# vgl-hub/kreeq

Measured on AMD Instinct MI355X. Metric: distinct+total k-mers/sec at k=21 (count path), higher is better.
Workload: dtype u64

## Files before the change

### include/kreeq_amd.h

```cpp
#ifndef KREEQ_AMD_H
#define KREEQ_AMD_H

#include <stdint.h>

#ifdef __cplusplus
extern "C" {
#endif

#define KQ_ABI_VERSION 4

typedef enum {
    KQ_OK = 0,
    KQ_ERR_INVALID = -1,
    KQ_ERR_NO_DEVICE = -2,
    KQ_ERR_HIP = -3,
    KQ_ERR_NOMEM = -4,
    KQ_ERR_TABLE_FULL = -5,
    KQ_ERR_CAPACITY = -6,
    KQ_ERR_MISMATCH = -7
} kq_status;

typedef struct kq_handle kq_handle;

typedef struct {
    uint64_t key;
    uint32_t fw[4], bw[4], cov;
    uint32_t hc;
} kq_entry;

typedef struct {
    uint32_t fw, bw, cov;
    uint8_t  isFw;
    uint8_t  pad[3];
} kq_dbgbase;

typedef struct {
    uint64_t total;
    uint64_t unique;
    uint64_t distinct;
    uint64_t missing;
    uint64_t edges;
} kq_stats;

typedef struct {
    uint64_t kmers_counted;
    uint64_t slots_used;
    uint64_t slots_total;
    uint64_t hc_used;
    uint64_t hc_total;
    uint64_t table_bytes;
    uint64_t table_passes;
} kq_info;


int  kq_create(kq_handle** out, int device, int k, int map_count, uint64_t capacity_hint);
void kq_destroy(kq_handle* h);
int  kq_clear(kq_handle* h);
int  kq_set_stream(kq_handle* h, void* hip_stream);
void* kq_get_stream(kq_handle* h);
enum { KQ_OPT_TRUST_CAPACITY = 1, KQ_OPT_COUNT_PATH = 2, KQ_OPT_SLICE_KMERS = 3, KQ_OPT_COUNT_MAP_RANGE = 4, KQ_OPT_PROFILE = 5,
       KQ_OPT_LOOKUP_PATH = 6, KQ_OPT_MERGE_PATH = 7, KQ_OPT_NARROW_MID = 8, KQ_OPT_PENDING_BYTES = 9, KQ_OPT_BUCKET_WINDOW = 10, KQ_OPT_OVERLAP = 11, KQ_OPT_COUNT_MAP_PASSES = 12, KQ_OPT_KERNEL_SET = 13, KQ_OPT_SHARD_WINDOW = 14, KQ_OPT_SUBGRAPH_BATCH = 15, KQ_OPT_VARIANT_BATCH = 16,
       KQ_OPT_TEST_FAIL_PLAN = 100  };
int  kq_set_option(kq_handle* h, int option, int64_t value);
int  kq_get_profile(kq_handle* h, char* buf, uint64_t cap);
int  kq_sync(kq_handle* h);
int  kq_flush(kq_handle* h);
int  kq_get_info(kq_handle* h, kq_info* out);
const char* kq_last_error(void);
int  kq_abi_version(void);
int  kq_device_available(void);
int  kq_device_memory(int device, uint64_t* free_bytes, uint64_t* total_bytes);


int  kq_count_batch(kq_handle* h, const char* bases, uint64_t len);
int  kq_count_batch_dev(kq_handle* h, const char* d_bases, uint64_t len);

void* kq_host_alloc(uint64_t bytes);
void  kq_host_free(void* p);
int  kq_count_batch_async(kq_handle* h, const char* bases, uint64_t len, uint64_t* ticket);
int  kq_host_wait(kq_handle* h, uint64_t ticket);

void kq_pack_bases(const char* bases, uint64_t len, uint32_t* codes, uint16_t* inv);
int  kq_count_packed_dev(kq_handle* h, const uint32_t* d_codes, const uint16_t* d_inv, uint64_t n_bases);
int  kq_count_packed_async(kq_handle* h, const uint32_t* codes, const uint16_t* inv, uint64_t n_bases, uint64_t* ticket);

int  kq_pack_bases_dev(kq_handle* h, const char* d_bases, uint64_t len, uint32_t* d_codes, uint16_t* d_inv);

enum { KQ_FASTX_FASTQ = 1, KQ_FASTX_FASTA = 2 };
int  kq_parse_fastx_dev(kq_handle* h, const char* d_text, uint64_t len, int format, char* d_bases, uint64_t cap, uint64_t* n_bases);
int  kq_count_fastx_dev(kq_handle* h, const char* d_text, uint64_t len, int format);
int  kq_count_fastx_async(kq_handle* h, const char* text, uint64_t len, int format, uint64_t* ticket);

typedef struct { uint64_t off; uint32_t size; uint32_t data_off; uint32_t data_len; uint32_t crc32; uint32_t isize; } kq_bgzf_block;
enum { KQ_BGZF_END = 1 };
int  kq_bgzf_scan(const void* data, uint64_t len, kq_bgzf_block* blocks, uint64_t cap, uint64_t* n_blocks, uint64_t* consumed);
int  kq_inflate_bgzf_dev(kq_handle* h, const void* d_comp, uint64_t comp_len, const kq_bgzf_block* blocks, uint64_t n_blocks,
                         char* d_text, uint64_t cap, uint64_t* n_text);
int  kq_count_bgzf_dev(kq_handle* h, const void* d_comp, uint64_t comp_len, const kq_bgzf_block* blocks, uint64_t n_blocks, int format, uint32_t flags);

enum { KQ_BGZF_EOF = 2 };
uint64_t kq_bgzf_bound(uint64_t n_text, uint32_t flags);
int  kq_deflate_bgzf_dev(kq_handle* h, const char* d_text, uint64_t n_text, void* d_out, uint64_t cap, uint64_t* n_out, uint32_t flags);
int  kq_deflate_bgzf(kq_handle* h, const char* text, uint64_t n_text, void* out, uint64_t cap, uint64_t* n_out, uint32_t flags);

int  kq_emit_records(kq_handle* h, const char* bases, uint64_t len,
                     uint64_t* keys, uint8_t* edges, uint64_t cap, uint64_t* n_out);
int  kq_emit_partitioned_dev(kq_handle* h, const char* d_bases, uint64_t len, int n_parts,
                             uint64_t* d_keys, uint8_t* d_edges, uint64_t cap,
                             uint64_t* part_counts);

int  kq_emit_packed_dev(kq_handle* h, const char* d_bases, uint64_t len, int n_parts,
                        uint64_t* d_recs, uint64_t cap, uint64_t* part_counts);
int  kq_insert_packed_dev(kq_handle* h, const uint64_t* d_recs, uint64_t n);

int  kq_emit_sharded_dev(kq_handle* h, const char* d_bases, uint64_t len, int n_parts, uint32_t* d_recs, uint8_t* d_aux, uint64_t cap,
                         uint64_t* d_bucket_counts, uint64_t* part_counts);
int  kq_insert_sharded_dev(kq_handle* h, const uint32_t* d_recs, const uint8_t* d_aux, uint64_t n, int n_peers, const uint64_t* d_bucket_counts);

int  kq_emit_sharded8_dev(kq_handle* h, const char* d_bases, uint64_t len, int n_parts, uint64_t* d_recs, uint64_t cap,
                          uint64_t* d_bucket_counts, uint64_t* part_counts);
int  kq_insert_sharded8_dev(kq_handle* h, const uint64_t* d_recs, uint64_t n, int n_peers, const uint64_t* d_bucket_counts);

int  kq_insert_records(kq_handle* h, const uint64_t* keys, const uint8_t* edges, uint64_t n);
int  kq_insert_records_dev(kq_handle* h, const uint64_t* d_keys, const uint8_t* d_edges, uint64_t n);


int  kq_summary(kq_handle* h, kq_stats* out);
int  kq_histogram(kq_handle* h, uint64_t* cov, uint64_t* cnt, uint64_t cap, uint64_t* n_out);


int  kq_lookup_sequence(kq_handle* h, const char* bases, uint64_t len, uint32_t cov_cutoff,
                        uint16_t map_lo, uint16_t map_hi, kq_dbgbase* per_base,
                        uint64_t counters[3]);
int  kq_lookup_sequence_dev(kq_handle* h, const char* d_bases, uint64_t len, uint32_t cov_cutoff,
                            uint16_t map_lo, uint16_t map_hi, kq_dbgbase* d_per_base,
                            uint64_t* d_counters);


enum { KQ_COPY_TO_DEVICE = 1, KQ_COPY_TO_HOST = 2 };
void* kq_dev_alloc(kq_handle* h, uint64_t bytes);
void  kq_dev_free(kq_handle* h, void* p);
int   kq_copy_async(kq_handle* h, void* dst, const void* src, uint64_t bytes, int kind);

int  kq_per_base_triples_dev(kq_handle* h, const kq_dbgbase* d_per_base, const uint64_t* seg_start, const uint64_t* seg_len,
                             uint64_t n_segs, uint32_t* d_triples);

int  kq_per_base_merge_dev(kq_handle* h, kq_dbgbase* d_per_base, const uint64_t* seg_start, const uint64_t* seg_len,
                           uint64_t n_segs, uint32_t* d_triples);

typedef struct { uint64_t first, n, abs_pos; uint32_t name_off, name_len, n_ctx, flags; } kq_table_seg;
enum { KQ_TABLE_SEG_HEADER = 1 };
enum { KQ_TABLE_KWIG = 1, KQ_TABLE_BED = 2, KQ_TABLE_CSV = 3 };
int  kq_format_table_dev(kq_handle* h, int format, const uint32_t* d_triples, uint64_t n_triples, const kq_table_seg* segs, uint64_t n_segs,
                         const char* names, uint64_t names_len, char* d_out, uint64_t cap, uint64_t* n_out);
int  kq_format_table(kq_handle* h, int format, const uint32_t* triples, uint64_t n_triples, const kq_table_seg* segs, uint64_t n_segs,
                     const char* names, uint64_t names_len, char* out, uint64_t cap, uint64_t* n_out);


int  kq_lookup_keys(kq_handle* h, const uint64_t* keys, uint64_t n, kq_entry* out);

int  kq_branch_scan(kq_handle* h, const char* bases, uint64_t len, uint32_t cov_cutoff, uint8_t* flags);

typedef struct { uint64_t pos, seg_start, seq_off; uint16_t seq_len, ref_len; uint8_t type, pad[3]; } kq_variant_path;
enum { KQ_VAR_SNV = 0, KQ_VAR_INS = 1, KQ_VAR_DEL = 2, KQ_VAR_COM = 3 };
int  kq_search_variants(kq_handle* h, const char* bases, uint64_t len, int depth, int max_span, uint32_t cov_cutoff,
                        kq_variant_path* paths, uint64_t path_cap, uint64_t* n_paths,
                        char* seq, uint64_t seq_cap, uint64_t* n_seq);


int  kq_merge(kq_handle* dst, kq_handle* src);

int  kq_import(kq_handle* h, const kq_entry* entries, uint64_t n);
int  kq_export(kq_handle* h, uint16_t map_lo, uint16_t map_hi, kq_entry* out, uint64_t cap,
               uint64_t* n_out);


int  kq_export_map_images(kq_handle* h, uint16_t map_lo, uint16_t map_hi, void* out, uint64_t cap, uint64_t* offsets,
                          kq_entry* hc_out, uint64_t hc_cap, uint64_t* n_hc);
int  kq_import_map_image(kq_handle* h, uint16_t map, const void* image, uint64_t n_bytes, uint64_t* n_entries,
                         uint64_t* n_tombstones);


enum { KQ_SUBGRAPH_NO_REFERENCE = 1 };
int  kq_subgraph_seed(kq_handle* db, kq_handle* sub, const char* bases, uint64_t len, uint32_t flags);
int  kq_subgraph_seed_dev(kq_handle* db, kq_handle* sub, const char* d_bases, uint64_t len, uint32_t flags);
int  kq_subgraph_expand(kq_handle* db, kq_handle* sub, int depth, uint64_t* n_added);
int  kq_subgraph_best_first(kq_handle* db, kq_handle* sub, int depth, uint32_t cov_cutoff, uint64_t* n_added);
int  kq_subgraph_trim(kq_handle* sub, uint32_t cov_cutoff);

typedef struct { uint64_t seq_off, head_key; uint32_t n_kmers, cov; uint8_t head_rc, pad[7]; } kq_gfa_segment;
typedef struct { uint32_t from, to, count; uint8_t from_rc, to_rc, pad[2]; } kq_gfa_edge;
typedef struct { uint64_t n_segments, n_seq, n_edges, n_dropped_edges, n_cycles; } kq_gfa_counts;
enum { KQ_GFA_NO_COLLAPSE = 1 };
int  kq_subgraph_gfa(kq_handle* sub, uint32_t flags, kq_gfa_segment* segs, uint64_t seg_cap, char* seq, uint64_t seq_cap,
                     kq_gfa_edge* edges, uint64_t edge_cap, kq_gfa_counts* counts);

#ifdef __cplusplus
}
#endif
#endif
```

### kreeq_amd/build.py

```python
import os
import shutil
import subprocess

PKG = os.path.dirname(os.path.abspath(__file__))
ROOT = os.path.dirname(PKG)
LIB = os.path.join(PKG, "lib", "libkreeq_amd.so")
CLI = os.path.join(PKG, "bin", "kreeq")
HOSTLIB = os.path.join(PKG, "lib", "libkreeq_host.so")

HIP_SOURCES = [os.path.join(PKG, "csrc", "kreeq_amd.hip")]
HIP_DEPS = HIP_SOURCES + [os.path.join(PKG, "csrc", f) for f in ("kq_device.h", "kq_partition.h", "kq_kernels.h", "kq_fastx.h", "kq_bgzf.h", "kq_bgzf_host.h", "kq_inflate_core.h", "kq_deflate.h", "kq_deflate_core.h", "kq_dbimage.h", "kq_dbimage_host.h", "kq_mem_host.h", "kq_plan_host.h", "kq_roff_host.h", "kq_seg_gate_host.h", "kq_select_host.h", "kq_formats.h", "kq_subgraph.h", "kq_gfa.h", "kq_bestfirst_core.h", "kq_nodequeue_core.h", "kq_variant_core.h", "kq_variants.h", "kq_table_core.h", "kq_table.h")] + [os.path.join(ROOT, "include", "kreeq_amd.h")]
HOST_DIR = os.path.join(PKG, "host")
DECOMPRESSOR_DIR = os.path.join(HOST_DIR, "decompressor")
DECOMPRESSOR = os.path.join(PKG, "bin", "kreeq-decompressor")


def _stale(target, deps):
    if not os.path.exists(target):
        return True
    t = os.path.getmtime(target)
    return any(os.path.getmtime(d) > t for d in deps if os.path.exists(d))


def hipcc():
    for c in (shutil.which("hipcc"), "/opt/rocm/bin/hipcc"):
        if c and os.path.exists(c):
            return c
    raise RuntimeError("hipcc not found: the HIP library cannot be built (there is no CPU fallback)")


def build_lib(force=False, verbose=False, out=None, defines=()):
    target = out or LIB
    if force or _stale(target, HIP_DEPS):
        os.makedirs(os.path.dirname(target), exist_ok=True)
        cmd = [hipcc(), "-O3", "-std=c++17", "--offload-arch=gfx950", "-fPIC", "-shared", "-Wall", "-Wextra",
               "-o", target] + ["-D" + d for d in defines] + HIP_SOURCES
        if verbose:
            print(" ".join(cmd))
        subprocess.check_call(cmd)
    return target


def host_sources():
    if not os.path.isdir(HOST_DIR):
        return []
    return sorted(os.path.join(HOST_DIR, f) for f in os.listdir(HOST_DIR) if f.endswith(".cpp") and f != "hostlib.cpp")


def build_hostlib(force=False, verbose=False):
    srcs = [os.path.join(HOST_DIR, f) for f in ("hostlib.cpp", "kreeq_db.cpp")]
    deps = srcs + [os.path.join(HOST_DIR, "kreeq_db.h"), os.path.join(ROOT, "include", "kreeq_amd.h")]
    if force or _stale(HOSTLIB, deps):
        os.makedirs(os.path.dirname(HOSTLIB), exist_ok=True)
        cmd = ["g++", "-O2", "-std=c++17", "-Wall", "-Wextra", "-fPIC", "-shared", "-pthread", "-I", os.path.join(ROOT, "include"), "-o", HOSTLIB] + srcs
        if verbose:
            print(" ".join(cmd))
        subprocess.check_call(cmd)
    return HOSTLIB


def build_cli(force=False, verbose=False):
    srcs = host_sources()
    if not srcs:
        return None
    deps = srcs + [os.path.join(HOST_DIR, f) for f in os.listdir(HOST_DIR) if f.endswith(".h")] + [LIB]
    if force or _stale(CLI, deps):
        os.makedirs(os.path.dirname(CLI), exist_ok=True)
        cmd = ["g++", "-O2", "-std=c++17", "-Wall", "-Wextra", "-pthread", "-I", os.path.join(ROOT, "include"), "-o", CLI] + srcs + \
              ["-L", os.path.dirname(LIB), "-lkreeq_amd", "-lz", "-Wl,-rpath,$ORIGIN/../lib"]
        if verbose:
            print(" ".join(cmd))
        subprocess.check_call(cmd)
    return CLI


def build_decompressor(force=False, verbose=False):
    srcs = [os.path.join(DECOMPRESSOR_DIR, "main.cpp")]
    deps = srcs + [os.path.join(HOST_DIR, "bkwig_index.h"), os.path.join(PKG, "csrc", "kq_table_core.h"), os.path.join(ROOT, "include", "kreeq_amd.h"), LIB]
    if force or _stale(DECOMPRESSOR, deps):
        os.makedirs(os.path.dirname(DECOMPRESSOR), exist_ok=True)
        cmd = ["g++", "-O2", "-std=c++17", "-Wall", "-Wextra", "-o", DECOMPRESSOR] + srcs + \
              ["-L", os.path.dirname(LIB), "-lkreeq_amd", "-Wl,-rpath,$ORIGIN/../lib"]
        if verbose:
            print(" ".join(cmd))
        subprocess.check_call(cmd)
    return DECOMPRESSOR


def build_all(force=False, verbose=False):
    build_lib(force, verbose)
    build_cli(force, verbose)
    build_decompressor(force, verbose)
    build_hostlib(force, verbose)
```

### kreeq_amd/capi.py

```python
import ctypes as C
import os

import numpy as np

from . import build as _build

ENTRY_DTYPE = np.dtype([("key", "<u8"), ("fw", "<u4", 4), ("bw", "<u4", 4), ("cov", "<u4"), ("hc", "<u4")])
DBGBASE_DTYPE = np.dtype([("fw", "<u4"), ("bw", "<u4"), ("cov", "<u4"), ("isFw", "u1"), ("pad", "u1", 3)])
VARIANT_PATH_DTYPE = np.dtype([("pos", "<u8"), ("seg_start", "<u8"), ("seq_off", "<u8"), ("seq_len", "<u2"), ("ref_len", "<u2"), ("type", "u1"), ("pad", "u1", 3)])
VAR_SNV, VAR_INS, VAR_DEL, VAR_COM = 0, 1, 2, 3
ERR_CAPACITY = -6

SYMBOLS = ["kq_create", "kq_destroy", "kq_clear", "kq_set_option", "kq_get_profile", "kq_set_stream", "kq_get_stream", "kq_sync", "kq_flush", "kq_get_info", "kq_last_error",
           "kq_abi_version", "kq_device_available", "kq_device_memory", "kq_count_batch", "kq_count_batch_dev", "kq_host_alloc", "kq_host_free", "kq_count_batch_async", "kq_host_wait", "kq_pack_bases", "kq_count_packed_dev", "kq_count_packed_async",
           "kq_pack_bases_dev", "kq_parse_fastx_dev", "kq_count_fastx_dev", "kq_count_fastx_async", "kq_bgzf_scan", "kq_inflate_bgzf_dev", "kq_count_bgzf_dev", "kq_bgzf_bound", "kq_deflate_bgzf_dev", "kq_deflate_bgzf", "kq_emit_records",
           "kq_emit_partitioned_dev", "kq_emit_packed_dev", "kq_insert_packed_dev", "kq_emit_sharded_dev", "kq_insert_sharded_dev", "kq_emit_sharded8_dev", "kq_insert_sharded8_dev", "kq_insert_records", "kq_insert_records_dev", "kq_summary", "kq_histogram",
           "kq_lookup_sequence", "kq_lookup_sequence_dev", "kq_dev_alloc", "kq_dev_free", "kq_copy_async", "kq_per_base_triples_dev", "kq_per_base_merge_dev", "kq_format_table_dev", "kq_format_table", "kq_lookup_keys", "kq_branch_scan", "kq_search_variants", "kq_merge", "kq_import", "kq_export",
           "kq_export_map_images", "kq_import_map_image", "kq_subgraph_seed", "kq_subgraph_seed_dev", "kq_subgraph_expand", "kq_subgraph_best_first", "kq_subgraph_trim", "kq_subgraph_gfa"]

FASTX_FASTQ, FASTX_FASTA = 1, 2
BGZF_END = 1
BGZF_EOF = 2
BGZF_MEMBER_TEXT = 0xff00
BGZF_BLOCK_DTYPE = np.dtype([("off", "<u8"), ("size", "<u4"), ("data_off", "<u4"), ("data_len", "<u4"), ("crc32", "<u4"), ("isize", "<u4"), ("pad", "<u4")])
TABLE_KWIG, TABLE_BED, TABLE_CSV = 1, 2, 3
TABLE_SEG_HEADER = 1
TABLE_SEG_DTYPE = np.dtype([("first", "<u8"), ("n", "<u8"), ("abs_pos", "<u8"), ("name_off", "<u4"), ("name_len", "<u4"), ("n_ctx", "<u4"), ("flags", "<u4")])
SUBGRAPH_NO_REFERENCE = 1
GFA_NO_COLLAPSE = 1
GFA_SEGMENT_DTYPE = np.dtype([("seq_off", "<u8"), ("head_key", "<u8"), ("n_kmers", "<u4"), ("cov", "<u4"), ("head_rc", "u1"), ("pad", "u1", 7)])
GFA_EDGE_DTYPE = np.dtype([("from", "<u4"), ("to", "<u4"), ("count", "<u4"), ("from_rc", "u1"), ("to_rc", "u1"), ("pad", "u1", 2)])


class KqError(RuntimeError):
    def __init__(self, code, msg):
        super().__init__(f"kreeq_amd error {code}: {msg}")
        self.code = code


class Stats(C.Structure):
    _fields_ = [("total", C.c_uint64), ("unique", C.c_uint64), ("distinct", C.c_uint64), ("missing", C.c_uint64),
                ("edges", C.c_uint64)]


class GfaCounts(C.Structure):
    _fields_ = [("n_segments", C.c_uint64), ("n_seq", C.c_uint64), ("n_edges", C.c_uint64), ("n_dropped_edges", C.c_uint64), ("n_cycles", C.c_uint64)]


class Info(C.Structure):
    _fields_ = [("kmers_counted", C.c_uint64), ("slots_used", C.c_uint64), ("slots_total", C.c_uint64), ("hc_used", C.c_uint64),
                ("hc_total", C.c_uint64), ("table_bytes", C.c_uint64), ("table_passes", C.c_uint64)]


_lib = None


def lib_path():
    return _build.LIB


def _preload_process_hip_runtime():
    import importlib.util

    try:
        spec = importlib.util.find_spec("torch")
    except (ImportError, ValueError):
        spec = None
    if not spec or not spec.origin:
        return
    d = os.path.join(os.path.dirname(spec.origin), "lib")
    for name in ("libhsa-runtime64.so", "libamdhip64.so"):
        p = os.path.join(d, name)
        if os.path.exists(p):
            try:
                C.CDLL(p, mode=C.RTLD_GLOBAL)
            except OSError:
                return


def load():
    global _lib
    if _lib is not None:
        return _lib
    path = os.environ.get("KQ_LIB") or _build.LIB
    if not os.path.exists(path):
        raise KqError(-2, f"{path} is missing: build it with `python -c 'import __graft_entry__ as g; g.build()'` "
                          "(the product has no CPU fallback)")
    _preload_process_hip_runtime()
    L = C.CDLL(path)
    vp, u64, u32, u16, ci = C.c_void_p, C.c_uint64, C.c_uint32, C.c_uint16, C.c_int
    L.kq_create.argtypes = [C.POINTER(vp), ci, ci, ci, u64]
    L.kq_destroy.argtypes = [vp]
    L.kq_destroy.restype = None
    L.kq_clear.argtypes = [vp]
    L.kq_set_stream.argtypes = [vp, vp]
    L.kq_set_option.argtypes = [vp, ci, C.c_int64]
    L.kq_get_profile.argtypes = [vp, C.c_char_p, u64]
    L.kq_get_stream.argtypes = [vp]
    L.kq_get_stream.restype = vp
    L.kq_sync.argtypes = [vp]
    L.kq_flush.argtypes = [vp]
    L.kq_get_info.argtypes = [vp, C.POINTER(Info)]
    L.kq_last_error.restype = C.c_char_p
    L.kq_device_memory.argtypes = [ci, C.POINTER(u64), C.POINTER(u64)]
    L.kq_count_batch.argtypes = [vp, vp, u64]
    L.kq_count_batch_dev.argtypes = [vp, vp, u64]
    L.kq_host_alloc.argtypes = [u64]
    L.kq_host_alloc.restype = vp
    L.kq_host_free.argtypes = [vp]
    L.kq_host_free.restype = None
    L.kq_count_batch_async.argtypes = [vp, vp, u64, C.POINTER(u64)]
    L.kq_host_wait.argtypes = [vp, u64]
    L.kq_pack_bases.argtypes = [vp, u64, vp, vp]
    L.kq_pack_bases.restype = None
    L.kq_count_packed_dev.argtypes = [vp, vp, vp, u64]
    L.kq_count_packed_async.argtypes = [vp, vp, vp, u64, C.POINTER(u64)]
    L.kq_pack_bases_dev.argtypes = [vp, vp, u64, vp, vp]
    L.kq_parse_fastx_dev.argtypes = [vp, vp, u64, ci, vp, u64, C.POINTER(u64)]
    L.kq_count_fastx_dev.argtypes = [vp, vp, u64, ci]
    L.kq_count_fastx_async.argtypes = [vp, vp, u64, ci, C.POINTER(u64)]
    L.kq_bgzf_scan.argtypes = [vp, u64, vp, u64, C.POINTER(u64), C.POINTER(u64)]
    L.kq_inflate_bgzf_dev.argtypes = [vp, vp, u64, vp, u64, vp, u64, C.POINTER(u64)]
    L.kq_count_bgzf_dev.argtypes = [vp, vp, u64, vp, u64, ci, u32]
    L.kq_bgzf_bound.argtypes = [u64, u32]
    L.kq_bgzf_bound.restype = u64
    L.kq_deflate_bgzf_dev.argtypes = [vp, vp, u64, vp, u64, C.POINTER(u64), u32]
    L.kq_deflate_bgzf.argtypes = [vp, vp, u64, vp, u64, C.POINTER(u64), u32]
    L.kq_emit_records.argtypes = [vp, vp, u64, vp, vp, u64, C.POINTER(u64)]
    L.kq_emit_partitioned_dev.argtypes = [vp, vp, u64, ci, vp, vp, u64, vp]
    L.kq_emit_packed_dev.argtypes = [vp, vp, u64, ci, vp, u64, vp]
    L.kq_insert_packed_dev.argtypes = [vp, vp, u64]
    L.kq_emit_sharded_dev.argtypes = [vp, vp, u64, ci, vp, vp, u64, vp, vp]
    L.kq_insert_sharded_dev.argtypes = [vp, vp, vp, u64, ci, vp]
    L.kq_emit_sharded8_dev.argtypes = [vp, vp, u64, ci, vp, u64, vp, vp]
    L.kq_insert_sharded8_dev.argtypes = [vp, vp, u64, ci, vp]
    L.kq_insert_records.argtypes = [vp, vp, vp, u64]
    L.kq_insert_records_dev.argtypes = [vp, vp, vp, u64]
    L.kq_summary.argtypes = [vp, C.POINTER(Stats)]
    L.kq_histogram.argtypes = [vp, vp, vp, u64, C.POINTER(u64)]
    L.kq_lookup_sequence.argtypes = [vp, vp, u64, u32, u16, u16, vp, vp]
    L.kq_lookup_sequence_dev.argtypes = [vp, vp, u64, u32, u16, u16, vp, vp]
    L.kq_dev_alloc.argtypes = [vp, u64]
    L.kq_dev_alloc.restype = vp
    L.kq_dev_free.argtypes = [vp, vp]
    L.kq_dev_free.restype = None
    L.kq_copy_async.argtypes = [vp, vp, vp, u64, ci]
    L.kq_per_base_triples_dev.argtypes = [vp, vp, vp, vp, u64, vp]
    L.kq_per_base_merge_dev.argtypes = [vp, vp, vp, vp, u64, vp]
    L.kq_format_table_dev.argtypes = [vp, ci, vp, u64, vp, u64, vp, u64, vp, u64, C.POINTER(u64)]
    L.kq_format_table.argtypes = [vp, ci, vp, u64, vp, u64, vp, u64, vp, u64, C.POINTER(u64)]
    L.kq_lookup_keys.argtypes = [vp, vp, u64, vp]
    L.kq_branch_scan.argtypes = [vp, vp, u64, u32, vp]
    L.kq_search_variants.argtypes = [vp, vp, u64, ci, ci, u32, vp, u64, C.POINTER(u64), vp, u64, C.POINTER(u64)]
    L.kq_merge.argtypes = [vp, vp]
    L.kq_import.argtypes = [vp, vp, u64]
    L.kq_export.argtypes = [vp, u16, u16, vp, u64, C.POINTER(u64)]
    L.kq_export_map_images.argtypes = [vp, u16, u16, vp, u64, vp, vp, u64, C.POINTER(u64)]
    L.kq_import_map_image.argtypes = [vp, u16, vp, u64, C.POINTER(u64), C.POINTER(u64)]
    L.kq_subgraph_seed.argtypes = [vp, vp, vp, u64, u32]
    L.kq_subgraph_seed_dev.argtypes = [vp, vp, vp, u64, u32]
    L.kq_subgraph_expand.argtypes = [vp, vp, ci, C.POINTER(u64)]
    L.kq_subgraph_best_first.argtypes = [vp, vp, ci, u32, C.POINTER(u64)]
    L.kq_subgraph_trim.argtypes = [vp, u32]
    L.kq_subgraph_gfa.argtypes = [vp, u32, vp, u64, vp, u64, vp, u64, C.POINTER(GfaCounts)]
    _lib = L
    return L


def _check(rc):
    if rc != 0:
        raise KqError(rc, load().kq_last_error().decode(errors="replace"))


def _p(a):
    return a.ctypes.data_as(C.c_void_p) if a is not None else None


def pack_bases(bases: bytes):
    buf = np.frombuffer(bases, dtype=np.uint8)
    units = (len(buf) + 15) // 16
    codes, inv = np.zeros(max(units, 1), dtype=np.uint32), np.zeros(max(units, 1), dtype=np.uint16)
    load().kq_pack_bases(_p(buf) if len(buf) else None, len(buf), _p(codes), _p(inv))
    return codes[:units], inv[:units]


def bgzf_bound(n_text, flags=0):
    return int(load().kq_bgzf_bound(n_text, flags))


def bgzf_scan(data: bytes, cap=None):
    buf = np.frombuffer(data, dtype=np.uint8)
    n, used = C.c_uint64(0), C.c_uint64(0)
    L = load()
    room = len(buf) // 26 + 1 if cap is None else cap
    blocks = np.zeros(max(room, 1), dtype=BGZF_BLOCK_DTYPE)
    rc = L.kq_bgzf_scan(_p(buf) if len(buf) else None, len(buf), _p(blocks) if room else None, room, C.byref(n), C.byref(used))
    if rc != 0:
        e = KqError(rc, L.kq_last_error().decode(errors="replace"))
        e.n_blocks, e.consumed = n.value, used.value
        raise e
    return blocks[:n.value], used.value


def device_available():
# ... 356 lines not shown
```

### kreeq_amd/csrc/kq_formats.h

```cpp
#pragma once
#include <cstdint>
namespace kq {
#ifndef KQ_REGION_SHIFT
#define KQ_REGION_SHIFT 11
#endif
constexpr int REGION_SHIFT = KQ_REGION_SHIFT;
constexpr uint32_t REGION_SLOTS = 1u << REGION_SHIFT;
constexpr int HI_K = 29;
constexpr int TILE_STARTS = 4032;
constexpr uint64_t n_tiles_of(uint64_t lead, uint64_t len) { return (lead + len + TILE_STARTS - 1) / TILE_STARTS; }
struct EmitRange { uint64_t lo, hi; };

constexpr int NB_MAX = 2048;
constexpr int PART_MAX_K = 28;
constexpr int FMT_PACK8 = 0, FMT_WIDE = 1, FMT_NARROW = 2;
constexpr int FMT_PACK8_TO_NARROW = 3;
constexpr uint32_t NARROW_CBITS = 8, NARROW_MAX_K = 21;
constexpr int FMT_TOP8 = 4;
constexpr int FMT_TIGHT = 5;
constexpr int FMT_NARROW_TO_TIGHT = 6;

constexpr int MS_THREADS = 256;
constexpr int MS_ITEMS = 16;
constexpr int MS_TILE = MS_THREADS * MS_ITEMS;
constexpr int SEG_MAX = 65536;
constexpr uint32_t SUB_BITS_MAX = 8;
constexpr int AUX_IDX6 = 0, AUX_EDGE_BYTE = 1, AUX_TIGHT = 2;
constexpr uint64_t TIGHT_MIN_REGIONS = 1ull << 16;
constexpr int P1_F = 1;
constexpr uint32_t P2_UNIT = 4 * MS_TILE;
constexpr uint32_t SCAN_CHUNK = 16384;

struct PartCfg {
    uint64_t n_regions;
    uint32_t g_shift;
    uint32_t n_coarse;
    uint32_t mode;
    uint32_t map_count;
    uint32_t map_mask;
    uint32_t filt_lo, filt_hi;
    uint32_t raw_out;
    uint32_t narrow;
    uint32_t owner_sub;
    uint32_t sub_bits;
    uint32_t win_lo, win_hi;
    uint32_t n_rng;
};

constexpr int P3_MAX_SETS = 64;
struct P3Set { const uint64_t* recs; const uint8_t* aux; const unsigned long long* base; uint64_t n_max; };

struct LevelCfg {
    uint64_t n_regions;
    uint32_t n_seg, nb, seg_shift, out_shift;
    uint32_t in_raw;
    uint32_t k;
    uint32_t narrow;
    uint32_t top8;
    uint32_t nr_shift, nr_rps, nr_sub, nr_div, nr_inv;
    uint32_t nr_mid, nr_fshift, nr_fmask, nr_f24;
    uint32_t spb;
    uint32_t rep_shift;
    const uint32_t* rstart = nullptr;
};
}
```

### kreeq_amd/csrc/kq_kernels.h

```cpp
#pragma once

#include <hip/hip_runtime.h>

#include <type_traits>

#include "../../include/kreeq_amd.h"
#include "kq_device.h"
#include "kq_partition.h"

using namespace kq;


__global__ __launch_bounds__(TILE_THREADS) void k_count_direct(TableView t, const uint8_t* __restrict__ ab,
                                                                uint64_t lead, uint64_t len, int k, EmitRange er, PartCfg filt,
                                                                const uint16_t* __restrict__ pinv ) {
    uint32_t n_new = 0;
    uint64_t n_kmers = 0;
    scan_tiles(ab, lead, len, k, [&](uint64_t pos, uint64_t fw, uint64_t rv, uint32_t prev, uint32_t next) {
        if (pos < er.lo || pos >= er.hi) return;
        const bool is_fw = fw < rv;
        const uint64_t key = is_fw ? fw : rv;
        if (filt.filt_lo != 0 || filt.filt_hi != filt.map_count) {
            const uint32_t m = map_index(key, filt.map_count, filt.map_mask);
            if (m < filt.filt_lo || m >= filt.filt_hi) return;
// ... 376 lines not shown
        });
        landed(nxt.x); landed(nxt.y); landed(nxt.z); landed(nxt.w);
    }
}

__global__ __launch_bounds__(1024) void k_lv_units(const unsigned long long* __restrict__ seg_off, const unsigned long long* __restrict__ seg_hi, LevelCfg lv,
                                                   unsigned long long* __restrict__ unit_base) {
    __shared__ unsigned long long s_part[1024];
    const uint32_t tid = threadIdx.x, per = (lv.n_seg + 1023) / 1024;
    const uint32_t lo = min(tid * per, lv.n_seg), hi = min(lo + per, lv.n_seg);
    unsigned long long sum = 0;
    for (uint32_t b = lo; b < hi; ++b) sum += (seg_hi[b] - seg_off[b] + P2_UNIT - 1) / P2_UNIT;
    s_part[tid] = sum;
    __syncthreads();
    if (tid < 64) {
        unsigned long long loc[16], tot = 0;
#pragma unroll
        for (int j = 0; j < 16; ++j) { loc[j] = s_part[tid * 16 + j]; tot += loc[j]; }
        unsigned long long incl = tot;
#pragma unroll
        for (int o = 1; o < 64; o <<= 1) { unsigned long long nn = __shfl_up(incl, o, 64); if ((int)tid >= o) incl += nn; }
        unsigned long long run = incl - tot;
#pragma unroll
        for (int j = 0; j < 16; ++j) { s_part[tid * 16 + j] = run; run += loc[j]; }
        if (tid == 63) unit_base[lv.n_seg] = incl;
    }
    __syncthreads();
    unsigned long long run = s_part[tid];
    for (uint32_t b = lo; b < hi; ++b) { unit_base[b] = run; run += (seg_hi[b] - seg_off[b] + P2_UNIT - 1) / P2_UNIT; }
}
__device__ __forceinline__ uint32_t seg_of_unit(const unsigned long long* unit_base, uint32_t n_seg, uint64_t u) {
    uint32_t lo = 0, hi = n_seg;
    while (hi - lo > 1) { uint32_t mid = (lo + hi) >> 1; if (unit_base[mid] <= u) lo = mid; else hi = mid; }
    return lo;
}
template <int FMT>
__global__ __launch_bounds__(MS_THREADS) void k_lv_hist(const uint64_t* __restrict__ recs, const uint8_t* __restrict__ , LevelCfg lv,
                                                        const unsigned long long* __restrict__ seg_off, const unsigned long long* __restrict__ seg_hi,
                                                        const unsigned long long* __restrict__ unit_base, uint32_t* __restrict__ m2) {
    __shared__ uint32_t s_hist[NB_MAX];
    const uint64_t n_units = unit_base[lv.n_seg];
    for (uint64_t u = blockIdx.x; u < n_units; u += gridDim.x) {
        const uint32_t b_in = seg_of_unit(unit_base, lv.n_seg, u);
        const uint32_t b = lv.spb > 1 ? b_in / lv.spb : b_in;
        const uint64_t lo = seg_off[b_in] + (u - unit_base[b_in]) * P2_UNIT;
        const uint64_t hi = lo + P2_UNIT < seg_hi[b_in] ? lo + P2_UNIT : seg_hi[b_in];
        for (uint32_t i = threadIdx.x; i < lv.nb; i += MS_THREADS) s_hist[i] = 0;
        __syncthreads();
        const uint64_t last = hi - 1;
        if (FMT == FMT_NARROW) {
            const uint4* v4 = reinterpret_cast<const uint4*>(recs);
            const uint64_t q0 = lo >> 2, q1 = (hi + 3) >> 2;
            for (uint64_t qb = q0; qb < q1; qb += 4ull * MS_THREADS) {
                uint4 q[4];
#pragma unroll
                for (int j = 0; j < 4; ++j) q[j] = v4[min(qb + (uint64_t)j * MS_THREADS + threadIdx.x, q1 - 1)];
#pragma unroll
                for (int j = 0; j < 4; ++j) {
                    const uint64_t qi = qb + (uint64_t)j * MS_THREADS + threadIdx.x;
                    const uint32_t e[4] = {q[j].x, q[j].y, q[j].z, q[j].w};
#pragma unroll
                    for (int c = 0; c < 4; ++c) {
                        const uint64_t ri = 4 * qi + c;
                        if (qi < q1 && ri >= lo && ri < hi) atomicAdd(&s_hist[narrow_bin(lv, b, e[c])], 1u);
                    }
                }
            }
        } else
        for (uint64_t base = lo; base < hi; base += 8ull * MS_THREADS) {
            uint64_t r[8];
#pragma unroll
            for (int j = 0; j < 8; ++j) {
                const uint64_t i = min(base + (uint64_t)j * MS_THREADS + threadIdx.x, last);
                r[j] = FMT == FMT_NARROW ? (uint64_t)reinterpret_cast<const uint32_t*>(recs)[i] : recs[i];
            }
#pragma unroll
            for (int j = 0; j < 8; ++j)
                if (base + (uint64_t)j * MS_THREADS + threadIdx.x < hi) {
                    const uint32_t bin = FMT == FMT_NARROW ? narrow_bin(lv, b, (uint32_t)r[j])
                        : FMT == FMT_TOP8 ? narrow_bin(lv, b, (uint32_t)(r[j] >> 32))
                        : (FMT == FMT_PACK8 && lv.top8) ? (uint32_t)(rec_hash<false>(r[j]) >> (64 - NARROW_CBITS))
                        : level_bin(lv, b, hash_region(lv.in_raw ? table_hash(r[j], lv.k) : rec_hash<FMT == FMT_WIDE>(r[j]), lv.n_regions));
                    atomicAdd(&s_hist[bin], 1u);
                }
        }
        __syncthreads();
        for (uint32_t i = threadIdx.x; i < lv.nb; i += MS_THREADS) m2[u * lv.nb + i] = s_hist[i];
        __syncthreads();
    }
}
__global__ __launch_bounds__(256) void k_lv_offsets(uint32_t* __restrict__ m2, LevelCfg lv, const unsigned long long* __restrict__ unit_base,
                                                    unsigned long long* __restrict__ group_count) {
    const uint64_t r = ((uint64_t)blockIdx.x * blockDim.x + threadIdx.x) >> 6;
    const uint32_t lane = threadIdx.x & 63;
    const uint32_t n_lseg = lv.n_seg / lv.spb;
    if (r >= (uint64_t)n_lseg * lv.nb) return;
    const uint32_t b = (uint32_t)(r / lv.nb), bin = (uint32_t)(r % lv.nb);
    const uint64_t u0 = unit_base[b * lv.spb], u1 = unit_base[(b + 1) * lv.spb];
    unsigned long long run = 0;
    for (uint64_t base = u0; base < u1; base += 64) {
        const uint64_t u = base + lane;
        const uint32_t c = u < u1 ? m2[u * lv.nb + bin] : 0u;
        unsigned long long incl = c;
#pragma unroll
        for (int o = 1; o < 64; o <<= 1) { const unsigned long long n = __shfl_up(incl, o, 64); if ((int)lane >= o) incl += n; }
        if (u < u1) m2[u * lv.nb + bin] = (uint32_t)(run + incl - c);
        run += __shfl(incl, 63, 64);
    }
    if (lane == 0) group_count[r] = run;
}
__global__ __launch_bounds__(256) void k_lv_offsets_thread(uint32_t* __restrict__ m2, LevelCfg lv, const unsigned long long* __restrict__ unit_base,
                                                           unsigned long long* __restrict__ group_count) {
    const uint64_t r = (uint64_t)blockIdx.x * blockDim.x + threadIdx.x;
    const uint32_t n_lseg = lv.n_seg / lv.spb;
    if (r >= (uint64_t)n_lseg * lv.nb) return;
    const uint32_t b = (uint32_t)(r / lv.nb), bin = (uint32_t)(r % lv.nb);
    const uint64_t u0 = unit_base[b * lv.spb], u1 = unit_base[(b + 1) * lv.spb];
    unsigned long long run = 0;
    for (uint64_t u = u0; u < u1; ++u) {
        const uint32_t c = m2[u * lv.nb + bin];
        m2[u * lv.nb + bin] = (uint32_t)run;
        run += c;
    }
    group_count[r] = run;
}
#ifndef KQ_LV_THREADS
#define KQ_LV_THREADS 512
#define KQ_LV_ITEMS 8
#define KQ_LV_OCC 4
#endif
constexpr int LV_THREADS = KQ_LV_THREADS, LV_ITEMS = KQ_LV_ITEMS, LV_TILE = LV_THREADS * LV_ITEMS;
template <int FMT, int NBC>
__global__ __launch_bounds__(LV_THREADS, KQ_LV_OCC) void k_lv_scatter(const uint64_t* __restrict__ recs, const uint8_t* __restrict__ recs_aux, LevelCfg lv,
                                                           const unsigned long long* __restrict__ seg_off, const unsigned long long* __restrict__ seg_hi,
                                                           const unsigned long long* __restrict__ unit_base, const uint32_t* __restrict__ m2,
                                                           const unsigned long long* __restrict__ group_base, uint64_t* __restrict__ out,
                                                           uint8_t* __restrict__ out_aux) {
    constexpr bool WIDE = FMT == FMT_WIDE, TIGHT = FMT == FMT_NARROW_TO_TIGHT, NARROW = FMT == FMT_NARROW || TIGHT, CONVERT = FMT == FMT_PACK8_TO_NARROW,
                   TOP8 = FMT == FMT_TOP8, HAS_AUX = WIDE || NARROW;
    constexpr int MS_FMT = (CONVERT || TIGHT) ? FMT_NARROW : TOP8 ? FMT_PACK8 : FMT;
    const uint32_t* recs32 = reinterpret_cast<const uint32_t*>(recs);
    __shared__ MsShared<NBC, MS_FMT, LV_TILE> s;
    __shared__ uint32_t s_rst[TIGHT ? NBC : 1];
    const uint32_t nb = lv.nb;
    const uint64_t n_units = unit_base[lv.n_seg];
    for (uint64_t u = blockIdx.x; u < n_units; u += gridDim.x) {
        const uint32_t b_in = seg_of_unit(unit_base, lv.n_seg, u);
        const uint32_t b = lv.spb > 1 ? b_in / lv.spb : b_in;
        const uint64_t lo = seg_off[b_in] + (u - unit_base[b_in]) * P2_UNIT;
        const uint64_t hi = lo + P2_UNIT < seg_hi[b_in] ? lo + P2_UNIT : seg_hi[b_in];
        for (uint32_t i = threadIdx.x; i < nb; i += LV_THREADS)
            s.gbase[i] = (uint32_t)(group_base[(uint64_t)b * nb + i] + m2[u * nb + i]);
        if (TIGHT) {
            const uint32_t first = (b >> lv.nr_shift) * lv.nr_rps + (b & ((1u << lv.nr_shift) - 1u)) * lv.nr_sub;
            for (uint32_t i = threadIdx.x; i < nb; i += LV_THREADS) s_rst[i] = lv.rstart[first + i];
        }
        __syncthreads();
        uint64_t nxt[LV_ITEMS];
        uint32_t nxt_aux[LV_ITEMS];
        const uint64_t last = hi - 1;
#pragma unroll
        for (int j = 0; j < LV_ITEMS; ++j) {
            const uint64_t i = min(lo + (uint64_t)j * LV_THREADS + threadIdx.x, last);
            nxt[j] = NARROW ? (uint64_t)recs32[i] : recs[i];
            nxt_aux[j] = HAS_AUX ? recs_aux[i] : 0;
        }
#pragma unroll
        for (int j = 0; j < LV_ITEMS; ++j) { landed(nxt[j]); if (HAS_AUX) landed(nxt_aux[j]); }
        for (uint64_t pos = lo; pos < hi; pos += LV_TILE) {
            uint64_t rec[LV_ITEMS];
            uint32_t aux[LV_ITEMS], bin[LV_ITEMS];
#pragma unroll
            for (int j = 0; j < LV_ITEMS; ++j) {
                const uint64_t i = pos + (uint64_t)j * LV_THREADS + threadIdx.x;
                rec[j] = (WIDE && lv.in_raw) ? table_hash(nxt[j], lv.k) : nxt[j];
                aux[j] = nxt_aux[j];
                if (TIGHT) {
                    const uint32_t bn = i >= hi ? nb : narrow_bin(lv, b, (uint32_t)rec[j]);
                    rec[j] = narrow_word(tight_rec(b >> lv.nr_shift, (uint32_t)rec[j], aux[j], s_rst[bn < nb ? bn : 0u]), 0u, bn);
                }
                else if (NARROW) rec[j] = narrow_word((uint32_t)rec[j], aux[j], i >= hi ? nb : narrow_bin(lv, b, (uint32_t)rec[j]));
                else if (CONVERT) {
                    const uint64_t hh = rec_hash<false>(rec[j]);
                    rec[j] = narrow_word(narrow_main(hh), narrow_aux(hh, (uint32_t)(rec[j] >> REC_EDGE_SHIFT) & 63u), i >= hi ? nb : (uint32_t)(hh >> (64 - NARROW_CBITS)));
                }
                else if (TOP8) bin[j] = i >= hi ? nb : narrow_bin(lv, b, (uint32_t)(rec[j] >> 32));
                else bin[j] = i >= hi ? nb : level_bin(lv, b, hash_region(rec_hash<WIDE>(rec[j]), lv.n_regions));
            }
#pragma unroll
            for (int j = 0; j < LV_ITEMS; ++j) {
                const uint64_t i = min(pos + LV_TILE + (uint64_t)j * LV_THREADS + threadIdx.x, last);
                nxt[j] = NARROW ? (uint64_t)recs32[i] : recs[i];
                nxt_aux[j] = HAS_AUX ? recs_aux[i] : 0;
            }
            block_multisplit<MS_FMT, LV_THREADS, LV_ITEMS>(s, rec, aux, bin, nb, out, out_aux, [&] {
#pragma unroll
                for (int j = 0; j < LV_ITEMS; ++j) { landed(nxt[j]); if (HAS_AUX) landed(nxt_aux[j]); }
            }, NBC <= 512 ? lv.rep_shift : 0u);
        }
    }
}
#ifndef KQ_LVS_OCC
#define KQ_LVS_OCC 4
#define KQ_LVS_OCC_TIGHT 4
#endif
template <bool TIGHT>
__global__ __launch_bounds__(LV_THREADS, TIGHT ? KQ_LVS_OCC_TIGHT : KQ_LVS_OCC) void k_lv_scatter_s(const uint32_t* __restrict__ recs32, const uint8_t* __restrict__ recs_aux, LevelCfg lv,
                                                           const unsigned long long* __restrict__ seg_off, const unsigned long long* __restrict__ seg_hi,
                                                           const unsigned long long* __restrict__ unit_base, const uint32_t* __restrict__ m2,
                                                           const unsigned long long* __restrict__ group_base, uint32_t* __restrict__ out,
                                                           uint8_t* __restrict__ out_aux) {
    constexpr int NC = 512;
    static_assert(LV_THREADS == NC && LV_ITEMS == 8, "one counter per thread");
    __shared__ uint64_t s_buf[LV_TILE];
    __shared__ uint32_t s_hist[2][NC], s_loff[NC + 1], s_grel[NC], s_wave[LV_THREADS / 64];
    __shared__ uint32_t s_rst[TIGHT ? NC : 1];
    const int tid = threadIdx.x;
    const uint32_t nb = lv.nb, rs = lv.rep_shift, n_ctr = (nb + 1) << rs;
    const uint32_t sub = (uint32_t)tid & ((1u << rs) - 1u), my_bin = (uint32_t)tid >> rs;
    const bool own_bin = sub == 0 && my_bin < nb;
    const uint64_t n_units = unit_base[lv.n_seg];
    for (uint64_t u = blockIdx.x; u < n_units; u += gridDim.x) {
        const uint32_t b_in = seg_of_unit(unit_base, lv.n_seg, u);
        const uint32_t b = lv.spb > 1 ? b_in / lv.spb : b_in;
        const uint64_t lo = seg_off[b_in] + (u - unit_base[b_in]) * P2_UNIT;
        const uint64_t hi = lo + P2_UNIT < seg_hi[b_in] ? lo + P2_UNIT : seg_hi[b_in];
        uint32_t gabs = own_bin ? (uint32_t)(group_base[(uint64_t)b * nb + my_bin] + m2[u * nb + my_bin]) : 0u;
        if (TIGHT) {
            const uint32_t first = (b >> lv.nr_shift) * lv.nr_rps + (b & ((1u << lv.nr_shift) - 1u)) * lv.nr_sub;
            if ((uint32_t)tid < nb) s_rst[tid] = lv.rstart[first + tid];
        }
        s_hist[0][tid] = 0;
        __syncthreads();
        uint32_t nxt[LV_ITEMS], nxt_aux[LV_ITEMS];
        const uint64_t last = hi - 1;
#pragma unroll
        for (int j = 0; j < LV_ITEMS; ++j) {
            const uint64_t i = min(lo + (uint64_t)j * LV_THREADS + tid, last);
            nxt[j] = recs32[i];
            nxt_aux[j] = recs_aux[i];
        }
#pragma unroll
        for (int j = 0; j < LV_ITEMS; ++j) { landed(nxt[j]); landed(nxt_aux[j]); }
        uint32_t par = 0;
        for (uint64_t pos = lo; pos < hi; pos += LV_TILE, par ^= 1u) {
            uint32_t* hist = s_hist[par];
            uint64_t w[LV_ITEMS];
#pragma unroll
            for (int j = 0; j < LV_ITEMS; ++j) {
                const uint64_t i = pos + (uint64_t)j * LV_THREADS + tid;
                const uint32_t bn = i >= hi ? nb : narrow_bin(lv, b, nxt[j]);
                w[j] = TIGHT ? narrow_word(tight_rec(b >> lv.nr_shift, nxt[j], nxt_aux[j], s_rst[bn < nb ? bn : 0u]), 0u, bn) : narrow_word(nxt[j], nxt_aux[j], bn);
                if (bn != nb) atomicAdd(&hist[(bn << rs) | sub], 1u);
            }
#pragma unroll
            for (int j = 0; j < LV_ITEMS; ++j) {
                const uint64_t i = min(pos + LV_TILE + (uint64_t)j * LV_THREADS + tid, last);
                nxt[j] = recs32[i];
                nxt_aux[j] = recs_aux[i];
            }
            __syncthreads();
            const uint32_t cnt = (uint32_t)tid < n_ctr ? hist[tid] : 0u;
            uint32_t incl = cnt;
#pragma unroll
            for (int o = 1; o < 64; o <<= 1) { const uint32_t n = __shfl_up(incl, o, 64); if ((tid & 63) >= o) incl += n; }
            if ((tid & 63) == 63) s_wave[tid >> 6] = incl;
            s_hist[par ^ 1u][tid] = 0;
            __syncthreads();
            uint32_t excl = incl - cnt;
            for (int v = 0; v < (tid >> 6); ++v) excl += s_wave[v];
            s_loff[tid] = excl;
            hist[tid] = excl;
            if (own_bin) s_grel[my_bin] = gabs - excl;
            __syncthreads();
            if (own_bin) gabs += s_loff[(my_bin + 1) << rs] - excl;
#pragma unroll
            for (int j = 0; j < LV_ITEMS; ++j) {
                const uint32_t bn = narrow_word_bin(w[j]);
                if (bn != nb) s_buf[atomicAdd(&hist[(bn << rs) | sub], 1u)] = w[j];
            }
            __syncthreads();
            const uint32_t total = s_loff[nb << rs];
            uint64_t cv[LV_ITEMS];
            uint32_t cg[LV_ITEMS];
#pragma unroll
            for (int it = 0; it < LV_ITEMS; ++it) cv[it] = s_buf[tid + it * LV_THREADS];
#pragma unroll
            for (int it = 0; it < LV_ITEMS; ++it) cg[it] = s_grel[(uint32_t)(tid + it * LV_THREADS) < total ? narrow_word_bin(cv[it]) : 0u] + (tid + it * LV_THREADS);
#pragma unroll
            for (int j = 0; j < LV_ITEMS; ++j) { landed(nxt[j]); landed(nxt_aux[j]); }
#pragma unroll
            for (int it = 0; it < LV_ITEMS; ++it) {
                if ((uint32_t)(tid + it * LV_THREADS) < total) {
                    out[cg[it]] = (uint32_t)cv[it];
                    if (!TIGHT) out_aux[cg[it]] = (uint8_t)(cv[it] >> 48);
                }
            }
        }
    }
}
#ifndef KQ_LVG_BACK
#define KQ_LVG_BACK 0
#endif
__global__ __launch_bounds__(LV_THREADS, KQ_LVS_OCC_TIGHT) void k_lv_segment_s(const uint32_t* __restrict__ recs32, const uint8_t* __restrict__ recs_aux, LevelCfg lv,
                                                           const unsigned long long* __restrict__ seg_off, unsigned long long* __restrict__ gb,
                                                           uint32_t* __restrict__ out) {
    constexpr int NC = 512;
    constexpr bool BACK = KQ_LVG_BACK != 0;
    static_assert(LV_THREADS == NC && LV_ITEMS == 8, "one counter per thread");
    __shared__ uint64_t s_buf[LV_TILE];
    __shared__ uint32_t s_hist[2][NC], s_loff[NC + 1], s_grel[NC], s_wave[LV_THREADS / 64], s_rst[NC];
    const int tid = threadIdx.x;
    const uint32_t nb = lv.nb, rs = lv.rep_shift, n_ctr = (nb + 1) << rs;
    const uint32_t sub = (uint32_t)tid & ((1u << rs) - 1u), my_bin = (uint32_t)tid >> rs;
    const bool own_bin = sub == 0 && my_bin < nb;
    const uint32_t b = blockIdx.x;
    const uint64_t lo = seg_off[b], hi = seg_off[b + 1];
    {
        const uint32_t first = (b >> lv.nr_shift) * lv.nr_rps + (b & ((1u << lv.nr_shift) - 1u)) * lv.nr_sub;
        if ((uint32_t)tid < nb) s_rst[tid] = lv.rstart[first + tid];
    }
    s_hist[0][tid] = 0;
    s_hist[1][tid] = 0;
    __syncthreads();
    {
        const uint4* v4 = reinterpret_cast<const uint4*>(recs32);
        const uint64_t q0 = lo >> 2, q1 = hi > lo ? (hi + 3) >> 2 : q0;
        for (uint64_t qb = q0; qb < q1; qb += 4ull * LV_THREADS) {
            uint4 q[4];
#pragma unroll
            for (int j = 0; j < 4; ++j) q[j] = v4[min(qb + (uint64_t)j * LV_THREADS + tid, q1 - 1)];
#pragma unroll
            for (int j = 0; j < 4; ++j) {
                const uint64_t qi = qb + (uint64_t)j * LV_THREADS + tid;
                const uint32_t e[4] = {q[j].x, q[j].y, q[j].z, q[j].w};
#pragma unroll
                for (int c = 0; c < 4; ++c) {
                    const uint64_t ri = 4 * qi + c;
                    if (qi < q1 && ri >= lo && ri < hi) atomicAdd(&s_hist[1][(narrow_bin(lv, b, e[c]) << rs) | sub], 1u);
                }
            }
        }
    }
    __syncthreads();
    uint32_t gabs = 0;
    {
        uint32_t cnt = 0;
        if (own_bin) for (uint32_t r = 0; r < (1u << rs); ++r) cnt += s_hist[1][(uint32_t)tid + r];
        uint32_t incl = cnt;
#pragma unroll
        for (int o = 1; o < 64; o <<= 1) { const uint32_t n = __shfl_up(incl, o, 64); if ((tid & 63) >= o) incl += n; }
        if ((tid & 63) == 63) s_wave[tid >> 6] = incl;
        __syncthreads();
        uint32_t excl = incl - cnt;
        for (int v = 0; v < (tid >> 6); ++v) excl += s_wave[v];
        if (own_bin) {
            gabs = (uint32_t)lo + excl;
            gb[(uint64_t)b * nb + my_bin] = lo + excl;
        }
        if (b + 1 == lv.n_seg && tid == 0) gb[(uint64_t)lv.n_seg * nb] = hi;
    }
    if (hi == lo) return;
    uint32_t nxt[LV_ITEMS], nxt_aux[LV_ITEMS];
    const uint64_t last = hi - 1, n_rounds = (hi - lo + LV_TILE - 1) / LV_TILE;
    uint64_t pos = BACK ? lo + (n_rounds - 1) * LV_TILE : lo;
#pragma unroll
    for (int j = 0; j < LV_ITEMS; ++j) {
        const uint64_t i = min(pos + (uint64_t)j * LV_THREADS + tid, last);
        nxt[j] = recs32[i];
        nxt_aux[j] = recs_aux[i];
    }
#pragma unroll
    for (int j = 0; j < LV_ITEMS; ++j) { landed(nxt[j]); landed(nxt_aux[j]); }
    uint32_t par = 0;
    for (uint64_t r = 0; r < n_rounds; ++r, par ^= 1u) {
        uint32_t* hist = s_hist[par];
        uint64_t w[LV_ITEMS];
#pragma unroll
        for (int j = 0; j < LV_ITEMS; ++j) {
            const uint64_t i = pos + (uint64_t)j * LV_THREADS + tid;
            const uint32_t bn = i >= hi ? nb : narrow_bin(lv, b, nxt[j]);
            w[j] = narrow_word(tight_rec(b >> lv.nr_shift, nxt[j], nxt_aux[j], s_rst[bn < nb ? bn : 0u]), 0u, bn);
            if (bn != nb) atomicAdd(&hist[(bn << rs) | sub], 1u);
        }
        pos = BACK ? (r + 1 < n_rounds ? pos - LV_TILE : pos) : pos + LV_TILE;
#pragma unroll
        for (int j = 0; j < LV_ITEMS; ++j) {
            const uint64_t i = min(pos + (uint64_t)j * LV_THREADS + tid, last);
            nxt[j] = recs32[i];
            nxt_aux[j] = recs_aux[i];
        }
        __syncthreads();
        const uint32_t cnt = (uint32_t)tid < n_ctr ? hist[tid] : 0u;
        uint32_t incl = cnt;
#pragma unroll
        for (int o = 1; o < 64; o <<= 1) { const uint32_t n = __shfl_up(incl, o, 64); if ((tid & 63) >= o) incl += n; }
        if ((tid & 63) == 63) s_wave[tid >> 6] = incl;
        s_hist[par ^ 1u][tid] = 0;
        __syncthreads();
        uint32_t excl = incl - cnt;
        for (int v = 0; v < (tid >> 6); ++v) excl += s_wave[v];
        s_loff[tid] = excl;
        hist[tid] = excl;
        if (own_bin) s_grel[my_bin] = gabs - excl;
        __syncthreads();
        if (own_bin) gabs += s_loff[(my_bin + 1) << rs] - excl;
#pragma unroll
        for (int j = 0; j < LV_ITEMS; ++j) {
            const uint32_t bn = narrow_word_bin(w[j]);
            if (bn != nb) s_buf[atomicAdd(&hist[(bn << rs) | sub], 1u)] = w[j];
        }
        __syncthreads();
        const uint32_t total = s_loff[nb << rs];
        uint64_t cv[LV_ITEMS];
        uint32_t cg[LV_ITEMS];
#pragma unroll
        for (int it = 0; it < LV_ITEMS; ++it) cv[it] = s_buf[tid + it * LV_THREADS];
#pragma unroll
        for (int it = 0; it < LV_ITEMS; ++it) cg[it] = s_grel[(uint32_t)(tid + it * LV_THREADS) < total ? narrow_word_bin(cv[it]) : 0u] + (tid + it * LV_THREADS);
#pragma unroll
        for (int j = 0; j < LV_ITEMS; ++j) { landed(nxt[j]); landed(nxt_aux[j]); }
#pragma unroll
        for (int it = 0; it < LV_ITEMS; ++it)
            if ((uint32_t)(tid + it * LV_THREADS) < total) out[cg[it]] = (uint32_t)cv[it];
    }
}
__global__ void k_set2(unsigned long long* p, unsigned long long a, unsigned long long b) { p[0] = a; p[1] = b; }

__global__ __launch_bounds__(1024) void k_scan_sums(const unsigned long long* __restrict__ a, uint64_t n, unsigned long long* __restrict__ sums) {
    const uint64_t lo = (uint64_t)blockIdx.x * SCAN_CHUNK, hi = lo + SCAN_CHUNK < n ? lo + SCAN_CHUNK : n;
    unsigned long long v = 0;
    for (uint64_t i = lo + threadIdx.x; i < hi; i += 1024) v += a[i];
    uint64_t t = block_sum(v);
    if (threadIdx.x == 0) sums[blockIdx.x] = t;
}
__global__ __launch_bounds__(1024) void k_scan_apply(unsigned long long* __restrict__ a, uint64_t n, const unsigned long long* __restrict__ sums) {
    __shared__ unsigned long long s_part[1024];
    const uint64_t lo = (uint64_t)blockIdx.x * SCAN_CHUNK + (uint64_t)threadIdx.x * (SCAN_CHUNK / 1024);
    unsigned long long v[SCAN_CHUNK / 1024], sum = 0;
#pragma unroll
    for (uint32_t j = 0; j < SCAN_CHUNK / 1024; ++j) { v[j] = lo + j < n ? a[lo + j] : 0; sum += v[j]; }
    s_part[threadIdx.x] = sum;
    __syncthreads();
    if (threadIdx.x < 64) {
        unsigned long long loc[16], tot = 0;
#pragma unroll
        for (int j = 0; j < 16; ++j) { loc[j] = s_part[threadIdx.x * 16 + j]; tot += loc[j]; }
        unsigned long long incl = tot;
#pragma unroll
        for (int o = 1; o < 64; o <<= 1) { unsigned long long nn = __shfl_up(incl, o, 64); if ((int)threadIdx.x >= o) incl += nn; }
        unsigned long long run = incl - tot;
#pragma unroll
        for (int j = 0; j < 16; ++j) { s_part[threadIdx.x * 16 + j] = run; run += loc[j]; }
    }
    __syncthreads();
    unsigned long long run = sums[blockIdx.x] + s_part[threadIdx.x];
#pragma unroll
    for (uint32_t j = 0; j < SCAN_CHUNK / 1024; ++j) { if (lo + j < n) a[lo + j] = run; run += v[j]; }
}


template <class T> __device__ __forceinline__ T ld_global(const T* p) { return *(const __attribute__((address_space(1))) T*)p; }

template <uint32_t GRP, class LO = uint64_t>
struct SetTickets {
    LO lo; uint32_t cnt, first, n_grp;
    __device__ __forceinline__ void build(const P3Set* __restrict__ sets, uint32_t n_sets, uint64_t r, uint32_t lane) {
        lo = 0; cnt = 0;
        if (lane < n_sets) { const unsigned long long* b = ld_global(&sets[lane].base); lo = (LO)ld_global(b + r); cnt = (uint32_t)(ld_global(b + r + 1) - lo); }
// ... 1025 lines not shown
```

### kreeq_amd/csrc/kq_select_host.h

```cpp
#pragma once
#include "kq_formats.h"

namespace kq {

constexpr int KS_P1_ROUND2 = 1,
              KS_LV_NARROW_S = 2,
              KS_LV_TIGHT_UNITS = 4,
              KS_P3_SET_OFFSETS = 16,
              KS_SEG_NEVER = 32,
              KS_SEG_ALWAYS = 64,
              KS_P1_NO_COMPACT = 128,
              KS_ALL = KS_P1_ROUND2 | KS_LV_NARROW_S | KS_LV_TIGHT_UNITS | KS_P3_SET_OFFSETS | KS_SEG_NEVER | KS_SEG_ALWAYS | KS_P1_NO_COMPACT;

enum Kernel { K_P1_HIST, K_P1_SCATTER, K_P1_SCATTER_S, K_P1_SCATTER_C, K_LV_HIST, K_LV_SCATTER, K_LV_SCATTER_S, K_LV_SEGMENT_S, K_LV_UNITS ,
              K_COUNT_REGIONS, K_COUNT_REGIONS_Q4, K_COUNT_REGIONS_Q4R, K_LOOKUP_REGIONS };
struct KernelSel {
    Kernel fam; int fmt = 0, nbc = 0, bin = 0, kc = 0, tpr = 0; bool flag = false;
    bool operator==(const KernelSel& o) const { return fam == o.fam && fmt == o.fmt && nbc == o.nbc && bin == o.bin && kc == o.kc && tpr == o.tpr && flag == o.flag; }
};
inline KernelSel sel_of(Kernel fam, int fmt, int nbc, int bin, int kc, int tpr = 0, bool flag = false) { KernelSel s{fam}; s.fmt = fmt; s.nbc = nbc; s.bin = bin; s.kc = kc; s.tpr = tpr; s.flag = flag; return s; }

struct P1Case { bool plain, owner_plain, narrow_filt, narrow_win; };
inline P1Case p1_case(int k, uint32_t mode, uint32_t narrow, uint32_t map_mask, bool full_range, bool windowed) {
    const bool plain = mode == 0 && full_range;
    return P1Case{plain, mode == 1 && map_mask != 0 && full_range, mode == 0 && narrow && !plain && map_mask != 0 && k <= (int)NARROW_MAX_K,
                  plain && narrow && (k <= (int)NARROW_MAX_K || k > PART_MAX_K) && windowed};
}
inline KernelSel select_p1_hist(int k, uint32_t mode, uint32_t narrow, uint32_t map_mask, bool full_range, bool windowed) {
    const P1Case c = p1_case(k, mode, narrow, map_mask, full_range, windowed);
    const int bin = c.owner_plain ? 3 : c.narrow_filt ? 4 : c.narrow_win ? 6 : !c.plain ? 0 : narrow ? 2 : 1;
    return sel_of(K_P1_HIST, 0, 0, bin, bin == 0 ? 0 : bin == 1 ? (k == 31 ? 31 : 0) : bin == 6 && k == 31 ? 31 : k == 21 ? 21 : 0);
}
inline KernelSel select_p1_hist_cached(int k, int pass_bin) { return sel_of(K_P1_HIST, 0, 0, pass_bin == 4 ? 5 : 2, k == 21 ? 21 : 0); }
inline KernelSel select_p1_scatter(int k, uint32_t mode, uint32_t narrow, uint32_t map_mask, bool full_range, bool windowed, bool lockstep,
                                   uint32_t n_coarse, int tpr, int kernel_set) {
    const P1Case c = p1_case(k, mode, narrow, map_mask, full_range, windowed);
    const bool small = n_coarse < 512;
    const int nbc = small ? 512 : NB_MAX, kc21 = k == 21 ? 21 : 0, kc31 = k == 31 ? 31 : 0;
    if (narrow) {
        const bool top8 = k > PART_MAX_K;
        int bin, kc, t = 1;
        if (top8) { bin = c.narrow_win ? 6 : c.plain ? 2 : 0; kc = bin ? kc31 : 0; }
        else if (c.narrow_filt) { bin = 4; kc = kc21; }
        else if (c.narrow_win) { bin = 6; kc = kc21; }
        else if (c.plain) { bin = 2; kc = kc21; t = tpr; }
        else { bin = 0; kc = 0; }
        if (kernel_set & KS_P1_ROUND2) return sel_of(K_P1_SCATTER, top8 ? FMT_TOP8 : FMT_NARROW, 512, bin, kc);
        if (bin == 4 && !(kernel_set & KS_P1_NO_COMPACT)) return sel_of(K_P1_SCATTER_C, 0, 0, 0, kc);
        return sel_of(K_P1_SCATTER_S, 0, 0, bin, kc, t, top8);
    }
    if (lockstep) return c.plain && k == 31 ? sel_of(K_P1_SCATTER, FMT_WIDE, nbc, 1, 31)  : sel_of(K_P1_SCATTER, FMT_WIDE, nbc, 0, 0);
    if (c.owner_plain && small) return sel_of(K_P1_SCATTER, FMT_PACK8, 512, 3, kc21);
    return sel_of(K_P1_SCATTER, FMT_PACK8, nbc, c.plain ? 1 : 0, 0);
}

inline int level_format(uint32_t lv_narrow, bool lockstep) { return lv_narrow == 2 ? FMT_TOP8 : lv_narrow ? FMT_NARROW : lockstep ? FMT_WIDE : FMT_PACK8; }
inline KernelSel select_level_hist(uint32_t lv_narrow, bool lockstep) { return sel_of(K_LV_HIST, level_format(lv_narrow, lockstep), 0, 0, 0); }
inline KernelSel select_level_scatter(uint32_t lv_narrow, bool lockstep, bool lv_top8, uint32_t nb, bool rstart, int kernel_set) {
    const int fmt = level_format(lv_narrow, lockstep), nbc = nb < 512 ? 512 : NB_MAX;
    if (lv_top8) return sel_of(K_LV_SCATTER, FMT_PACK8_TO_NARROW, 512, 0, 0);
    if (fmt == FMT_NARROW && nb < 512 && (rstart ? !(kernel_set & KS_LV_TIGHT_UNITS) : (kernel_set & KS_LV_NARROW_S) != 0)) return sel_of(K_LV_SCATTER_S, 0, 0, 0, 0, 0, rstart);
    return sel_of(K_LV_SCATTER, fmt == FMT_NARROW && rstart ? FMT_NARROW_TO_TIGHT : fmt, nbc, 0, 0);
}
inline KernelSel select_last_level(int plan_fmt, uint32_t lv_narrow, bool rstart, uint32_t nr_shift, uint32_t nb, uint32_t spb, bool even_buckets, int kernel_set) {
    const bool ok = plan_fmt == FMT_NARROW && lv_narrow == 1 && rstart && nr_shift != 0 && nb < 512 && spb == 1;
    return sel_of(ok && ((kernel_set & KS_SEG_ALWAYS) || (even_buckets && !(kernel_set & KS_SEG_NEVER))) ? K_LV_SEGMENT_S : K_LV_UNITS, 0, 0, 0, 0);
}

inline bool table_pass_wants_matrix(int fmt, int kernel_set) { return (fmt == FMT_TIGHT || fmt == FMT_NARROW) && !(kernel_set & KS_P3_SET_OFFSETS); }
inline KernelSel select_table_pass(int fmt, int k, bool matrix) {
    if (fmt == FMT_TIGHT || fmt == FMT_NARROW) return sel_of(matrix ? K_COUNT_REGIONS_Q4R : K_COUNT_REGIONS_Q4, 0, 0, 0, k == 21 ? 21 : 0, 0, fmt == FMT_TIGHT);
    return sel_of(K_COUNT_REGIONS, fmt, 0, 0, 0);
}
inline KernelSel select_hot_pass(int fmt) { return sel_of(K_COUNT_REGIONS, fmt == FMT_TIGHT ? FMT_NARROW : fmt, 0, 0, 0, 0, true); }
inline KernelSel select_lookup(int fmt) { return sel_of(K_LOOKUP_REGIONS, fmt, 0, 0, 0); }

}
```

### kreeq_amd/csrc/kreeq_amd.hip

```cpp
#include <hip/hip_runtime.h>
#include <hipcub/hipcub.hpp>

#include <algorithm>
#include <cstdarg>
#include <cstdio>
#include <cstdlib>
#include <cstring>
#include <mutex>
#include <new>
#include <numeric>
#include <string>
#include <thread>
#include <type_traits>
#include <vector>

#include "../../include/kreeq_amd.h"
#include "kq_device.h"
#include "kq_partition.h"
#include "kq_mem_host.h"
#include "kq_plan_host.h"
#include "kq_roff_host.h"
#include "kq_seg_gate_host.h"
#include "kq_select_host.h"
#include "kq_bgzf_host.h"

using namespace kq;

#include "kq_kernels.h"
#include "kq_fastx.h"
#include "kq_bgzf.h"
#include "kq_deflate.h"
#include "kq_dbimage.h"
#include "kq_subgraph.h"
#include "kq_gfa.h"
#include "kq_variants.h"
#include "kq_table.h"


static thread_local std::string g_err;
static int fail(int code, const char* fmt, ...) {
    char buf[512];
    va_list ap; va_start(ap, fmt); vsnprintf(buf, sizeof buf, fmt, ap); va_end(ap);
    g_err = buf;
    return code;
}
#define HIPC(expr)                                                                                   \
    do {                                                                                             \
        hipError_t e_ = (expr);                                                                      \
        if (e_ != hipSuccess)                                                                        \
            return fail(e_ == hipErrorOutOfMemory ? KQ_ERR_NOMEM : KQ_ERR_HIP, "%s: %s (%s:%d)", #expr, \
                        hipGetErrorString(e_), __FILE__, __LINE__);                                  \
    } while (0)

struct Scrambled {
    void* p = nullptr; size_t bytes = 0, chunk = 0;
    std::vector<hipMemGenericAllocationHandle_t> hs;
    bool vmm = false;

    Scrambled() = default;
    Scrambled(const Scrambled&) = delete;
    Scrambled& operator=(const Scrambled&) = delete;
    Scrambled(Scrambled&& o) noexcept { swap(o); }
    Scrambled& operator=(Scrambled&& o) noexcept { if (this != &o) { reset(); swap(o); } return *this; }
    ~Scrambled() { reset(); }
    void swap(Scrambled& o) noexcept { std::swap(p, o.p); std::swap(bytes, o.bytes); std::swap(chunk, o.chunk); hs.swap(o.hs); std::swap(vmm, o.vmm); }
    friend void swap(Scrambled& a, Scrambled& b) noexcept { a.swap(b); }

    void reset() {
        if (!p) return;
        (void)hipDeviceSynchronize();
        if (vmm) {
            (void)hipMemUnmap(p, hs.size() * chunk);
            for (auto& hnd : hs) (void)hipMemRelease(hnd);
            (void)hipMemAddressFree(p, hs.size() * chunk);
        } else (void)hipFree(p);
        p = nullptr; bytes = chunk = 0; hs.clear(); vmm = false;
    }
    bool alloc(size_t n, int device, bool try_vmm) {
        reset();
        if (try_vmm && map_chunks(n, device)) return true;
        if (hipMalloc(&p, n) != hipSuccess) { (void)hipGetLastError(); p = nullptr; return false; }
        bytes = n; vmm = false;
        return true;
    }
private:
    bool map_chunks(size_t n_bytes, int device) {
        static const size_t chunk_mb = getenv("KQ_SCRAMBLE_MB") ? (size_t)atoi(getenv("KQ_SCRAMBLE_MB")) : 2;
        if (!chunk_mb) return false;
        hipMemAllocationProp prop = {};
        prop.type = hipMemAllocationTypePinned; prop.location.type = hipMemLocationTypeDevice; prop.location.id = device;
        size_t gran = 0;
        if (hipMemGetAllocationGranularity(&gran, &prop, hipMemAllocationGranularityMinimum) != hipSuccess || !gran) { (void)hipGetLastError(); return false; }
        const size_t ck = ((chunk_mb << 20) + gran - 1) / gran * gran, n = (n_bytes + ck - 1) / ck;
        void* base = nullptr;
        if (hipMemAddressReserve(&base, n * ck, 0, nullptr, 0) != hipSuccess) { (void)hipGetLastError(); return false; }
        std::vector<hipMemGenericAllocationHandle_t> fresh;
        fresh.reserve(n);
        bool ok = true;
        for (size_t i = 0; i < n && ok; ++i) { hipMemGenericAllocationHandle_t hnd; ok = hipMemCreate(&hnd, ck, &prop, 0) == hipSuccess; if (ok) fresh.push_back(hnd); }
        size_t mapped = 0;
        if (ok) {
            size_t mul = 7919;
            while (std::gcd(mul, n) != 1) ++mul;
            for (; mapped < n && ok; ++mapped) ok = hipMemMap((char*)base + mapped * ck, ck, 0, fresh[(mapped * mul + 13) % n], 0) == hipSuccess;
            if (!ok) --mapped;
        }
        if (ok) {
            hipMemAccessDesc acc = {};
            acc.location = prop.location; acc.flags = hipMemAccessFlagsProtReadWrite;
            ok = hipMemSetAccess(base, n * ck, &acc, 1) == hipSuccess;
        }
        if (!ok) {
            (void)hipGetLastError();
            if (mapped) (void)hipMemUnmap(base, mapped * ck);
            for (auto& hnd : fresh) (void)hipMemRelease(hnd);
            (void)hipMemAddressFree(base, n * ck);
            return false;
        }
        p = base; bytes = n * ck; chunk = ck; hs.swap(fresh); vmm = true;
        return true;
    }
};
static int scr_ensure(Scrambled& b, size_t need, int device) {
    if (b.bytes >= need) return KQ_OK;
    b.reset();
    const size_t sz = need + std::min<size_t>(need / 4, (size_t)256 << 20) + 4096;
    if (!b.alloc(sz, device, true)) return fail(KQ_ERR_NOMEM, "partition scratch allocation failed");
    return KQ_OK;
}

struct ScratchSet { DevMem part; Scrambled part2; };

struct kq_handle {
    int device = 0, k = 0, map_count = 0;
    Stream own_stream;
    hipStream_t stream = nullptr;
    int n_cu = 256;
    DevMem slots;
    uint64_t n_regions = 0;
    uint32_t win_lo = 0, win_hi = 256;
    bool windowed = false;
    DevMem hc;
    uint64_t hc_cap = 0;
    DevMem rstart;
    DevMem st;
    PinnedMem st_host;
    DevMem scratch;
    DevMem stage;
    uint64_t kmers_bound = 0;
    uint64_t used_bound = 0;
    uint64_t hc_check_at = 0;
    bool table_empty = true;
    uint32_t mid_rps = 2048;
    int merge_path = 0;
    int lookup_path = 0;
    bool slots_dirty = false;
    bool trust_capacity = false;
    int count_path = 0;
    uint64_t slice_kmers = 1ull << 28;
    bool slice_user = false;
    uint32_t filt_lo = 0, filt_hi = 0;
    bool profile = false;
    std::vector<std::pair<const char*, Event>> marks;
    ScratchSet work, fork_work;
    hipStream_t base = nullptr;
    Stream fork_stream[2];
    bool fork_busy[2] = {false, false};
    static constexpr int EV_RING = 64;
    Event ev_ring[EV_RING];
    uint64_t ev_next = 0;
    int overlap = 1;
    int kernel_set = 0;
    struct HistKey { const void* ab; const void* pinv; uint64_t lead, len, er_lo, er_hi; uint32_t g1, n_rng; int k;
                     bool operator==(const HistKey& o) const { return ab == o.ab && pinv == o.pinv && lead == o.lead && len == o.len && er_lo == o.er_lo && er_hi == o.er_hi && g1 == o.g1 && n_rng == o.n_rng && k == o.k; } };
    struct HistEntry { HistKey key; DevMem m1_all; };
    std::vector<HistEntry> hist_cache;
    size_t hist_cache_bytes = 0;
    int map_passes = 1;
    Scrambled arena;
    size_t arena_bytes = 0, arena_used = 0;
    DevMem d_sets;
    P3Set pend_sets[P3_MAX_SETS] = {};
    DevMem tot;
    DevMem roff;
    int n_pend = 0, pend_fmt = -1, pend_aux_fmt = 0;
    uint64_t pend_records = 0;
    int64_t pend_budget = -1;
    uint64_t table_passes = 0;
    static constexpr int IN_SLOTS = 3, IN_TICKETS = 512;
    Stream copy_stream;
    DevMem in_buf[IN_SLOTS];
    Event in_consumed[IN_SLOTS];
    std::vector<Event> in_copied;
    uint64_t in_next = 0;
    std::mutex in_m;
    uint8_t in_bad[IN_TICKETS] = {};
    DevMem fx_units, fx_out, in_cmp[IN_SLOTS];
    DevMem fx_res;
    PinnedMem fx_res_host;
    int fx_bad = 0;
    DevMem bz_desc, bz_stat, bz_text, bz_carry;
    PinnedMem bz_desc_host, bz_stat_host;
    DevMem df_slots, df_sizes, df_offs, df_stat, df_in, df_out;
    PinnedMem df_stat_host;
    uint64_t bz_carry_len = 0;
    bool bz_bad = false;
    std::string bz_err;
    bool hist_cache_off = false;
    bool test_fail_plan = false;
    DevMem hot;
    uint64_t var_batch = 0;
    uint64_t sg_batch = 0;
    std::vector<DevMem> user_mem;
    DevMem tab_segs;

    TableView view() const {
        TableView v; v.slots = slots.as<Slot>() - (reg_lo() << REGION_SHIFT); v.n_regions = n_regions; v.hc = hc.as<HcSlot>(); v.hc_mask = hc_cap - 1; v.st = d_state(); v.k = (uint32_t)k;
        v.reg_lo = reg_lo(); v.reg_hi = reg_hi();
        v.rps = k >= HI_K ? (uint32_t)(n_regions >> 8) : 0u;
        v.rstart = rstart.as<uint32_t>();
        return v;
    }
    DevState* d_state() const { return st.as<DevState>(); }
    DevState* host_state() const { return st_host.as<DevState>(); }
    FxResult* fx_host() const { return fx_res_host.as<FxResult>(); }
    uint64_t reg_lo() const { return windowed ? (uint64_t)win_lo * (n_regions >> 8) : 0; }
    uint64_t reg_hi() const { return windowed ? (uint64_t)win_hi * (n_regions >> 8) : n_regions; }
    uint64_t n_alloc_regions() const { return reg_hi() - reg_lo(); }
    uint64_t n_slots() const { return n_alloc_regions() << REGION_SHIFT; }
    uint64_t table_bytes() const { return n_slots() * sizeof(Slot); }
    TableShape shape() const { return TableShape{k, n_regions, map_count, mid_rps}; }
};

static void marks_reset(kq_handle* h);
static int flush_pending(kq_handle* h);

static int ev_get(kq_handle* h, hipEvent_t* out) {
    Event& e = h->ev_ring[h->ev_next++ % kq_handle::EV_RING];
    if (!e) HIPC(e.create(hipEventDisableTiming));
    else HIPC(hipEventSynchronize(e.get()));
    *out = e.get();
    return KQ_OK;
}
static int join_forks(kq_handle* h) {
    for (int w = 0; w < 2; ++w) {
        if (!h->fork_busy[w]) continue;
        hipEvent_t e; int rc = ev_get(h, &e); if (rc) return rc;
        HIPC(hipEventRecord(e, h->fork_stream[w].get()));
        HIPC(hipStreamWaitEvent(h->base, e, 0));
        h->fork_busy[w] = false;
    }
    return KQ_OK;
}

static int grid_for(const kq_handle* h, uint64_t work_items, int per_block, int per_cu = 8) {
    uint64_t blocks = (work_items + per_block - 1) / per_block;
    uint64_t cap = (uint64_t)h->n_cu * per_cu;
    if (blocks > cap) blocks = cap;
    if (blocks < 1) blocks = 1;
    return (int)blocks;
}

static void clear_words(kq_handle* h, void* p, uint32_t words_per_slot, uint64_t n_slots) {
    const uint64_t n_pairs = n_slots * words_per_slot / 2;
    hipLaunchKernelGGL(k_clear_slots, dim3(grid_for(h, n_pairs, 256)), dim3(256), 0, h->stream, (ulonglong2*)p, words_per_slot, n_pairs);
}
static void clear_main(kq_handle* h, Slot* p, uint64_t n_slots) { (void)hipMemsetAsync(p, 0, (size_t)n_slots * sizeof(Slot), h->stream); }
static void materialize(kq_handle* h) {
    if (!h->slots_dirty) return;
    clear_main(h, h->slots.as<Slot>(), h->n_slots());
    h->slots_dirty = false;
}
static int alloc_main(kq_handle* h, uint64_t n_regions, uint64_t alloc_regions, DevMem& slots, DevMem& rstart) {
    HIPC(slots.alloc((size_t)(alloc_regions << REGION_SHIFT) * sizeof(Slot)));
    if (rstart.alloc((size_t)(n_regions + 1) * sizeof(uint32_t)) != hipSuccess) { slots.reset(); return fail(KQ_ERR_NOMEM, "region index allocation failed"); }
    clear_main(h, slots.as<Slot>(), alloc_regions << REGION_SHIFT);
    hipLaunchKernelGGL(k_region_starts, dim3(grid_for(h, n_regions + 1, 256)), dim3(256), 0, h->stream, rstart.as<uint32_t>(), n_regions);
    return KQ_OK;
}
static int alloc_hc(kq_handle* h, uint64_t cap, DevMem& hc) {
    HIPC(hc.alloc((size_t)cap * sizeof(HcSlot)));
    clear_words(h, hc.get(), sizeof(HcSlot) / 8, cap);
    return KQ_OK;
}

static int read_state_raw(kq_handle* h) {
    HIPC(hipMemcpyAsync(h->host_state(), h->d_state(), sizeof(DevState), hipMemcpyDeviceToHost, h->stream));
    HIPC(hipStreamSynchronize(h->stream));
    return KQ_OK;
}
static int read_state(kq_handle* h) {
    int frc = flush_pending(h);
    if (frc) return frc;
    return read_state_raw(h);
}
static int check_errors(kq_handle* h) {
    int rc = read_state(h);
    if (rc) return rc;
    if (h->host_state()->err_table_full) return fail(KQ_ERR_TABLE_FULL, "k-mer table region overflow (slots %llu / %llu)",
                                                 (unsigned long long)h->host_state()->slots_used, (unsigned long long)h->n_slots());
    if (h->host_state()->err_hc_full) return fail(KQ_ERR_TABLE_FULL, "high-copy side table overflow (%llu / %llu)",
                                              (unsigned long long)h->host_state()->hc_used, (unsigned long long)h->hc_cap);
    return KQ_OK;
}

static int grow_main(kq_handle* h, uint64_t need_slots) {
    int frc = flush_pending(h);
    if (frc) return frc;
    const GrowTarget grown = grow_target(h->n_slots(), h->n_regions, need_slots);
    const uint64_t want = grown.slots, new_regions = grown.regions;
    if (!grown.ok) return fail(KQ_ERR_TABLE_FULL, "cannot grow k-mer table to %llu slots: region index overflow", (unsigned long long)want);
    DevMem slots, rstart;
    int rc = alloc_main(h, new_regions, want >> REGION_SHIFT, slots, rstart);
    if (rc) return rc == KQ_ERR_NOMEM ? fail(KQ_ERR_TABLE_FULL, "cannot grow k-mer table to %llu slots: out of device memory",
                                             (unsigned long long)want) : rc;
    const uint64_t n_old = h->n_slots();
    const TableView old_view = h->view();
    slots.swap(h->slots); rstart.swap(h->rstart);
    h->n_regions = new_regions;
    if (h->slots_dirty) h->slots_dirty = false;
    else hipLaunchKernelGGL(k_rehash, dim3(grid_for(h, n_old, 256)), dim3(256), 0, h->stream, h->view(), old_view);
    HIPC(hipStreamSynchronize(h->stream));
    return KQ_OK;
}
static int grow_hc(kq_handle* h, uint64_t need) {
    uint64_t want = h->hc_cap;
    while (want < need) want *= 2;
    DevMem hc;
    int rc = alloc_hc(h, want, hc);
    if (rc) return rc;
    const uint64_t n_old = h->hc_cap;
    hc.swap(h->hc); h->hc_cap = want;
    HIPC(hipMemsetAsync(&h->d_state()->hc_used, 0, sizeof(unsigned long long), h->stream));
    hipLaunchKernelGGL(k_rehash_hc, dim3(grid_for(h, n_old, 256)), dim3(256), 0, h->stream, h->view(), hc.as<HcSlot>(), n_old);
    HIPC(hipStreamSynchronize(h->stream));
    return KQ_OK;
}

static int reserve(kq_handle* h, uint64_t extra, uint64_t extra_instances) {
    int rc;
    bool state_read = false;
    if (!h->trust_capacity) {
        uint64_t need = main_need(h->used_bound, extra);
        if (need > h->n_slots()) {
            rc = read_state(h); if (rc) return rc;
            state_read = true;
            h->used_bound = h->host_state()->slots_used;
            need = main_need(h->used_bound, extra);
            if (need > h->n_slots()) { rc = grow_main(h, need); if (rc) return rc; }
        }
    }
    h->used_bound += extra;
    h->kmers_bound += extra_instances;
    uint64_t need_hc = hc_need(h->kmers_bound);
    if (hc_follows_fill(h->kmers_bound) && h->kmers_bound >= h->hc_check_at && h->n_pend == 0) {
        if (!state_read) { rc = read_state_raw(h); if (rc) return rc; }
        need_hc = hc_need(h->kmers_bound, h->host_state()->hc_used);
        h->hc_check_at = 2 * h->kmers_bound;
    }
    if (need_hc > h->hc_cap) { rc = grow_hc(h, need_hc); if (rc) return rc; }
    return KQ_OK;
}

static int stage_in(kq_handle* h, const void* host, size_t bytes, void** dev) {
    HIPC(h->stage.ensure(bytes + 64));
    if (bytes) HIPC(hipMemcpyAsync(h->stage.get(), host, bytes, hipMemcpyHostToDevice, h->stream));
    *dev = h->stage.get();
    return KQ_OK;
}

static void parallel_sort_entries(kq_entry* a, uint64_t n) {
    auto less = [](const kq_entry& x, const kq_entry& y) { return x.key < y.key; };
    unsigned hw = std::thread::hardware_concurrency();
    unsigned t = std::max(1u, std::min(16u, hw ? hw : 1u));
    while (t > 1 && n / t < (1u << 16)) t /= 2;
    if (t <= 1) { std::sort(a, a + n, less); return; }
    std::vector<uint64_t> cut(t + 1);
    for (unsigned i = 0; i <= t; ++i) cut[i] = n * i / t;
    {
        std::vector<std::thread> th;
        for (unsigned i = 0; i < t; ++i) th.emplace_back([&, i] { std::sort(a + cut[i], a + cut[i + 1], less); });
        for (auto& x : th) x.join();
    }
    for (unsigned width = 1; width < t; width *= 2) {
        std::vector<std::thread> th;
        for (unsigned i = 0; i + width < t; i += 2 * width) {
            const uint64_t lo = cut[i], mid = cut[i + width], hi = cut[std::min(i + 2 * width, t)];
            th.emplace_back([=] { std::inplace_merge(a + lo, a + mid, a + hi, less); });
        }
        for (auto& x : th) x.join();
    }
}

template <class Fn> struct KernelRow { KernelSel sel; Fn fn; };
template <class Fn, size_t N, class... A>
static int launch_row(const KernelRow<Fn> (&rows)[N], const char* family, const KernelSel& s, kq_handle* h, dim3 grid, dim3 block, A... args) {
    for (const KernelRow<Fn>& r : rows) if (r.sel == s) { hipLaunchKernelGGL(r.fn, grid, block, 0, h->stream, args...); return KQ_OK; }
    return fail(KQ_ERR_INVALID, "%s has no instantiation <fmt %d, nbc %d, bin %d, kc %d, tpr %d, flag %d> (selector family %d)", family, s.fmt, s.nbc, s.bin, s.kc, s.tpr, (int)s.flag, (int)s.fam);
}
template <int B, int K> static KernelRow<decltype(&k_p1_hist<0, 0>)> p1h() { return {sel_of(K_P1_HIST, 0, 0, B, K), k_p1_hist<B, K>}; }
template <int W, int N, int B, int K> static KernelRow<decltype(&k_p1_scatter<0, 512, 0, 0>)> p1w() { return {sel_of(K_P1_SCATTER, W, N, B, K), k_p1_scatter<W, N, B, K>}; }
template <int B, int K, int T, bool TOP8 = false> static KernelRow<decltype(&k_p1_scatter_s<0, 0, 1>)> p1s() { return {sel_of(K_P1_SCATTER_S, 0, 0, B, K, T, TOP8), k_p1_scatter_s<B, K, T, TOP8>}; }
template <int K> static KernelRow<decltype(&k_p1_scatter_c<0>)> p1c() { return {sel_of(K_P1_SCATTER_C, 0, 0, 0, K), k_p1_scatter_c<K>}; }
template <int W> static KernelRow<decltype(&k_lv_hist<0>)> lvh() { return {sel_of(K_LV_HIST, W, 0, 0, 0), k_lv_hist<W>}; }
template <int W, int N> static KernelRow<decltype(&k_lv_scatter<0, 512>)> lvw() { return {sel_of(K_LV_SCATTER, W, N, 0, 0), k_lv_scatter<W, N>}; }
template <bool T> static KernelRow<decltype(&k_lv_scatter_s<false>)> lvs() { return {sel_of(K_LV_SCATTER_S, 0, 0, 0, 0, 0, T), k_lv_scatter_s<T>}; }
template <int W, bool HOT> static KernelRow<decltype(&k_count_regions<0, false>)> p3g() { return {sel_of(K_COUNT_REGIONS, W, 0, 0, 0, 0, HOT), k_count_regions<W, HOT>}; }
template <int K, bool T> static KernelRow<decltype(&k_count_regions_q4<0, false>)> p3q() { return {sel_of(K_COUNT_REGIONS_Q4, 0, 0, 0, K, 0, T), k_count_regions_q4<K, T>}; }
template <int K, bool T> static KernelRow<decltype(&k_count_regions_q4r<0, false>)> p3r() { return {sel_of(K_COUNT_REGIONS_Q4R, 0, 0, 0, K, 0, T), k_count_regions_q4r<K, T>}; }
template <int W> static KernelRow<decltype(&k_lookup_regions<0>)> lkr() { return {sel_of(K_LOOKUP_REGIONS, W, 0, 0, 0), k_lookup_regions<W>}; }

extern "C" {

const char* kq_last_error(void) { return g_err.c_str(); }
int kq_abi_version(void) { return KQ_ABI_VERSION; }

int kq_device_available(void) {
    int n = 0;
    if (hipGetDeviceCount(&n) != hipSuccess || n <= 0) return 0;
    hipDeviceProp_t p;
    if (hipGetDeviceProperties(&p, 0) != hipSuccess) return 0;
    return strncmp(p.gcnArchName, "gfx950", 6) == 0 ? 1 : 0;
}

int kq_device_memory(int device, uint64_t* free_bytes, uint64_t* total_bytes) {
    if (!free_bytes || !total_bytes) return fail(KQ_ERR_INVALID, "null argument");
    int n = 0;
    if (hipGetDeviceCount(&n) != hipSuccess || n <= 0) return fail(KQ_ERR_NO_DEVICE, "no HIP device visible (this library has no CPU path)");
    if (device < 0 || device >= n) return fail(KQ_ERR_NO_DEVICE, "device %d out of range (%d visible)", device, n);
    HIPC(hipSetDevice(device));
    size_t f = 0, t = 0;
    HIPC(hipMemGetInfo(&f, &t));
    *free_bytes = f; *total_bytes = t;
    return KQ_OK;
}

static int set_window(kq_handle* h, uint32_t lo, uint32_t hi, bool shard = false) {
    if (lo >= hi || hi > 256) return fail(KQ_ERR_INVALID, "bucket window [%u, %u) is not a range of the 256 hash-prefix buckets", lo, hi);
    if (shard && h->k > (int)NARROW_MAX_K && h->k < HI_K)
        return fail(KQ_ERR_INVALID, "shard windows need k <= %u (5-byte records) or k >= %d (8-byte hash-remainder records); k = %u..%d shards own map ranges", NARROW_MAX_K, HI_K, NARROW_MAX_K + 1, HI_K - 1);
    if (!shard && h->k > (int)NARROW_MAX_K) return fail(KQ_ERR_INVALID, "bucket windows need k <= %u (5-byte records)", NARROW_MAX_K);
    if (!h->table_empty || h->n_pend || h->kmers_bound) return fail(KQ_ERR_INVALID, "the bucket window is chosen before anything is counted");
    if (h->windowed && hi - lo == h->win_hi - h->win_lo && !(lo == 0 && hi == 256)) {
        HIPC(hipStreamSynchronize(h->stream));
        h->win_lo = lo; h->win_hi = hi;
        return KQ_OK;
    }
    const WindowGeom g = window_geometry(h->n_alloc_regions(), lo, hi, h->k);
    if (!g.ok) return fail(KQ_ERR_INVALID, "bucket window too narrow for a table of %llu regions", (unsigned long long)h->n_alloc_regions());
    HIPC(hipStreamSynchronize(h->stream));
    DevMem slots, rstart;
    int rc = alloc_main(h, g.virt, g.alloc_new, slots, rstart);
    if (rc) return rc;
    HIPC(hipStreamSynchronize(h->stream));
    slots.swap(h->slots); rstart.swap(h->rstart);
    h->n_regions = g.virt; h->win_lo = lo; h->win_hi = hi; h->windowed = !(lo == 0 && hi == 256);
    h->slots_dirty = false;
    return KQ_OK;
}

int kq_create(kq_handle** out, int device, int k, int map_count, uint64_t capacity_hint) {
    if (!out) return fail(KQ_ERR_INVALID, "out is null");
    *out = nullptr;
    if (k < 2 || k > 32) return fail(KQ_ERR_INVALID, "k must be in 2..32 (got %d)", k);
    if (map_count < 1 || map_count > 65535) return fail(KQ_ERR_INVALID, "map_count must be in 1..65535 (got %d)", map_count);
    int n = 0;
    if (hipGetDeviceCount(&n) != hipSuccess || n <= 0) return fail(KQ_ERR_NO_DEVICE, "no HIP device visible (this library has no CPU path)");
    if (device < 0 || device >= n) return fail(KQ_ERR_NO_DEVICE, "device %d out of range (%d visible)", device, n);
    HIPC(hipSetDevice(device));
    hipDeviceProp_t prop;
    HIPC(hipGetDeviceProperties(&prop, device));
    if (strncmp(prop.gcnArchName, "gfx950", 6) != 0)
        return fail(KQ_ERR_NO_DEVICE, "device %d is %s; this library carries gfx950 code only", device, prop.gcnArchName);
    kq_handle* h = new (std::nothrow) kq_handle();
    if (!h) return fail(KQ_ERR_NOMEM, "host allocation failed");
    h->device = device; h->k = k; h->map_count = map_count; h->n_cu = prop.multiProcessorCount;
    h->filt_hi = (uint32_t)map_count;
    hipError_t e = h->own_stream.create(hipStreamNonBlocking);
    if (e != hipSuccess) { delete h; return fail(KQ_ERR_HIP, "hipStreamCreate: %s", hipGetErrorString(e)); }
    h->stream = h->base = h->own_stream.get();
    int rc = KQ_OK;
    do {
        if (h->st.alloc(sizeof(DevState)) != hipSuccess || h->st_host.alloc(sizeof(DevState)) != hipSuccess) {
            rc = fail(KQ_ERR_NOMEM, "state allocation failed"); break;
        }
        (void)hipMemsetAsync(h->d_state(), 0, sizeof(DevState), h->stream);
        const uint64_t regions = initial_regions(capacity_hint, k);
        rc = alloc_main(h, regions, regions, h->slots, h->rstart); if (rc) break;
        h->n_regions = regions;
        uint64_t hc = 1u << 16;
        rc = alloc_hc(h, hc, h->hc); if (rc) break;
        h->hc_cap = hc;
        if (hipStreamSynchronize(h->stream) != hipSuccess) { rc = fail(KQ_ERR_HIP, "table initialisation failed"); break; }
    } while (0);
    if (rc) { kq_destroy(h); return rc; }
    *out = h;
    return KQ_OK;
}

void kq_destroy(kq_handle* h) {
    if (!h) return;
    (void)hipSetDevice(h->device);
    if (h->stream) (void)hipStreamSynchronize(h->stream);
    for (auto& s : h->fork_stream) if (s) (void)hipStreamSynchronize(s.get());
    if (h->copy_stream) (void)hipStreamSynchronize(h->copy_stream.get());
    delete h;
}

int kq_clear(kq_handle* h) {
    if (!h) return fail(KQ_ERR_INVALID, "null handle");
    HIPC(hipSetDevice(h->device));
    h->slots_dirty = true;
    clear_words(h, h->hc.get(), sizeof(HcSlot) / 8, h->hc_cap);
    HIPC(hipMemsetAsync(h->d_state(), 0, sizeof(DevState), h->stream));
    h->kmers_bound = 0;
    h->used_bound = 0;
    h->hc_check_at = 0;
    h->table_empty = true;
    h->n_pend = 0; h->arena_used = 0; h->pend_records = 0;
    h->fx_bad = 0;
    h->bz_bad = false; h->bz_carry_len = 0;
    return KQ_OK;
}

int kq_set_stream(kq_handle* h, void* s) {
    if (!h) return fail(KQ_ERR_INVALID, "null handle");
    HIPC(hipStreamSynchronize(h->stream));
    h->stream = h->base = s ? (hipStream_t)s : h->own_stream.get();
    return KQ_OK;
}
int kq_set_option(kq_handle* h, int option, int64_t value) {
    if (!h) return fail(KQ_ERR_INVALID, "null handle");
    switch (option) {
        case KQ_OPT_TRUST_CAPACITY: h->trust_capacity = value != 0; return KQ_OK;
        case KQ_OPT_COUNT_PATH:
            if (value < 0 || value > 2) return fail(KQ_ERR_INVALID, "KQ_OPT_COUNT_PATH must be 0, 1 or 2");
            h->count_path = (int)value; return KQ_OK;
        case KQ_OPT_COUNT_MAP_RANGE: {
            const int64_t lo = value & 0xFFFF, hi = (value >> 16) & 0xFFFF;
            if (lo >= hi || hi > h->map_count) return fail(KQ_ERR_INVALID, "map range [%lld,%lld) outside [0,%d]", (long long)lo, (long long)hi, h->map_count);
            h->filt_lo = (uint32_t)lo; h->filt_hi = (uint32_t)hi; return KQ_OK;
        }
        case KQ_OPT_NARROW_MID:
            if (value < 2 || value > (1 << 14)) return fail(KQ_ERR_INVALID, "KQ_OPT_NARROW_MID must be in [2, 16384]");
            h->mid_rps = (uint32_t)value; return KQ_OK;
        case KQ_OPT_MERGE_PATH:
            if (value < 0 || value > 2) return fail(KQ_ERR_INVALID, "KQ_OPT_MERGE_PATH must be 0, 1 or 2");
            h->merge_path = (int)value; return KQ_OK;
        case KQ_OPT_LOOKUP_PATH:
            if (value < 0 || value > 2) return fail(KQ_ERR_INVALID, "KQ_OPT_LOOKUP_PATH must be 0, 1 or 2");
            h->lookup_path = (int)value; return KQ_OK;
        case KQ_OPT_PROFILE: h->profile = value != 0; if (!h->profile) marks_reset(h); return KQ_OK;
        case KQ_OPT_TEST_FAIL_PLAN: h->test_fail_plan = value != 0; return KQ_OK;
        case KQ_OPT_COUNT_MAP_PASSES: {
            if (value != 1 && value != 2 && value != 4 && value != 8) return fail(KQ_ERR_INVALID, "KQ_OPT_COUNT_MAP_PASSES must be 1, 2, 4 or 8");
            if ((h->map_count & (h->map_count - 1)) != 0 || value > h->map_count) return fail(KQ_ERR_INVALID, "KQ_OPT_COUNT_MAP_PASSES needs a power-of-two map count");
            HIPC(hipStreamSynchronize(h->stream));
            h->hist_cache.clear(); h->hist_cache_bytes = 0;
            h->map_passes = (int)value; return KQ_OK;
        }
        case KQ_OPT_KERNEL_SET:
            if (value < 0 || (value & ~(int64_t)KS_ALL)) return fail(KQ_ERR_INVALID, "KQ_OPT_KERNEL_SET is a mask of bits 1, 2, 4, 16, 32, 64, 128");
            h->kernel_set = (int)value; return KQ_OK;
        case KQ_OPT_OVERLAP:
            if (value < 0 || value > 2) return fail(KQ_ERR_INVALID, "KQ_OPT_OVERLAP must be 0, 1 or 2");
            h->overlap = (int)value; return KQ_OK;
        case KQ_OPT_PENDING_BYTES: {
            if (value < -1) return fail(KQ_ERR_INVALID, "KQ_OPT_PENDING_BYTES must be -1 (auto), 0 (off) or a byte count");
            int rc = flush_pending(h);
            if (rc) return rc;
            if (h->arena.p && value != h->pend_budget) { HIPC(hipStreamSynchronize(h->stream)); h->arena.reset(); h->arena_bytes = 0; }
            h->pend_budget = value; return KQ_OK;
        }
        case KQ_OPT_BUCKET_WINDOW:
            HIPC(hipSetDevice(h->device));
            return set_window(h, (uint32_t)(value & 0xFFFF), (uint32_t)((value >> 16) & 0xFFFF));
        case KQ_OPT_SHARD_WINDOW:
            HIPC(hipSetDevice(h->device));
            return set_window(h, (uint32_t)(value & 0xFFFF), (uint32_t)((value >> 16) & 0xFFFF), true);
        case KQ_OPT_SLICE_KMERS:
            if (value < 1) return fail(KQ_ERR_INVALID, "KQ_OPT_SLICE_KMERS must be positive");
            h->slice_kmers = (uint64_t)value; h->slice_user = true; return KQ_OK;
        case KQ_OPT_SUBGRAPH_BATCH:
            if (value < 0) return fail(KQ_ERR_INVALID, "KQ_OPT_SUBGRAPH_BATCH must be 0 (automatic) or a number of searches");
            h->sg_batch = (uint64_t)value; return KQ_OK;
        case KQ_OPT_VARIANT_BATCH:
            if (value < 0) return fail(KQ_ERR_INVALID, "KQ_OPT_VARIANT_BATCH must be 0 (automatic) or a number of searches");
            h->var_batch = (uint64_t)value; return KQ_OK;
        default: return fail(KQ_ERR_INVALID, "unknown option %d", option);
    }
}
int kq_get_profile(kq_handle* h, char* buf, uint64_t cap) {
    if (!h || !buf || !cap) return fail(KQ_ERR_INVALID, "null argument");
    HIPC(hipSetDevice(h->device));
    HIPC(hipStreamSynchronize(h->stream));
    std::string out;
    for (size_t i = 1; i < h->marks.size(); ++i) {
        float ms = 0;
        HIPC(hipEventElapsedTime(&ms, h->marks[i - 1].second.get(), h->marks[i].second.get()));
        char tmp[96];
        snprintf(tmp, sizeof tmp, "%s%s=%.4f", out.empty() ? "" : ";", h->marks[i].first, ms);
        out += tmp;
    }
    if (out.size() + 1 > cap) return fail(KQ_ERR_CAPACITY, "profile buffer too small: need %zu", out.size() + 1);
    memcpy(buf, out.c_str(), out.size() + 1);
    return KQ_OK;
}
void* kq_get_stream(kq_handle* h) { return h ? (void*)h->stream : nullptr; }
int kq_sync(kq_handle* h) {
    if (!h) return fail(KQ_ERR_INVALID, "null handle");
    HIPC(hipSetDevice(h->device));
    HIPC(hipStreamSynchronize(h->stream));
    const int rc = check_errors(h);
    if (h->bz_bad) return fail(KQ_ERR_INVALID, "%s: submitted for counting and skipped (kq_clear resets this)", h->bz_err.c_str());
    if (h->fx_bad) return fail(KQ_ERR_INVALID, "malformed %s text was submitted for counting and skipped (kq_clear resets this)", h->fx_bad == KQ_FASTX_FASTQ ? "FASTQ" : "FASTA");
    return rc;
}
int kq_flush(kq_handle* h) {
    if (!h) return fail(KQ_ERR_INVALID, "null handle");
    HIPC(hipSetDevice(h->device));
    return flush_pending(h);
}
int kq_get_info(kq_handle* h, kq_info* out) {
    if (!h || !out) return fail(KQ_ERR_INVALID, "null argument");
    HIPC(hipSetDevice(h->device));
    int rc = read_state(h);
    if (rc) return rc;
    out->kmers_counted = h->host_state()->kmers_added;
    out->slots_used = h->host_state()->slots_used;
    out->slots_total = h->n_slots();
    out->hc_used = h->host_state()->hc_used;
    out->hc_total = h->hc_cap;
    out->table_bytes = h->n_slots() * sizeof(Slot) + h->hc_cap * sizeof(HcSlot);
    out->table_passes = h->table_passes;
    return KQ_OK;
}

struct PartPlan : PlanSizes {
    bool even_buckets = false;
    uint64_t *recs1, *recs2;
    uint8_t *aux1, *aux2;
    unsigned long long *m1, *seg_off, *unit_base, *group_base, *sums, *total, *hot;
    uint32_t* m2;
    uint8_t* a1() const { return fmt == FMT_WIDE || fmt == FMT_NARROW ? aux1 : nullptr; }
    uint8_t* a2() const { return fmt == FMT_WIDE || fmt == FMT_NARROW ? aux2 : nullptr; }
};
static int plan_alloc(kq_handle* h, PartPlan* p, uint64_t n_max, uint64_t n_tiles, uint32_t p1_bins, bool allow_narrow = false,
                      uint64_t min_segs = 0 ) {
    if (h->test_fail_plan) { h->test_fail_plan = false; return fail(KQ_ERR_NOMEM, "partition scratch allocation failed (injected by KQ_OPT_TEST_FAIL_PLAN)"); }
    if (n_max >= (1ull << 32) - 16) return fail(KQ_ERR_INVALID, "a partition pass handles fewer than 2^32 records (got %llu): slice the input", (unsigned long long)n_max);
    static_cast<PlanSizes&>(*p) = plan_sizes(h->shape(), h->n_cu, n_max, n_tiles, p1_bins, allow_narrow, min_segs);
    const PlanLayout at = plan_layout(*p);
    if (p->split2) { int rc2 = scr_ensure(h->work.part2, at.part2_bytes, h->device); if (rc2) return rc2; }
    HIPC(h->work.part.ensure((size_t)at.words * 8));
    uint64_t* const base = h->work.part.as<uint64_t>();
    uint64_t* const base2 = p->split2 ? (uint64_t*)h->work.part2.p : base;
    p->recs1 = base + at.recs1; p->aux1 = (uint8_t*)(base + at.aux1);
    p->recs2 = base2 + at.recs2; p->aux2 = (uint8_t*)(base2 + at.aux2);
    p->m1 = (unsigned long long*)(base + at.m1);
    p->seg_off = (unsigned long long*)(base + at.seg_off);
    p->unit_base = (unsigned long long*)(base + at.unit_base);
    p->group_base = (unsigned long long*)(base + at.group_base);
    p->sums = (unsigned long long*)(base + at.sums);
    p->total = (unsigned long long*)(base + at.total);
    p->hot = (unsigned long long*)(base + at.hot);
    p->m2 = (uint32_t*)(base + at.m2);
    return KQ_OK;
}
static void scan_u64(kq_handle* h, unsigned long long* a, uint64_t n, unsigned long long* sums_scratch, unsigned long long* total) {
    if (n <= 2 * SCAN_CHUNK) {
        hipLaunchKernelGGL(k_exclusive_scan, dim3(1), dim3(1024), 0, h->stream, a, n, total);
        return;
    }
    const uint64_t chunks = (n + SCAN_CHUNK - 1) / SCAN_CHUNK;
    hipLaunchKernelGGL(k_scan_sums, dim3((unsigned)chunks), dim3(1024), 0, h->stream, a, n, sums_scratch);
    hipLaunchKernelGGL(k_exclusive_scan, dim3(1), dim3(1024), 0, h->stream, sums_scratch, chunks, total);
    hipLaunchKernelGGL(k_scan_apply, dim3((unsigned)chunks), dim3(1024), 0, h->stream, a, n, sums_scratch);
}
static void mark(kq_handle* h, const char* name) {
    if (!h->profile) return;
    Event e;
    if (e.create(hipEventDefault) != hipSuccess) return;
    (void)hipEventRecord(e.get(), h->stream);
    h->marks.emplace_back(name, std::move(e));
}
static void marks_reset(kq_handle* h) { h->marks.clear(); }

struct P1Scan { const uint8_t* ab; uint64_t lead, len; EmitRange er; const uint16_t* pinv; };
static int launch_p1_hist(kq_handle* h, const KernelSel& s, uint32_t grid, const P1Scan& in, const PartCfg& cfg, uint32_t g1, unsigned long long* m1) {
    static const KernelRow<decltype(&k_p1_hist<0, 0>)> rows[] = {p1h<6, 21>(), p1h<6, 31>(), p1h<6, 0>(), p1h<2, 21>(), p1h<2, 0>(), p1h<1, 31>(), p1h<1, 0>(),
                                                                  p1h<3, 21>(), p1h<3, 0>(), p1h<4, 21>(), p1h<4, 0>(), p1h<0, 0>(), p1h<5, 21>(), p1h<5, 0>()};
    return launch_row(rows, "k_p1_hist", s, h, dim3(grid), dim3(TILE_THREADS), in.ab, in.lead, in.len, h->k, cfg, in.er, g1, m1, in.pinv);
}
static int launch_p1_scatter(kq_handle* h, const KernelSel& s, uint32_t grid, const P1Scan& in, const PartCfg& cfg, const unsigned long long* m1, uint64_t* out, uint8_t* out_aux, int aux_fmt) {
    static const KernelRow<decltype(&k_p1_scatter<0, 512, 0, 0>)> wide[] = {
        p1w<FMT_TOP8, 512, 6, 31>(), p1w<FMT_TOP8, 512, 6, 0>(), p1w<FMT_TOP8, 512, 2, 31>(), p1w<FMT_TOP8, 512, 2, 0>(), p1w<FMT_TOP8, 512, 0, 0>(),
        p1w<FMT_NARROW, 512, 4, 21>(), p1w<FMT_NARROW, 512, 4, 0>(), p1w<FMT_NARROW, 512, 6, 21>(), p1w<FMT_NARROW, 512, 6, 0>(), p1w<FMT_NARROW, 512, 2, 21>(), p1w<FMT_NARROW, 512, 2, 0>(), p1w<FMT_NARROW, 512, 0, 0>(),
        p1w<FMT_WIDE, 512, 1, 31>(), p1w<FMT_WIDE, NB_MAX, 1, 31>(), p1w<FMT_WIDE, 512, 0, 0>(), p1w<FMT_WIDE, NB_MAX, 0, 0>(),
        p1w<FMT_PACK8, 512, 3, 21>(), p1w<FMT_PACK8, 512, 3, 0>(), p1w<FMT_PACK8, 512, 1, 0>(), p1w<FMT_PACK8, NB_MAX, 1, 0>(), p1w<FMT_PACK8, 512, 0, 0>(), p1w<FMT_PACK8, NB_MAX, 0, 0>()};
    static const KernelRow<decltype(&k_p1_scatter_s<0, 0, 1>)> streamed[] = {
        p1s<4, 21, 1>(), p1s<4, 0, 1>(), p1s<6, 21, 1>(), p1s<6, 0, 1>(), p1s<2, 21, KQ_P1S_TPR>(), p1s<2, 0, KQ_P1S_TPR>(), p1s<0, 0, 1>(),
        p1s<6, 31, 1, true>(), p1s<6, 0, 1, true>(), p1s<2, 31, 1, true>(), p1s<2, 0, 1, true>(), p1s<0, 0, 1, true>()};
    static const KernelRow<decltype(&k_p1_scatter_c<0>)> compact[] = {p1c<21>(), p1c<0>()};
    if (s.fam == K_P1_SCATTER_S) return launch_row(streamed, "k_p1_scatter_s", s, h, dim3(grid), dim3(TILE_THREADS * s.tpr), in.ab, in.lead, in.len, h->k, cfg, in.er, m1, (uint32_t*)out, out_aux, in.pinv);
    if (s.fam == K_P1_SCATTER_C) return launch_row(compact, "k_p1_scatter_c", s, h, dim3(grid), dim3(TILE_THREADS), in.ab, in.lead, in.len, h->k, cfg, in.er, m1, (uint32_t*)out, out_aux, in.pinv);
    return launch_row(wide, "k_p1_scatter", s, h, dim3(grid), dim3(TILE_THREADS), in.ab, in.lead, in.len, h->k, cfg, in.er, m1, out, out_aux, aux_fmt, in.pinv);
}

static int run_p1(kq_handle* h, PartPlan* p, const PartCfg& cfg, const uint8_t* ab, uint64_t lead, uint64_t len, EmitRange er, uint64_t* out,
                  uint8_t* out_aux, int aux_fmt, const uint16_t* pinv = nullptr ) {
    const P1Scan in{ab, lead, len, er, pinv};
    const bool full_range = cfg.filt_lo == 0 && cfg.filt_hi == cfg.map_count, windowed = cfg.win_lo != 0 || cfg.win_hi != (1u << NARROW_CBITS);
    const KernelSel hist = select_p1_hist(h->k, cfg.mode, cfg.narrow, cfg.map_mask, full_range, windowed);
    const bool narrow_filt = hist.bin == 4, narrow_win = hist.bin == 6;
    int rc = KQ_OK;
    auto cached_hist = [&](const kq_handle::HistKey& key, size_t bytes, const PartCfg& all) -> kq_handle::HistEntry* {
        for (auto& e : h->hist_cache) if (e.key == key) return &e;
        if (h->hist_cache_bytes + bytes > ((size_t)4 << 30)) return nullptr;
        DevMem buf;
        if (buf.alloc(bytes) != hipSuccess) { (void)hipGetLastError(); return nullptr; }
        rc = launch_p1_hist(h, select_p1_hist_cached(h->k, hist.bin), p->g1, in, all, p->g1, buf.as<unsigned long long>());
        if (rc) return nullptr;
        h->hist_cache.push_back(kq_handle::HistEntry{key, std::move(buf)});
        h->hist_cache_bytes += bytes;
        return &h->hist_cache.back();
    };
    bool have_hist = false;
    const size_t row = (size_t)p->g1 * sizeof(unsigned long long), block = row << NARROW_CBITS;
    if (narrow_filt && h->map_passes > 1 && P1_F == 1 && !h->hist_cache_off) {
        const uint32_t n = (uint32_t)h->map_passes, per = cfg.map_count / n, rr = cfg.filt_lo / per;
        if (cfg.filt_lo == rr * per && cfg.filt_hi == (rr + 1) * per) {
            PartCfg all = cfg;
            all.n_rng = n; all.n_coarse = n << NARROW_CBITS;
            if (const auto* ent = cached_hist({ab, pinv, lead, len, er.lo, er.hi, p->g1, n, h->k}, n * block, all)) {
                (void)hipMemcpyAsync(p->m1, ent->m1_all.as<char>() + rr * block, block, hipMemcpyDeviceToDevice, h->stream);
                have_hist = true;
            }
        }
    }
    if (narrow_win && h->map_passes > 1 && P1_F == 1 && !h->hist_cache_off) {
        PartCfg all = cfg;
        all.win_lo = 0; all.win_hi = 1u << NARROW_CBITS;
        if (const auto* ent = cached_hist({ab, pinv, lead, len, er.lo, er.hi, p->g1, 0xB0C4E7u, h->k}, block, all)) {
            (void)hipMemcpyAsync(p->m1, ent->m1_all.get(), block, hipMemcpyDeviceToDevice, h->stream);
            if (cfg.win_lo) (void)hipMemsetAsync(p->m1, 0, (size_t)cfg.win_lo * row, h->stream);
            if (cfg.win_hi < (1u << NARROW_CBITS)) (void)hipMemsetAsync((char*)p->m1 + (size_t)cfg.win_hi * row, 0, (size_t)((1u << NARROW_CBITS) - cfg.win_hi) * row, h->stream);
            have_hist = true;
        }
    }
    if (!rc && !have_hist) rc = launch_p1_hist(h, hist, p->g1 * P1_F, in, cfg, p->g1, p->m1);
    if (rc) return rc;
    scan_u64(h, p->m1, (uint64_t)cfg.n_coarse * p->g1 * P1_F, p->sums, p->total);
    hipLaunchKernelGGL(k_p1_offsets, dim3((cfg.n_coarse + 256) / 256), dim3(256), 0, h->stream, p->m1, p->total, cfg, p->g1, p->seg_off);
    mark(h, "k_p1_hist+scan");
    rc = launch_p1_scatter(h, select_p1_scatter(h->k, cfg.mode, cfg.narrow, cfg.map_mask, full_range, windowed, out_aux != nullptr, cfg.n_coarse, KQ_P1S_TPR, h->kernel_set), p->g1, in, cfg, p->m1, out, out_aux, aux_fmt);
    mark(h, "k_p1_scatter");
    return rc;
}
struct LevelIn { const uint64_t* recs; const uint8_t* aux; const unsigned long long *seg_lo, *seg_hi; uint32_t n_seg, spb; };
static LevelIn own_segments(const PartPlan& p, const uint64_t* recs, const uint8_t* aux, uint32_t n_seg) { return LevelIn{recs, aux, p.seg_off, p.seg_off + 1, n_seg, 1}; }
struct LevelUnits { const uint64_t* in; const uint8_t* in_aux; LevelCfg lv; const unsigned long long *seg_lo, *seg_hi, *unit_base; uint32_t* m2; unsigned grid; };
static int launch_level_hist(kq_handle* h, const KernelSel& s, const LevelUnits& u) {
    static const KernelRow<decltype(&k_lv_hist<0>)> rows[] = {lvh<FMT_TOP8>(), lvh<FMT_NARROW>(), lvh<FMT_WIDE>(), lvh<FMT_PACK8>()};
    return launch_row(rows, "k_lv_hist", s, h, dim3(u.grid), dim3(MS_THREADS), u.in, u.in_aux, u.lv, u.seg_lo, u.seg_hi, u.unit_base, u.m2);
}
static int launch_level_scatter(kq_handle* h, const KernelSel& s, const LevelUnits& u, const unsigned long long* gb, uint64_t* out, uint8_t* out_aux) {
    static const KernelRow<decltype(&k_lv_scatter<0, 512>)> rows[] = {
        lvw<FMT_PACK8_TO_NARROW, 512>(), lvw<FMT_TOP8, 512>(), lvw<FMT_TOP8, NB_MAX>(), lvw<FMT_NARROW_TO_TIGHT, 512>(), lvw<FMT_NARROW_TO_TIGHT, NB_MAX>(),
        lvw<FMT_NARROW, 512>(), lvw<FMT_NARROW, NB_MAX>(), lvw<FMT_WIDE, 512>(), lvw<FMT_WIDE, NB_MAX>(), lvw<FMT_PACK8, 512>(), lvw<FMT_PACK8, NB_MAX>()};
    static const KernelRow<decltype(&k_lv_scatter_s<false>)> streamed[] = {lvs<true>(), lvs<false>()};
    if (s.fam == K_LV_SCATTER_S) return launch_row(streamed, "k_lv_scatter_s", s, h, dim3(u.grid), dim3(LV_THREADS), (const uint32_t*)u.in, u.in_aux, u.lv, u.seg_lo, u.seg_hi, u.unit_base, u.m2, gb, (uint32_t*)out, out_aux);
    return launch_row(rows, "k_lv_scatter", s, h, dim3(u.grid), dim3(LV_THREADS), u.in, u.in_aux, u.lv, u.seg_lo, u.seg_hi, u.unit_base, u.m2, gb, out, out_aux);
}
static int run_level(kq_handle* h, PartPlan* p, const LevelCfg& lv, const LevelIn& src, uint64_t* out, uint8_t* out_aux,
                     unsigned long long* gb = nullptr ) {
    if (!gb) gb = p->group_base;
    const LevelCfg lv_ = with_rep_shift(lv);
    const uint64_t groups = (uint64_t)(lv.n_seg / lv.spb) * lv.nb;
    hipLaunchKernelGGL(k_lv_units, dim3(1), dim3(1024), 0, h->stream, src.seg_lo, src.seg_hi, lv_, p->unit_base);
    const LevelUnits u{src.recs, src.aux, lv_, src.seg_lo, src.seg_hi, p->unit_base, p->m2, (unsigned)std::min<uint64_t>(p->n_max / P2_UNIT + lv.n_seg + 1, 1u << 30)};
    int rc = launch_level_hist(h, select_level_hist(lv.narrow, src.aux != nullptr), u);
    if (rc) return rc;
    if (p->n_max / P2_UNIT + 1 <= 8 * (uint64_t)(lv.n_seg / lv.spb))
        hipLaunchKernelGGL(k_lv_offsets_thread, dim3((unsigned)((groups + 255) / 256)), dim3(256), 0, h->stream, p->m2, lv_, p->unit_base, gb);
    else
        hipLaunchKernelGGL(k_lv_offsets, dim3((unsigned)((groups * 64 + 255) / 256)), dim3(256), 0, h->stream, p->m2, lv_, p->unit_base, gb);
    (void)hipMemsetAsync(gb + groups, 0, 8, h->stream);
    scan_u64(h, gb, groups + 1, p->sums, p->total + 1);
    mark(h, "k_lv_hist+offsets+scan");
    rc = launch_level_scatter(h, select_level_scatter(lv.narrow, src.aux != nullptr, lv.top8 != 0, lv.nb, lv.rstart != nullptr, h->kernel_set), u, gb, out, out_aux);
    mark(h, "k_lv_scatter");
    return rc;
}
static void run_segment_level(kq_handle* h, PartPlan* p, const LevelCfg& lv, const uint64_t* in, const uint8_t* in_aux, uint64_t* out, unsigned long long* gb) {
    mark(h, "segment_level");
    mark(h, "k_lv_hist+offsets+scan");
    hipLaunchKernelGGL(k_lv_segment_s, dim3(lv.n_seg), dim3(LV_THREADS), 0, h->stream, (const uint32_t*)in, in_aux, with_rep_shift(lv), p->seg_off, gb, (uint32_t*)out);
    mark(h, "k_lv_scatter");
}
__global__ void k_p3set(P3Set* sets, int i, P3Set v) { sets[i] = v; }

struct Dest {
    int fmt, aux_fmt;
    bool tight = false;
    uint64_t* recs = nullptr; uint8_t* aux = nullptr; unsigned long long* base = nullptr; uint64_t n_max = 0;
    bool in_arena() const { return recs != nullptr; }
};
static int arena_take(kq_handle* h, uint64_t n_max, uint64_t R, Dest* d) {
    if (h->pend_budget == 0) return KQ_OK;
    const int fmt = d->fmt;
    const SetLayout lay = set_bytes(n_max, fmt, R);
    const size_t need = lay.total;
    bool was_full = false;
    if (h->n_pend && (h->n_pend >= P3_MAX_SETS || h->pend_fmt != fmt || h->arena_used + need > h->arena_bytes)) {
        was_full = h->pend_fmt == fmt && h->n_pend < P3_MAX_SETS;
        int rc = flush_pending(h);
        if (rc) return rc;
    }
    const size_t want = arena_want(need, h->arena_bytes, was_full, h->pend_budget);
    if (want > h->arena_bytes) {
        size_t free_b = 0, total_b = 0;
        if (hipMemGetInfo(&free_b, &total_b) != hipSuccess) return KQ_OK;
        const size_t budget = arena_budget(want, need, h->arena_bytes, h->pend_budget, free_b, total_b, (size_t)h->table_bytes());
        if (budget == ARENA_STAY) return KQ_OK;
        if (budget) {
            if (h->arena.p) { HIPC(hipStreamSynchronize(h->stream)); HIPC(hipStreamSynchronize(h->base)); h->arena.reset(); h->arena_bytes = 0; }
            static const bool scramble_arena = !getenv("KQ_SCRAMBLE_ARENA") || atoi(getenv("KQ_SCRAMBLE_ARENA")) != 0;
            if (!h->arena.alloc(budget, h->device, scramble_arena && budget >= ((size_t)1 << 30))) return KQ_OK;
            h->arena_bytes = budget; h->arena_used = 0;
        }
    }
    uint8_t* set = (uint8_t*)h->arena.p + h->arena_used;
    d->recs = (uint64_t*)set;
    d->aux = lay.has_aux ? set + lay.aux_off : nullptr;
    d->base = (unsigned long long*)(set + lay.base_off);
    d->n_max = n_max;
    h->arena_used += need;
    return KQ_OK;
}
static int pend_add(kq_handle* h, const P3Set& set, int fmt, int aux_fmt) {
    if (h->n_pend && (h->n_pend >= P3_MAX_SETS || h->pend_fmt != fmt || h->pend_aux_fmt != aux_fmt)) {
        int rc = flush_pending(h);
        if (rc) return rc;
    }
    if (!h->d_sets) HIPC(h->d_sets.alloc(sizeof(P3Set) * P3_MAX_SETS));
    hipLaunchKernelGGL(k_p3set, dim3(1), dim3(1), 0, h->stream, h->d_sets.as<P3Set>(), h->n_pend, set);
    h->pend_sets[h->n_pend] = set;
    h->pend_fmt = fmt; h->pend_aux_fmt = aux_fmt;
    ++h->n_pend;
    h->pend_records += set.n_max;
    return KQ_OK;
}
static int flush_pending_base(kq_handle* h);
static int flush_pending(kq_handle* h) {
    if (!h->n_pend) return KQ_OK;
    hipStream_t work = h->stream;
    h->stream = h->base;
    int rc = join_forks(h);
    if (!rc) rc = flush_pending_base(h);
    if (!rc && h->fork_stream[0]) {
        hipEvent_t e; rc = ev_get(h, &e);
        if (!rc && hipEventRecord(e, h->base) != hipSuccess) rc = fail(KQ_ERR_HIP, "hipEventRecord failed");
        for (int w = 0; w < 2 && !rc; ++w) if (hipStreamWaitEvent(h->fork_stream[w].get(), e, 0) != hipSuccess) rc = fail(KQ_ERR_HIP, "hipStreamWaitEvent failed");
    }
    h->stream = work;
    return rc;
}
static_assert(ROFF_MAX_SETS == (uint32_t)P3_MAX_SETS, "the offset matrix has a column for every set of a pass");
static uint32_t* roff_take(kq_handle* h) {
    for (int i = 0; i < h->n_pend; ++i) if (h->pend_sets[i].n_max >> 32) return nullptr;
    const size_t need = roff_bytes(h->n_alloc_regions());
    if (!need || !roff_pitch((uint32_t)h->n_pend)) return nullptr;
    if (h->roff.bytes() < need && h->roff.alloc(need) != hipSuccess) { (void)hipGetLastError(); return nullptr; }
    return h->roff.as<uint32_t>();
}
static int launch_table_pass(kq_handle* h, const KernelSel& s, dim3 grid, const Q4SetsRow& rows, int empty, unsigned long long* hot, uint32_t rps) {
    static const KernelRow<decltype(&k_count_regions<0, false>)> generic[] = {p3g<FMT_TOP8, false>(), p3g<FMT_WIDE, false>(), p3g<FMT_PACK8, false>(), p3g<FMT_NARROW, true>(), p3g<FMT_TOP8, true>(), p3g<FMT_WIDE, true>(), p3g<FMT_PACK8, true>()};
    static const KernelRow<decltype(&k_count_regions_q4<0, false>)> compact[] = {p3q<21, true>(), p3q<0, true>(), p3q<21, false>(), p3q<0, false>()};
    static const KernelRow<decltype(&k_count_regions_q4r<0, false>)> matrix[] = {p3r<21, true>(), p3r<0, true>(), p3r<21, false>(), p3r<0, false>()};
    const P3Set* sets = h->d_sets.as<P3Set>();
    if (s.fam == K_COUNT_REGIONS_Q4R) return launch_row(matrix, "k_count_regions_q4r", s, h, grid, dim3(Q4_THREADS), h->view(), rows, empty, hot, rps);
    if (s.fam == K_COUNT_REGIONS_Q4) return launch_row(compact, "k_count_regions_q4", s, h, grid, dim3(Q4_THREADS), h->view(), sets, (uint32_t)h->n_pend, empty, hot, rps);
    return launch_row(generic, "k_count_regions", s, h, grid, dim3(P3_THREADS), h->view(), sets, (uint32_t)h->n_pend, h->pend_aux_fmt, empty, hot, rps);
}
static int flush_pending_base(kq_handle* h) {
    const uint64_t R = h->n_regions;
    HIPC(h->hot.ensure((size_t)(R + 2) * 8));
    int rc;
    if (hc_follows_fill(h->kmers_bound)) {
        rc = read_state_raw(h); if (rc) return rc;
        const uint64_t need_hc = hc_need(h->kmers_bound, h->host_state()->hc_used);
        if (need_hc > h->hc_cap) { rc = grow_hc(h, need_hc); if (rc) return rc; }
    }
    unsigned long long* hot = h->hot.as<unsigned long long>();
    HIPC(hipMemsetAsync(hot, 0, 8, h->stream));
    const dim3 grid((unsigned)std::min<uint64_t>(h->n_alloc_regions(), 1u << 30)), grid_hot(h->n_cu);
    const int empty = h->slots_dirty ? 2 : h->table_empty ? 1 : 0;
    const int fmt = h->pend_fmt;
    const uint32_t rps = (fmt == FMT_NARROW || fmt == FMT_TIGHT || fmt == FMT_TOP8) ? (uint32_t)(R >> NARROW_CBITS) : 1u;
    Q4SetsRow rows = {};
    if (table_pass_wants_matrix(fmt, h->kernel_set)) {
        if (uint32_t* roff = roff_take(h)) {
            rows.pitch = roff_pitch((uint32_t)h->n_pend);
            if (!h->tot) {
                const size_t tb = (size_t)TOT_LINES * 64;
                if (h->tot.alloc(tb) != hipSuccess) (void)hipGetLastError();
                else HIPC(hipMemsetAsync(h->tot.get(), 0, tb, h->stream));
            }
            rows.tot = h->tot.as<unsigned long long>();
            rows.roff = roff - h->reg_lo() * rows.pitch;
            for (int i = 0; i < h->n_pend; ++i) { rows.d[i].recs = (const uint32_t*)h->pend_sets[i].recs; rows.d[i].aux = h->pend_sets[i].aux; }
            const uint64_t n_rows = roff_rows(h->n_alloc_regions());
            hipLaunchKernelGGL(k_p3_region_offsets, dim3(grid_for(h, n_rows, ROFF_ROWS, 32)), dim3(ROFF_THREADS), 0, h->stream,
                               roff, h->d_sets.as<P3Set>(), (uint32_t)h->n_pend, rows.pitch, h->reg_lo(), n_rows);
        }
    }
    rc = launch_table_pass(h, select_table_pass(fmt, h->k, rows.roff != nullptr), grid, rows, empty, hot, rps);
    if (!rc) rc = launch_table_pass(h, select_hot_pass(fmt), grid_hot, rows, empty, hot, rps);
    if (rc) return rc;
    if (rows.roff && rows.tot) hipLaunchKernelGGL(k_fold_totals, dim3(1), dim3(256), 0, h->stream, rows.tot, h->d_state());
    h->n_pend = 0; h->arena_used = 0; h->pend_records = 0;
    ++h->table_passes;
    h->slots_dirty = false;
    h->table_empty = false;
    mark(h, "k_count_regions");
    HIPC(hipGetLastError());
    return KQ_OK;
}

static int dest_take(kq_handle* h, const PartPlan& p, uint64_t n_max, Dest* d) {
    d->tight = tight_ok(p.fmt, p.R, (bool)h->rstart);
    if (d->tight) { d->fmt = FMT_TIGHT; d->aux_fmt = AUX_TIGHT; }
    return arena_take(h, n_max, p.R, d);
}
static int sort_to_regions(kq_handle* h, PartPlan* p, const LevelIn& in, const Dest& d, P3Set* set) {
    const bool arena = d.in_arena();
    int rc = KQ_OK;
    uint64_t* fin = arena ? d.recs : p->recs2;
    uint8_t* fin_aux = arena ? d.aux : p->a2();
    unsigned long long* fin_base = arena ? d.base : p->group_base;
    if (p->fmt == FMT_NARROW || p->fmt == FMT_TOP8) {
        const uint32_t sb = p->cfg.sub_bits;
        const bool t8 = p->fmt == FMT_TOP8;
        const bool mid_to_2 = sb != 0 && in.recs == p->recs1;
        if (!arena && mid_to_2) { fin = p->recs1; fin_aux = p->a1(); }
        if (d.tight) fin_aux = nullptr;
        LevelCfg last = level_narrow(p->cfg, sb, false, t8);
        if (d.tight) last.rstart = h->rstart.as<uint32_t>();
        if (sb == 0) {
            last.n_seg = in.n_seg; last.spb = in.spb;
            rc = run_level(h, p, last, in, fin, fin_aux, fin_base);
        } else {
            LevelCfg mid = level_narrow(p->cfg, sb, true, t8);
            mid.n_seg = in.n_seg; mid.spb = in.spb;
            uint64_t* m = mid_to_2 ? p->recs2 : p->recs1;
            uint8_t* m_aux = mid_to_2 ? p->a2() : p->a1();
            rc = run_level(h, p, mid, in, m, m_aux);
            if (rc) return rc;
            (void)hipMemcpyAsync(p->seg_off, p->group_base, (size_t)(((1u << NARROW_CBITS) << sb) + 1) * 8, hipMemcpyDeviceToDevice, h->stream);
            if (select_last_level(p->fmt, last.narrow, last.rstart != nullptr, last.nr_shift, last.nb, last.spb, p->even_buckets, h->kernel_set).fam == K_LV_SEGMENT_S)
                run_segment_level(h, p, last, m, m_aux, fin, fin_base);
            else
                rc = run_level(h, p, last, own_segments(*p, m, m_aux, last.n_seg), fin, fin_aux, fin_base);
        }
    } else if (p->two_level) {
        rc = run_level(h, p, level_coarse_to_regions(p->cfg), in, fin, fin_aux, fin_base);
    } else {
        *set = P3Set{in.recs, in.aux, in.seg_lo, p->n_max};
        return KQ_OK;
    }
    *set = P3Set{fin, fin_aux, fin_base, arena ? d.n_max : p->n_max};
    return rc;
}

static int submit(kq_handle* h, const P3Set& set, const Dest& d) {
    HIPC(hipGetLastError());
    int rc = pend_add(h, set, d.fmt, d.aux_fmt);
    if (rc) return rc;
    return d.in_arena() ? KQ_OK : flush_pending(h);
}
static int sort_and_submit(kq_handle* h, PartPlan* p, const LevelIn& in, const Dest& d) {
    P3Set set; int rc = sort_to_regions(h, p, in, d, &set);
    return rc ? rc : submit(h, set, d);
}

static int plan_sequence(kq_handle* h, PartPlan* p, uint64_t lead, uint64_t len) {
    int rc = plan_alloc(h, p, len, n_tiles_of(lead, len), plan_cfg(h->shape(), true).n_coarse, true);
    if (rc) return rc;
    p->fmt = sequence_fmt(p->fmt, h->k);
    return KQ_OK;
}

static int count_partitioned(kq_handle* h, const uint8_t* ab, uint64_t lead, uint64_t len, EmitRange er, const uint16_t* pinv = nullptr) {
    PartPlan p;
    int rc = plan_sequence(h, &p, lead, len);
    if (rc) return rc;
    p.cfg.filt_lo = h->filt_lo; p.cfg.filt_hi = h->filt_hi;
    if (h->windowed) { p.cfg.win_lo = h->win_lo; p.cfg.win_hi = h->win_hi; }
    const bool leveled = p.fmt == FMT_NARROW || p.fmt == FMT_TOP8 || p.two_level;
    Dest dst{p.fmt, AUX_IDX6};
    const bool filtered = p.cfg.filt_lo != 0 || p.cfg.filt_hi != p.cfg.map_count || h->windowed;
    if (leveled && !filtered) { rc = dest_take(h, p, p.n_max, &dst); if (rc) return rc; }
    marks_reset(h);
    mark(h, "start");
    rc = run_p1(h, &p, p.cfg, ab, lead, len, er, p.recs1, p.a1(), AUX_IDX6, pinv);
    if (rc) return rc;
    if (leveled && filtered) {
        constexpr uint32_t NBK = 1u << NARROW_CBITS;
        const bool with_offsets = p.fmt == FMT_NARROW && p.cfg.sub_bits != 0 && p.cfg.n_coarse == NBK;
        unsigned long long offs[NBK + 1];
        unsigned long long n_recs = 0;
        if (with_offsets) HIPC(hipMemcpyAsync(offs, p.seg_off, sizeof offs, hipMemcpyDeviceToHost, h->stream));
        else HIPC(hipMemcpyAsync(&n_recs, p.total, sizeof n_recs, hipMemcpyDeviceToHost, h->stream));
        HIPC(hipStreamSynchronize(h->stream));
        if (with_offsets) { n_recs = offs[NBK]; p.even_buckets = kq::seg_gate_even(offs, NBK); }
        rc = dest_take(h, p, std::min<uint64_t>(p.n_max, ((uint64_t)n_recs + 15) & ~7ull), &dst); if (rc) return rc;
    }
    return sort_and_submit(h, &p, own_segments(p, p.recs1, p.a1(), p.cfg.n_coarse), dst);
}
static int count_partitioned_records(kq_handle* h, const uint64_t* d_recs, const uint8_t* d_aux, int aux_fmt, uint64_t n, bool raw) {
    PartPlan p;
    int rc = plan_alloc(h, &p, n, 0, 1, !d_aux && !raw);
    if (rc) return rc;
    if (d_aux) p.fmt = FMT_WIDE;
    Dest dst{p.fmt, aux_fmt};
    LevelCfg first = level_flat_to_coarse(p.cfg);
    if (p.fmt == FMT_NARROW) {
        rc = dest_take(h, p, p.n_max, &dst); if (rc) return rc;
        first.top8 = 1;
    } else {
        first.in_raw = raw ? 1 : 0; first.k = (uint32_t)h->k;
    }
    hipLaunchKernelGGL(k_set2, dim3(1), dim3(1), 0, h->stream, p.seg_off, 0ull, (unsigned long long)n);
    rc = run_level(h, &p, first, own_segments(p, d_recs, d_aux, 1), p.recs1, p.a1());
    if (rc) return rc;
    LevelIn coarse{p.recs1, p.a1(), p.group_base, p.group_base + 1, p.cfg.n_coarse, 1};
    if (p.two_level) {
        HIPC(hipMemcpyAsync(p.seg_off, p.group_base, (size_t)(p.cfg.n_coarse + 1) * 8, hipMemcpyDeviceToDevice, h->stream));
        coarse = own_segments(p, p.recs1, p.a1(), p.cfg.n_coarse);
    }
    return sort_and_submit(h, &p, coarse, dst);
}

static int count_seq_dev(kq_handle* h, const char* d_bases, const uint16_t* d_inv, uint64_t len) {
    if (!h || (!d_bases && len)) return fail(KQ_ERR_INVALID, "null argument");
    HIPC(hipSetDevice(h->device));
    if (len < (uint64_t)h->k) return KQ_OK;
    const uint64_t kmers = len - h->k + 1;
    size_t free_b = 0, total_b = 0;
    const bool have_mem_info = slice_reads_free(kmers, h->slice_kmers, h->slice_user, h->pend_budget, h->n_slots()) && hipMemGetInfo(&free_b, &total_b) == hipSuccess;
    const uint64_t slice = choose_slice(kmers, h->slice_kmers, h->slice_user, h->pend_budget, h->n_slots(), free_b, h->work.part.bytes(), have_mem_info);
    struct ForkGuard {
        kq_handle* h; bool swapped = false;
        void leave() { if (swapped) { std::swap(h->work, h->fork_work); swapped = false; } h->stream = h->base; }
        ~ForkGuard() { leave(); (void)join_forks(h); }
    } guard{h};
    const bool forked = slices_fork(h->overlap, h->profile, h->count_path, kmers, slice, h->filt_lo == 0 && h->filt_hi == (uint32_t)h->map_count && !h->windowed);
    if (forked) {
        for (int w = 0; w < 2; ++w) if (!h->fork_stream[w]) HIPC(h->fork_stream[w].create(hipStreamNonBlocking));
        hipEvent_t e_in; int erc = ev_get(h, &e_in); if (erc) return erc;
        HIPC(hipEventRecord(e_in, h->base));
        for (int w = 0; w < 2; ++w) HIPC(hipStreamWaitEvent(h->fork_stream[w].get(), e_in, 0));
    }
    uint64_t slice_no = 0;
    for (uint64_t a = 0; a < kmers; a += slice, ++slice_no) {
        const uint64_t b = std::min(kmers, a + slice);
        int rc = reserve(h, b - a, b - a);
        if (rc) return rc;
        const SliceView v = slice_view(d_bases, d_inv, len, h->k, a, b);
        const bool table_ok = part_table_ok(h->shape(), true);
        bool part = slice_partitions(b - a, table_ok, h->table_bytes(), h->n_regions, h->pend_budget, h->pend_records, h->arena.p != nullptr, h->arena_bytes);
        if (h->count_path == 1) part = false;
        if (h->count_path == 2) {
            if (!table_ok) return fail(KQ_ERR_INVALID, "table too large for the partitioned path");
            part = true;
        }
        if (part) {
            if (forked) {
                const int w = (int)(slice_no & 1);
                if (w == 1) { std::swap(h->work, h->fork_work); guard.swapped = true; }
                h->stream = h->fork_stream[w].get();
                h->fork_busy[w] = true;
            }
            rc = count_partitioned(h, v.ab, v.lead, v.len, v.er, v.pinv);
            if (forked) h->fork_busy[slice_no & 1] = true;
            guard.leave();
            if (rc) return rc;
            continue;
        }
        if (forked) { rc = join_forks(h); if (rc) return rc; }
        PartCfg filt = plan_cfg(h->shape());
        filt.filt_lo = h->filt_lo; filt.filt_hi = h->filt_hi;
        materialize(h);
        h->table_empty = false;
        hipLaunchKernelGGL(k_count_direct, dim3(grid_for(h, n_tiles_of(v.lead, v.len), 1, 32)), dim3(TILE_THREADS), 0, h->stream,
                           h->view(), v.ab, v.lead, v.len, h->k, v.er, filt, v.pinv);
        HIPC(hipGetLastError());
    }
    return KQ_OK;
}
int kq_count_batch_dev(kq_handle* h, const char* d_bases, uint64_t len) { return count_seq_dev(h, d_bases, nullptr, len); }
int kq_count_packed_dev(kq_handle* h, const uint32_t* d_codes, const uint16_t* d_inv, uint64_t n_bases) {
    if (!d_inv && n_bases) return fail(KQ_ERR_INVALID, "null argument");
    return count_seq_dev(h, (const char*)d_codes, d_inv, n_bases);
}
void kq_pack_bases(const char* bases, uint64_t len, uint32_t* codes, uint16_t* inv) {
    static const struct Lut { uint8_t v[256]; Lut() { for (int i = 0; i < 256; ++i) v[i] = 4; v['A'] = v['a'] = 0; v['C'] = v['c'] = 1; v['G'] = v['g'] = 2; v['T'] = v['t'] = 3; } } lut;
    const uint64_t full = len / 16;
    const uint8_t* b = (const uint8_t*)bases;
    for (uint64_t u = 0; u < full; ++u, b += 16) {
        uint32_t c = 0, m = 0;
        for (int i = 0; i < 16; ++i) { const uint32_t x = lut.v[b[i]]; c |= (x & 3u) << (2 * i); m |= (x >> 2) << i; }
        codes[u] = c; inv[u] = (uint16_t)m;
    }
    if (len % 16) {
        uint32_t c = 0, m = 0xFFFFu;
        for (uint64_t i = 0; i < len % 16; ++i) { const uint32_t x = lut.v[b[i]]; c |= (x & 3u) << (2 * i); if (!(x >> 2)) m &= ~(1u << i); }
        codes[full] = c; inv[full] = (uint16_t)m;
    }
}
int kq_count_batch(kq_handle* h, const char* bases, uint64_t len) {
    if (!h || (!bases && len)) return fail(KQ_ERR_INVALID, "null argument");
    HIPC(hipSetDevice(h->device));
    void* d = nullptr;
    int rc = stage_in(h, bases, len, &d);
    if (rc) return rc;
    rc = kq_count_batch_dev(h, (const char*)d, len);
    if (rc) return rc;
    HIPC(hipStreamSynchronize(h->stream));
    return KQ_OK;
}

void* kq_host_alloc(uint64_t bytes) {
    const size_t n = ((size_t)(bytes ? bytes : 1) + 4095) & ~(size_t)4095;
    void* p = aligned_alloc(4096, n);
    if (!p) return nullptr;
    if (hipHostRegister(p, n, hipHostRegisterDefault) != hipSuccess) { (void)hipGetLastError(); free(p); return nullptr; }
    return p;
}
void kq_host_free(void* p) { if (p) { (void)hipHostUnregister(p); free(p); } }

static int ingest_begin(kq_handle* h, size_t bytes, uint64_t* ticket, int* slot, hipEvent_t* copied) {
    if (!h->copy_stream) {
        for (auto& e : h->in_consumed) HIPC(e.create(hipEventDisableTiming));
        h->in_copied.resize(kq_handle::IN_TICKETS);
        for (auto& e : h->in_copied) HIPC(e.create(hipEventDisableTiming));
        HIPC(h->copy_stream.create(hipStreamNonBlocking));
    }
    const uint64_t t = h->in_next++;
    const int s = (int)(t % kq_handle::IN_SLOTS);
    *copied = h->in_copied[t % kq_handle::IN_TICKETS].get();
    *ticket = t; *slot = s;
    h->in_bad[t % kq_handle::IN_TICKETS] = 0;
    if (t >= (uint64_t)kq_handle::IN_SLOTS) HIPC(hipStreamWaitEvent(h->copy_stream.get(), h->in_consumed[s].get(), 0));
    if (h->in_buf[s].bytes() < bytes + 64) {
        if (h->in_buf[s]) { HIPC(hipStreamSynchronize(h->copy_stream.get())); HIPC(hipStreamSynchronize(h->stream)); }
        HIPC(h->in_buf[s].alloc(bytes + bytes / 4 + 4096));
    }
    return KQ_OK;
}
static int ingest_async(kq_handle* h, const void* a, size_t a_bytes, const void* b, size_t b_bytes, uint64_t n_bases, uint64_t* ticket) {
    HIPC(hipSetDevice(h->device));
    std::lock_guard<std::mutex> lock(h->in_m);
    const size_t b_off = (a_bytes + 63) & ~(size_t)63, bytes = b_off + b_bytes;
    int s = 0; hipEvent_t copied;
    int rc = ingest_begin(h, bytes, ticket, &s, &copied);
    if (rc) return rc;
    char* d = h->in_buf[s].as<char>();
    if (a_bytes) HIPC(hipMemcpyAsync(d, a, a_bytes, hipMemcpyHostToDevice, h->copy_stream.get()));
// ... 1667 lines not shown
```

Before: 59.74 billion.

## Split pending arena into per-band slabs and apply table bands independently

Adds a banded pending-record pool that divides the region space into eight bands, each with its own arena slab. The final partition level writes each band's records to its own slab, and the fullest band can be applied to the table on its own, so the whole pending arena no longer has to be flushed at once. Table clearing skips bands already written, and the phase-1 offsets readback now goes to pinned host memory behind an event instead of a full stream synchronize. This adds considerable bookkeeping complexity and risks fragmentation or extra passes when the bands are uneven.

Measured after the change: 57.87 billion. 0.969x the previous value.

```diff
diff --git a/include/kreeq_amd.h b/include/kreeq_amd.h
--- a/include/kreeq_amd.h
+++ b/include/kreeq_amd.h
@@ -50,6 +50,7 @@
     uint64_t hc_total;
     uint64_t table_bytes;
     uint64_t table_passes;
+    uint64_t band_passes;
 } kq_info;
 
 
diff --git a/kreeq_amd/build.py b/kreeq_amd/build.py
--- a/kreeq_amd/build.py
+++ b/kreeq_amd/build.py
@@ -9,7 +9,7 @@
 HOSTLIB = os.path.join(PKG, "lib", "libkreeq_host.so")
 
 HIP_SOURCES = [os.path.join(PKG, "csrc", "kreeq_amd.hip")]
-HIP_DEPS = HIP_SOURCES + [os.path.join(PKG, "csrc", f) for f in ("kq_device.h", "kq_partition.h", "kq_kernels.h", "kq_fastx.h", "kq_bgzf.h", "kq_bgzf_host.h", "kq_inflate_core.h", "kq_deflate.h", "kq_deflate_core.h", "kq_dbimage.h", "kq_dbimage_host.h", "kq_mem_host.h", "kq_plan_host.h", "kq_roff_host.h", "kq_seg_gate_host.h", "kq_select_host.h", "kq_formats.h", "kq_subgraph.h", "kq_gfa.h", "kq_bestfirst_core.h", "kq_nodequeue_core.h", "kq_variant_core.h", "kq_variants.h", "kq_table_core.h", "kq_table.h")] + [os.path.join(ROOT, "include", "kreeq_amd.h")]
+HIP_DEPS = HIP_SOURCES + [os.path.join(PKG, "csrc", f) for f in ("kq_device.h", "kq_partition.h", "kq_kernels.h", "kq_fastx.h", "kq_bgzf.h", "kq_bgzf_host.h", "kq_inflate_core.h", "kq_deflate.h", "kq_deflate_core.h", "kq_dbimage.h", "kq_dbimage_host.h", "kq_mem_host.h", "kq_plan_host.h", "kq_band_host.h", "kq_roff_host.h", "kq_seg_gate_host.h", "kq_select_host.h", "kq_formats.h", "kq_subgraph.h", "kq_gfa.h", "kq_bestfirst_core.h", "kq_nodequeue_core.h", "kq_variant_core.h", "kq_variants.h", "kq_table_core.h", "kq_table.h")] + [os.path.join(ROOT, "include", "kreeq_amd.h")]
 HOST_DIR = os.path.join(PKG, "host")
 DECOMPRESSOR_DIR = os.path.join(HOST_DIR, "decompressor")
 DECOMPRESSOR = os.path.join(PKG, "bin", "kreeq-decompressor")
diff --git a/kreeq_amd/capi.py b/kreeq_amd/capi.py
--- a/kreeq_amd/capi.py
+++ b/kreeq_amd/capi.py
@@ -49,7 +49,7 @@
 
 class Info(C.Structure):
     _fields_ = [("kmers_counted", C.c_uint64), ("slots_used", C.c_uint64), ("slots_total", C.c_uint64), ("hc_used", C.c_uint64),
-                ("hc_total", C.c_uint64), ("table_bytes", C.c_uint64), ("table_passes", C.c_uint64)]
+                ("hc_total", C.c_uint64), ("table_bytes", C.c_uint64), ("table_passes", C.c_uint64), ("band_passes", C.c_uint64)]
 
 
 _lib = None
diff --git a/kreeq_amd/csrc/kq_band_host.h b/kreeq_amd/csrc/kq_band_host.h
--- /dev/null
+++ b/kreeq_amd/csrc/kq_band_host.h
@@ -0,0 +1,132 @@
+#pragma once
+#include <cstddef>
+#include <cstdint>
+#include <vector>
+
+namespace kq {
+
+constexpr uint32_t N_BANDS = 8;
+constexpr uint32_t BAND_BUCKETS = 256 / N_BANDS;
+constexpr uint32_t BAND_MAX_SETS = 64;
+
+inline uint64_t band_slab_recs(uint64_t bound) {
+    const uint64_t piece = (bound + N_BANDS - 1) / N_BANDS;
+    return (piece + piece / 32 + 4096 + 63) & ~63ull;
+}
+inline size_t band_aux_off(uint64_t recs) { return (size_t)recs * 4; }
+inline size_t band_slab_bytes(uint64_t recs, bool has_aux) { return ((size_t)recs * (has_aux ? 5 : 4) + 255) & ~(size_t)255; }
+inline size_t band_off_bytes(uint64_t R) { return ((size_t)(R + 2) * 8 + 255) & ~(size_t)255; }
+
+inline uint64_t band_first(const unsigned long long* off, uint32_t b) { return off[b * BAND_BUCKETS]; }
+inline uint64_t band_count(const unsigned long long* off, uint32_t b) { return off[(b + 1) * BAND_BUCKETS] - off[b * BAND_BUCKETS]; }
+inline bool bands_fit(const unsigned long long* off, uint64_t slab_recs) {
+    for (uint32_t b = 0; b < N_BANDS; ++b) {
+        if (off[(b + 1) * BAND_BUCKETS] < off[b * BAND_BUCKETS]) return false;
+        if (band_count(off, b) > slab_recs) return false;
+    }
+    return true;
+}
+inline uintptr_t band_vbase(uintptr_t piece, uint64_t first, uint32_t rec_size) { return piece - (uintptr_t)(first * rec_size); }
+inline int fullest_band(const uint64_t (&bytes)[N_BANDS]) {
+    int best = -1;
+    uint64_t most = 0;
+    for (uint32_t b = 0; b < N_BANDS; ++b) if (bytes[b] > most) { most = bytes[b]; best = (int)b; }
+    return best;
+}
+
+struct BandPool {
+    uint64_t slab_recs = 0;
+    size_t slab_bytes = 0, off_bytes = 0, off_base = 0;
+    uint32_t n_slabs = 0, n_off = 0;
+    bool has_aux = false;
+    std::vector<uint32_t> free_slabs, free_offs;
+
+    bool format(size_t arena_bytes, uint64_t recs, bool aux, uint64_t R) {
+        slab_recs = recs; has_aux = aux;
+        slab_bytes = band_slab_bytes(recs, aux); off_bytes = band_off_bytes(R);
+        n_slabs = n_off = 0; free_slabs.clear(); free_offs.clear();
+        const size_t one_set = (size_t)N_BANDS * slab_bytes + off_bytes;
+        if (arena_bytes < one_set) return false;
+        const size_t whole = arena_bytes / one_set;
+        n_off = (uint32_t)(2 * whole + 1 < BAND_MAX_SETS ? 2 * whole + 1 : BAND_MAX_SETS);
+        while (n_off > 1 && arena_bytes < (size_t)n_off * off_bytes + (size_t)N_BANDS * slab_bytes) --n_off;
+        const size_t slabs = (arena_bytes - (size_t)n_off * off_bytes) / slab_bytes;
+        n_slabs = (uint32_t)(slabs < (1u << 30) ? slabs : (1u << 30));
+        off_base = (size_t)n_slabs * slab_bytes;
+        for (uint32_t i = n_slabs; i-- > 0;) free_slabs.push_back(i);
+        for (uint32_t i = n_off; i-- > 0;) free_offs.push_back(i);
+        return true;
+    }
+    bool all_free() const { return free_slabs.size() == n_slabs && free_offs.size() == n_off; }
+    size_t slab_at(uint32_t slab) const { return (size_t)slab * slab_bytes; }
+    size_t off_at(uint32_t slab) const { return off_base + (size_t)slab * off_bytes; }
+};
+
+struct BandSet {
+    static constexpr uint32_t NONE = 0xFFFFFFFFu;
+    uint32_t slab[N_BANDS], off_slab = NONE, held = 0;
+    uint64_t first[N_BANDS + 1];
+    bool live() const { return held != 0; }
+};
+
+struct BandBook {
+    BandPool pool;
+    BandSet sets[2 * BAND_MAX_SETS];
+    uint32_t list[N_BANDS][BAND_MAX_SETS];
+    uint32_t n_list[N_BANDS] = {};
+    uint64_t bytes[N_BANDS] = {};
+    uint32_t n_live = 0;
+
+    void reset() { for (auto& s : sets) s.held = 0; for (uint32_t b = 0; b < N_BANDS; ++b) { n_list[b] = 0; bytes[b] = 0; } n_live = 0; }
+    bool can_admit() const {
+        if (pool.free_slabs.size() < N_BANDS || pool.free_offs.empty() || n_live >= BAND_MAX_SETS) return false;
+        for (uint32_t b = 0; b < N_BANDS; ++b) if (n_list[b] >= BAND_MAX_SETS) return false;
+        return true;
+    }
+    uint32_t admit(const unsigned long long* off) {
+        uint32_t id = 0;
+        while (sets[id].live()) ++id;
+        BandSet& s = sets[id];
+        for (uint32_t b = 0; b < N_BANDS; ++b) {
+            s.slab[b] = pool.free_slabs.back(); pool.free_slabs.pop_back();
+            s.first[b] = band_first(off, b);
+            list[b][n_list[b]++] = id;
+            bytes[b] += band_count(off, b) * (pool.has_aux ? 5 : 4);
+        }
+        s.first[N_BANDS] = off[256];
+        s.off_slab = pool.free_offs.back(); pool.free_offs.pop_back();
+        s.held = N_BANDS;
+        ++n_live;
+        return id;
+    }
+    void retract(uint32_t id) {
+        BandSet& s = sets[id];
+        for (uint32_t b = N_BANDS; b-- > 0;) {
+            pool.free_slabs.push_back(s.slab[b]);
+            s.slab[b] = BandSet::NONE;
+            --n_list[b];
+            bytes[b] -= (s.first[b + 1] - s.first[b]) * (pool.has_aux ? 5 : 4);
+        }
+        pool.free_offs.push_back(s.off_slab);
+        s.off_slab = BandSet::NONE; s.held = 0;
+        --n_live;
+    }
+    void applied(uint32_t b) {
+        for (uint32_t i = 0; i < n_list[b]; ++i) {
+            BandSet& s = sets[list[b][i]];
+            pool.free_slabs.push_back(s.slab[b]);
+            s.slab[b] = BandSet::NONE;
+            if (--s.held == 0) { pool.free_offs.push_back(s.off_slab); s.off_slab = BandSet::NONE; --n_live; }
+        }
+        n_list[b] = 0; bytes[b] = 0;
+    }
+    int fullest() const {
+        int best = fullest_band(bytes);
+        if (best >= 0) return best;
+        uint32_t most = 0;
+        for (uint32_t b = 0; b < N_BANDS; ++b) if (n_list[b] > most) { most = n_list[b]; best = (int)b; }
+        return best;
+    }
+};
+
+}
diff --git a/kreeq_amd/csrc/kq_formats.h b/kreeq_amd/csrc/kq_formats.h
--- a/kreeq_amd/csrc/kq_formats.h
+++ b/kreeq_amd/csrc/kq_formats.h
@@ -62,5 +62,7 @@
     uint32_t spb;
     uint32_t rep_shift;
     const uint32_t* rstart = nullptr;
+    uint32_t seg0 = 0;
 };
+struct SegOut { uint32_t* v[8]; uint32_t shift; };
 }
diff --git a/kreeq_amd/csrc/kq_kernels.h b/kreeq_amd/csrc/kq_kernels.h
--- a/kreeq_amd/csrc/kq_kernels.h
+++ b/kreeq_amd/csrc/kq_kernels.h
@@ -552,7 +552,8 @@
         for (uint32_t i = threadIdx.x; i < nb; i += LV_THREADS)
             s.gbase[i] = (uint32_t)(group_base[(uint64_t)b * nb + i] + m2[u * nb + i]);
         if (TIGHT) {
-            const uint32_t first = (b >> lv.nr_shift) * lv.nr_rps + (b & ((1u << lv.nr_shift) - 1u)) * lv.nr_sub;
+            const uint32_t bg = b + lv.seg0;
+            const uint32_t first = (bg >> lv.nr_shift) * lv.nr_rps + (bg & ((1u << lv.nr_shift) - 1u)) * lv.nr_sub;
             for (uint32_t i = threadIdx.x; i < nb; i += LV_THREADS) s_rst[i] = lv.rstart[first + i];
         }
         __syncthreads();
@@ -577,7 +578,7 @@
                 aux[j] = nxt_aux[j];
                 if (TIGHT) {
                     const uint32_t bn = i >= hi ? nb : narrow_bin(lv, b, (uint32_t)rec[j]);
-                    rec[j] = narrow_word(tight_rec(b >> lv.nr_shift, (uint32_t)rec[j], aux[j], s_rst[bn < nb ? bn : 0u]), 0u, bn);
+                    rec[j] = narrow_word(tight_rec((b + lv.seg0) >> lv.nr_shift, (uint32_t)rec[j], aux[j], s_rst[bn < nb ? bn : 0u]), 0u, bn);
                 }
                 else if (NARROW) rec[j] = narrow_word((uint32_t)rec[j], aux[j], i >= hi ? nb : narrow_bin(lv, b, (uint32_t)rec[j]));
                 else if (CONVERT) {
@@ -627,7 +628,8 @@
         const uint64_t hi = lo + P2_UNIT < seg_hi[b_in] ? lo + P2_UNIT : seg_hi[b_in];
         uint32_t gabs = own_bin ? (uint32_t)(group_base[(uint64_t)b * nb + my_bin] + m2[u * nb + my_bin]) : 0u;
         if (TIGHT) {
-            const uint32_t first = (b >> lv.nr_shift) * lv.nr_rps + (b & ((1u << lv.nr_shift) - 1u)) * lv.nr_sub;
+            const uint32_t bg = b + lv.seg0;
+            const uint32_t first = (bg >> lv.nr_shift) * lv.nr_rps + (bg & ((1u << lv.nr_shift) - 1u)) * lv.nr_sub;
             if ((uint32_t)tid < nb) s_rst[tid] = lv.rstart[first + tid];
         }
         s_hist[0][tid] = 0;
@@ -650,7 +652,7 @@
             for (int j = 0; j < LV_ITEMS; ++j) {
                 const uint64_t i = pos + (uint64_t)j * LV_THREADS + tid;
                 const uint32_t bn = i >= hi ? nb : narrow_bin(lv, b, nxt[j]);
-                w[j] = TIGHT ? narrow_word(tight_rec(b >> lv.nr_shift, nxt[j], nxt_aux[j], s_rst[bn < nb ? bn : 0u]), 0u, bn) : narrow_word(nxt[j], nxt_aux[j], bn);
+                w[j] = TIGHT ? narrow_word(tight_rec((b + lv.seg0) >> lv.nr_shift, nxt[j], nxt_aux[j], s_rst[bn < nb ? bn : 0u]), 0u, bn) : narrow_word(nxt[j], nxt_aux[j], bn);
                 if (bn != nb) atomicAdd(&hist[(bn << rs) | sub], 1u);
             }
 #pragma unroll
@@ -704,7 +706,7 @@
 #endif
 __global__ __launch_bounds__(LV_THREADS, KQ_LVS_OCC_TIGHT) void k_lv_segment_s(const uint32_t* __restrict__ recs32, const uint8_t* __restrict__ recs_aux, LevelCfg lv,
                                                            const unsigned long long* __restrict__ seg_off, unsigned long long* __restrict__ gb,
-                                                           uint32_t* __restrict__ out) {
+                                                           SegOut where) {
     constexpr int NC = 512;
     constexpr bool BACK = KQ_LVG_BACK != 0;
     static_assert(LV_THREADS == NC && LV_ITEMS == 8, "one counter per thread");
@@ -715,6 +717,7 @@
     const uint32_t sub = (uint32_t)tid & ((1u << rs) - 1u), my_bin = (uint32_t)tid >> rs;
     const bool own_bin = sub == 0 && my_bin < nb;
     const uint32_t b = blockIdx.x;
+    uint32_t* __restrict__ const out = where.v[b >> where.shift];
     const uint64_t lo = seg_off[b], hi = seg_off[b + 1];
     {
         const uint32_t first = (b >> lv.nr_shift) * lv.nr_rps + (b & ((1u << lv.nr_shift) - 1u)) * lv.nr_sub;
diff --git a/kreeq_amd/csrc/kq_select_host.h b/kreeq_amd/csrc/kq_select_host.h
--- a/kreeq_amd/csrc/kq_select_host.h
+++ b/kreeq_amd/csrc/kq_select_host.h
@@ -11,6 +11,7 @@
               KS_SEG_ALWAYS = 64,
               KS_P1_NO_COMPACT = 128,
               KS_ALL = KS_P1_ROUND2 | KS_LV_NARROW_S | KS_LV_TIGHT_UNITS | KS_P3_SET_OFFSETS | KS_SEG_NEVER | KS_SEG_ALWAYS | KS_P1_NO_COMPACT;
+constexpr int KS_NO_BANDS = 512, KS_MASK = KS_ALL | KS_NO_BANDS;
 
 enum Kernel { K_P1_HIST, K_P1_SCATTER, K_P1_SCATTER_S, K_P1_SCATTER_C, K_LV_HIST, K_LV_SCATTER, K_LV_SCATTER_S, K_LV_SEGMENT_S, K_LV_UNITS ,
               K_COUNT_REGIONS, K_COUNT_REGIONS_Q4, K_COUNT_REGIONS_Q4R, K_LOOKUP_REGIONS };
diff --git a/kreeq_amd/csrc/kreeq_amd.hip b/kreeq_amd/csrc/kreeq_amd.hip
--- a/kreeq_amd/csrc/kreeq_amd.hip
+++ b/kreeq_amd/csrc/kreeq_amd.hip
@@ -19,6 +19,7 @@
 #include "kq_partition.h"
 #include "kq_mem_host.h"
 #include "kq_plan_host.h"
+#include "kq_band_host.h"
 #include "kq_roff_host.h"
 #include "kq_seg_gate_host.h"
 #include "kq_select_host.h"
@@ -187,6 +188,16 @@
     uint64_t pend_records = 0;
     int64_t pend_budget = -1;
     uint64_t table_passes = 0;
+    kq::BandBook bands;
+    bool pend_banded = false;
+    const void* pool_arena = nullptr;
+    size_t pool_bytes = 0;
+    uint64_t pool_regions = 0;
+    bool arena_final = false;
+    DevMem d_band_sets;
+    uint8_t band_written = 0;
+    uint64_t band_passes = 0;
+    PinnedMem offs_host;
     static constexpr int IN_SLOTS = 3, IN_TICKETS = 512;
     Stream copy_stream;
     DevMem in_buf[IN_SLOTS];
@@ -268,7 +279,11 @@
 static void clear_main(kq_handle* h, Slot* p, uint64_t n_slots) { (void)hipMemsetAsync(p, 0, (size_t)n_slots * sizeof(Slot), h->stream); }
 static void materialize(kq_handle* h) {
     if (!h->slots_dirty) return;
-    clear_main(h, h->slots.as<Slot>(), h->n_slots());
+    if (!h->band_written) clear_main(h, h->slots.as<Slot>(), h->n_slots());
+    else {
+        const uint64_t per = h->n_slots() / kq::N_BANDS;
+        for (uint32_t b = 0; b < kq::N_BANDS; ++b) if (!(h->band_written >> b & 1)) clear_main(h, h->slots.as<Slot>() + b * per, per);
+    }
     h->slots_dirty = false;
 }
 static int alloc_main(kq_handle* h, uint64_t n_regions, uint64_t alloc_regions, DevMem& slots, DevMem& rstart) {
@@ -518,6 +533,7 @@
     h->hc_check_at = 0;
     h->table_empty = true;
     h->n_pend = 0; h->arena_used = 0; h->pend_records = 0;
+    h->pend_banded = false; h->pool_arena = nullptr; h->band_written = 0;
     h->fx_bad = 0;
     h->bz_bad = false; h->bz_carry_len = 0;
     return KQ_OK;
@@ -560,7 +576,7 @@
             h->map_passes = (int)value; return KQ_OK;
         }
         case KQ_OPT_KERNEL_SET:
-            if (value < 0 || (value & ~(int64_t)KS_ALL)) return fail(KQ_ERR_INVALID, "KQ_OPT_KERNEL_SET is a mask of bits 1, 2, 4, 16, 32, 64, 128");
+            if (value < 0 || (value & ~(int64_t)KS_MASK)) return fail(KQ_ERR_INVALID, "KQ_OPT_KERNEL_SET is a mask of bits 1, 2, 4, 16, 32, 64, 128, 512");
             h->kernel_set = (int)value; return KQ_OK;
         case KQ_OPT_OVERLAP:
             if (value < 0 || value > 2) return fail(KQ_ERR_INVALID, "KQ_OPT_OVERLAP must be 0, 1 or 2");
@@ -570,6 +586,7 @@
             int rc = flush_pending(h);
             if (rc) return rc;
             if (h->arena.p && value != h->pend_budget) { HIPC(hipStreamSynchronize(h->stream)); h->arena.reset(); h->arena_bytes = 0; }
+            h->arena_final = false;
             h->pend_budget = value; return KQ_OK;
         }
         case KQ_OPT_BUCKET_WINDOW:
@@ -633,6 +650,7 @@
     out->hc_total = h->hc_cap;
     out->table_bytes = h->n_slots() * sizeof(Slot) + h->hc_cap * sizeof(HcSlot);
     out->table_passes = h->table_passes;
+    out->band_passes = h->band_passes;
     return KQ_OK;
 }
 
@@ -707,8 +725,9 @@
     return launch_row(wide, "k_p1_scatter", s, h, dim3(grid), dim3(TILE_THREADS), in.ab, in.lead, in.len, h->k, cfg, in.er, m1, out, out_aux, aux_fmt, in.pinv);
 }
 
+struct P1Readback { void* dst; const void* src; size_t bytes; hipEvent_t ev; };
 static int run_p1(kq_handle* h, PartPlan* p, const PartCfg& cfg, const uint8_t* ab, uint64_t lead, uint64_t len, EmitRange er, uint64_t* out,
-                  uint8_t* out_aux, int aux_fmt, const uint16_t* pinv = nullptr ) {
+                  uint8_t* out_aux, int aux_fmt, const uint16_t* pinv = nullptr , const P1Readback* back = nullptr) {
     const P1Scan in{ab, lead, len, er, pinv};
     const bool full_range = cfg.filt_lo == 0 && cfg.filt_hi == cfg.map_count, windowed = cfg.win_lo != 0 || cfg.win_hi != (1u << NARROW_CBITS);
     const KernelSel hist = select_p1_hist(h->k, cfg.mode, cfg.narrow, cfg.map_mask, full_range, windowed);
@@ -752,6 +771,10 @@
     if (rc) return rc;
     scan_u64(h, p->m1, (uint64_t)cfg.n_coarse * p->g1 * P1_F, p->sums, p->total);
     hipLaunchKernelGGL(k_p1_offsets, dim3((cfg.n_coarse + 256) / 256), dim3(256), 0, h->stream, p->m1, p->total, cfg, p->g1, p->seg_off);
+    if (back) {
+        HIPC(hipMemcpyAsync(back->dst, back->src, back->bytes, hipMemcpyDeviceToHost, h->stream));
+        HIPC(hipEventRecord(back->ev, h->stream));
+    }
     mark(h, "k_p1_hist+scan");
     rc = launch_p1_scatter(h, select_p1_scatter(h->k, cfg.mode, cfg.narrow, cfg.map_mask, full_range, windowed, out_aux != nullptr, cfg.n_coarse, KQ_P1S_TPR, h->kernel_set), p->g1, in, cfg, p->m1, out, out_aux, aux_fmt);
     mark(h, "k_p1_scatter");
@@ -773,10 +796,15 @@
     return launch_row(rows, "k_lv_scatter", s, h, dim3(u.grid), dim3(LV_THREADS), u.in, u.in_aux, u.lv, u.seg_lo, u.seg_hi, u.unit_base, u.m2, gb, out, out_aux);
 }
 static int run_level(kq_handle* h, PartPlan* p, const LevelCfg& lv, const LevelIn& src, uint64_t* out, uint8_t* out_aux,
-                     unsigned long long* gb = nullptr ) {
+                     unsigned long long* gb = nullptr , const unsigned long long* seed = nullptr) {
     if (!gb) gb = p->group_base;
+    unsigned long long* const gb_out = gb;
     const LevelCfg lv_ = with_rep_shift(lv);
     const uint64_t groups = (uint64_t)(lv.n_seg / lv.spb) * lv.nb;
+    if (seed) {
+        hipLaunchKernelGGL(k_set2, dim3(1), dim3(1), 0, h->stream, p->group_base, *seed, 0ull);
+        gb = p->group_base + 1;
+    }
     hipLaunchKernelGGL(k_lv_units, dim3(1), dim3(1024), 0, h->stream, src.seg_lo, src.seg_hi, lv_, p->unit_base);
     const LevelUnits u{src.recs, src.aux, lv_, src.seg_lo, src.seg_hi, p->unit_base, p->m2, (unsigned)std::min<uint64_t>(p->n_max / P2_UNIT + lv.n_seg + 1, 1u << 30)};
     int rc = launch_level_hist(h, select_level_hist(lv.narrow, src.aux != nullptr), u);
@@ -786,16 +814,17 @@
     else
         hipLaunchKernelGGL(k_lv_offsets, dim3((unsigned)((groups * 64 + 255) / 256)), dim3(256), 0, h->stream, p->m2, lv_, p->unit_base, gb);
     (void)hipMemsetAsync(gb + groups, 0, 8, h->stream);
-    scan_u64(h, gb, groups + 1, p->sums, p->total + 1);
+    scan_u64(h, seed ? gb - 1 : gb, groups + (seed ? 2 : 1), p->sums, p->total + 1);
     mark(h, "k_lv_hist+offsets+scan");
     rc = launch_level_scatter(h, select_level_scatter(lv.narrow, src.aux != nullptr, lv.top8 != 0, lv.nb, lv.rstart != nullptr, h->kernel_set), u, gb, out, out_aux);
+    if (seed) (void)hipMemcpyAsync(gb_out, gb, (size_t)(groups + 1) * 8, hipMemcpyDeviceToDevice, h->stream);
     mark(h, "k_lv_scatter");
     return rc;
 }
-static void run_segment_level(kq_handle* h, PartPlan* p, const LevelCfg& lv, const uint64_t* in, const uint8_t* in_aux, uint64_t* out, unsigned long long* gb) {
+static void run_segment_level(kq_handle* h, PartPlan* p, const LevelCfg& lv, const uint64_t* in, const uint8_t* in_aux, const SegOut& where, unsigned long long* gb) {
     mark(h, "segment_level");
     mark(h, "k_lv_hist+offsets+scan");
-    hipLaunchKernelGGL(k_lv_segment_s, dim3(lv.n_seg), dim3(LV_THREADS), 0, h->stream, (const uint32_t*)in, in_aux, with_rep_shift(lv), p->seg_off, gb, (uint32_t*)out);
+    hipLaunchKernelGGL(k_lv_segment_s, dim3(lv.n_seg), dim3(LV_THREADS), 0, h->stream, (const uint32_t*)in, in_aux, with_rep_shift(lv), p->seg_off, gb, where);
     mark(h, "k_lv_scatter");
 }
 __global__ void k_p3set(P3Set* sets, int i, P3Set v) { sets[i] = v; }
@@ -805,18 +834,13 @@
     bool tight = false;
     uint64_t* recs = nullptr; uint8_t* aux = nullptr; unsigned long long* base = nullptr; uint64_t n_max = 0;
     bool in_arena() const { return recs != nullptr; }
+    const kq::BandSet* band = nullptr;
+    uint32_t band_id = 0;
+    uint32_t* vrec[kq::N_BANDS] = {};
+    uint8_t* vaux[kq::N_BANDS] = {};
 };
-static int arena_take(kq_handle* h, uint64_t n_max, uint64_t R, Dest* d) {
-    if (h->pend_budget == 0) return KQ_OK;
-    const int fmt = d->fmt;
-    const SetLayout lay = set_bytes(n_max, fmt, R);
-    const size_t need = lay.total;
-    bool was_full = false;
-    if (h->n_pend && (h->n_pend >= P3_MAX_SETS || h->pend_fmt != fmt || h->arena_used + need > h->arena_bytes)) {
-        was_full = h->pend_fmt == fmt && h->n_pend < P3_MAX_SETS;
-        int rc = flush_pending(h);
-        if (rc) return rc;
-    }
+static int arena_fit(kq_handle* h, size_t need, bool was_full, bool* fits) {
+    *fits = false;
     const size_t want = arena_want(need, h->arena_bytes, was_full, h->pend_budget);
     if (want > h->arena_bytes) {
         size_t free_b = 0, total_b = 0;
@@ -830,6 +854,23 @@
             h->arena_bytes = budget; h->arena_used = 0;
         }
     }
+    *fits = h->arena.p != nullptr && need <= h->arena_bytes;
+    return KQ_OK;
+}
+static int arena_take(kq_handle* h, uint64_t n_max, uint64_t R, Dest* d) {
+    if (h->pend_budget == 0) return KQ_OK;
+    const int fmt = d->fmt;
+    const SetLayout lay = set_bytes(n_max, fmt, R);
+    const size_t need = lay.total;
+    bool was_full = false;
+    if (h->n_pend && (h->pend_banded || h->n_pend >= P3_MAX_SETS || h->pend_fmt != fmt || h->arena_used + need > h->arena_bytes)) {
+        was_full = !h->pend_banded && h->pend_fmt == fmt && h->n_pend < P3_MAX_SETS;
+        int rc = flush_pending(h);
+        if (rc) return rc;
+    }
+    bool fits = false;
+    int rc = arena_fit(h, need, was_full, &fits);
+    if (rc || !fits) return rc;
     uint8_t* set = (uint8_t*)h->arena.p + h->arena_used;
     d->recs = (uint64_t*)set;
     d->aux = lay.has_aux ? set + lay.aux_off : nullptr;
@@ -839,7 +880,7 @@
     return KQ_OK;
 }
 static int pend_add(kq_handle* h, const P3Set& set, int fmt, int aux_fmt) {
-    if (h->n_pend && (h->n_pend >= P3_MAX_SETS || h->pend_fmt != fmt || h->pend_aux_fmt != aux_fmt)) {
+    if (h->n_pend && (h->pend_banded || h->n_pend >= P3_MAX_SETS || h->pend_fmt != fmt || h->pend_aux_fmt != aux_fmt)) {
         int rc = flush_pending(h);
         if (rc) return rc;
     }
@@ -852,12 +893,13 @@
     return KQ_OK;
 }
 static int flush_pending_base(kq_handle* h);
+static int band_passes(kq_handle* h, uint32_t mask);
 static int flush_pending(kq_handle* h) {
     if (!h->n_pend) return KQ_OK;
     hipStream_t work = h->stream;
     h->stream = h->base;
     int rc = join_forks(h);
-    if (!rc) rc = flush_pending_base(h);
+    if (!rc) rc = h->pend_banded ? band_passes(h, (1u << kq::N_BANDS) - 1u) : flush_pending_base(h);
     if (!rc && h->fork_stream[0]) {
         hipEvent_t e; rc = ev_get(h, &e);
         if (!rc && hipEventRecord(e, h->base) != hipSuccess) rc = fail(KQ_ERR_HIP, "hipEventRecord failed");
@@ -874,24 +916,36 @@
     if (h->roff.bytes() < need && h->roff.alloc(need) != hipSuccess) { (void)hipGetLastError(); return nullptr; }
     return h->roff.as<uint32_t>();
 }
-static int launch_table_pass(kq_handle* h, const KernelSel& s, dim3 grid, const Q4SetsRow& rows, int empty, unsigned long long* hot, uint32_t rps) {
+static int launch_table_pass(kq_handle* h, const KernelSel& s, dim3 grid, const TableView& view, const P3Set* sets, uint32_t n_sets, const Q4SetsRow& rows, int empty, unsigned long long* hot, uint32_t rps) {
     static const KernelRow<decltype(&k_count_regions<0, false>)> generic[] = {p3g<FMT_TOP8, false>(), p3g<FMT_WIDE, false>(), p3g<FMT_PACK8, false>(), p3g<FMT_NARROW, true>(), p3g<FMT_TOP8, true>(), p3g<FMT_WIDE, true>(), p3g<FMT_PACK8, true>()};
     static const KernelRow<decltype(&k_count_regions_q4<0, false>)> compact[] = {p3q<21, true>(), p3q<0, true>(), p3q<21, false>(), p3q<0, false>()};
     static const KernelRow<decltype(&k_count_regions_q4r<0, false>)> matrix[] = {p3r<21, true>(), p3r<0, true>(), p3r<21, false>(), p3r<0, false>()};
-    const P3Set* sets = h->d_sets.as<P3Set>();
-    if (s.fam == K_COUNT_REGIONS_Q4R) return launch_row(matrix, "k_count_regions_q4r", s, h, grid, dim3(Q4_THREADS), h->view(), rows, empty, hot, rps);
-    if (s.fam == K_COUNT_REGIONS_Q4) return launch_row(compact, "k_count_regions_q4", s, h, grid, dim3(Q4_THREADS), h->view(), sets, (uint32_t)h->n_pend, empty, hot, rps);
-    return launch_row(generic, "k_count_regions", s, h, grid, dim3(P3_THREADS), h->view(), sets, (uint32_t)h->n_pend, h->pend_aux_fmt, empty, hot, rps);
+    if (s.fam == K_COUNT_REGIONS_Q4R) return launch_row(matrix, "k_count_regions_q4r", s, h, grid, dim3(Q4_THREADS), view, rows, empty, hot, rps);
+    if (s.fam == K_COUNT_REGIONS_Q4) return launch_row(compact, "k_count_regions_q4", s, h, grid, dim3(Q4_THREADS), view, sets, n_sets, empty, hot, rps);
+    return launch_row(generic, "k_count_regions", s, h, grid, dim3(P3_THREADS), view, sets, n_sets, h->pend_aux_fmt, empty, hot, rps);
+}
+static int pass_prepare(kq_handle* h) {
+    HIPC(h->hot.ensure((size_t)(h->n_regions + 2) * 8));
+    if (hc_follows_fill(h->kmers_bound)) {
+        int rc = read_state_raw(h); if (rc) return rc;
+        const uint64_t need_hc = hc_need(h->kmers_bound, h->host_state()->hc_used);
+        if (need_hc > h->hc_cap) { rc = grow_hc(h, need_hc); if (rc) return rc; }
+    }
+    return KQ_OK;
+}
+static int tot_take(kq_handle* h, unsigned long long** tot) {
+    if (!h->tot) {
+        const size_t tb = (size_t)TOT_LINES * 64;
+        if (h->tot.alloc(tb) != hipSuccess) (void)hipGetLastError();
+        else HIPC(hipMemsetAsync(h->tot.get(), 0, tb, h->stream));
+    }
+    *tot = h->tot.as<unsigned long long>();
+    return KQ_OK;
 }
 static int flush_pending_base(kq_handle* h) {
     const uint64_t R = h->n_regions;
-    HIPC(h->hot.ensure((size_t)(R + 2) * 8));
-    int rc;
-    if (hc_follows_fill(h->kmers_bound)) {
-        rc = read_state_raw(h); if (rc) return rc;
-        const uint64_t need_hc = hc_need(h->kmers_bound, h->host_state()->hc_used);
-        if (need_hc > h->hc_cap) { rc = grow_hc(h, need_hc); if (rc) return rc; }
-    }
+    int rc = pass_prepare(h);
+    if (rc) return rc;
     unsigned long long* hot = h->hot.as<unsigned long long>();
     HIPC(hipMemsetAsync(hot, 0, 8, h->stream));
     const dim3 grid((unsigned)std::min<uint64_t>(h->n_alloc_regions(), 1u << 30)), grid_hot(h->n_cu);
@@ -902,12 +956,7 @@
     if (table_pass_wants_matrix(fmt, h->kernel_set)) {
         if (uint32_t* roff = roff_take(h)) {
             rows.pitch = roff_pitch((uint32_t)h->n_pend);
-            if (!h->tot) {
-                const size_t tb = (size_t)TOT_LINES * 64;
-                if (h->tot.alloc(tb) != hipSuccess) (void)hipGetLastError();
-                else HIPC(hipMemsetAsync(h->tot.get(), 0, tb, h->stream));
-            }
-            rows.tot = h->tot.as<unsigned long long>();
+            rc = tot_take(h, &rows.tot); if (rc) return rc;
             rows.roff = roff - h->reg_lo() * rows.pitch;
             for (int i = 0; i < h->n_pend; ++i) { rows.d[i].recs = (const uint32_t*)h->pend_sets[i].recs; rows.d[i].aux = h->pend_sets[i].aux; }
             const uint64_t n_rows = roff_rows(h->n_alloc_regions());
@@ -915,16 +964,155 @@
                                roff, h->d_sets.as<P3Set>(), (uint32_t)h->n_pend, rows.pitch, h->reg_lo(), n_rows);
         }
     }
-    rc = launch_table_pass(h, select_table_pass(fmt, h->k, rows.roff != nullptr), grid, rows, empty, hot, rps);
-    if (!rc) rc = launch_table_pass(h, select_hot_pass(fmt), grid_hot, rows, empty, hot, rps);
+    const P3Set* sets = h->d_sets.as<P3Set>();
+    rc = launch_table_pass(h, select_table_pass(fmt, h->k, rows.roff != nullptr), grid, h->view(), sets, (uint32_t)h->n_pend, rows, empty, hot, rps);
+    if (!rc) rc = launch_table_pass(h, select_hot_pass(fmt), grid_hot, h->view(), sets, (uint32_t)h->n_pend, rows, empty, hot, rps);
     if (rc) return rc;
     if (rows.roff && rows.tot) hipLaunchKernelGGL(k_fold_totals, dim3(1), dim3(256), 0, h->stream, rows.tot, h->d_state());
     h->n_pend = 0; h->arena_used = 0; h->pend_records = 0;
     ++h->table_passes;
     h->slots_dirty = false;
     h->table_empty = false;
+    h->band_written = 0;
     mark(h, "k_count_regions");
     HIPC(hipGetLastError());
+    return KQ_OK;
+}
+
+static_assert(kq::BAND_MAX_SETS == (uint32_t)P3_MAX_SETS, "a band pass takes as many sets as any table pass");
+struct BandCols { P3Set v[kq::N_BANDS]; uint32_t col[kq::N_BANDS]; };
+__global__ void k_p3set_bands(P3Set* sets, BandCols c) { if (threadIdx.x < kq::N_BANDS) sets[threadIdx.x * P3_MAX_SETS + c.col[threadIdx.x]] = c.v[threadIdx.x]; }
+
+static void band_counts_to_handle(kq_handle* h) {
+    h->n_pend = (int)h->bands.n_live;
+    uint64_t by = 0;
+    for (uint32_t b = 0; b < kq::N_BANDS; ++b) by += h->bands.bytes[b];
+    h->pend_records = by / (h->bands.pool.has_aux ? 5 : 4);
+    if (!h->n_pend) h->pend_banded = false;
+}
+static int band_pass(kq_handle* h, uint32_t b) {
+    kq::BandBook& bk = h->bands;
+    const uint32_t n = bk.n_list[b];
+    const uint64_t R = h->n_regions, per = R / kq::N_BANDS, r0 = (uint64_t)b * per;
+    const int empty = (h->band_written >> b & 1) ? 0 : h->slots_dirty ? 2 : h->table_empty ? 1 : 0;
+    if (n == 0) {
+        if (empty == 2) clear_main(h, h->slots.as<Slot>() + (r0 << REGION_SHIFT), per << REGION_SHIFT);
+    } else {
+        unsigned long long* hot = h->hot.as<unsigned long long>();
+        HIPC(hipMemsetAsync(hot, 0, 8, h->stream));
+        const dim3 grid((unsigned)std::min<uint64_t>(per, 1u << 30)), grid_hot(h->n_cu);
+        const int fmt = h->pend_fmt;
+        const uint32_t rps = (uint32_t)(R >> NARROW_CBITS);
+        TableView view = h->view();
+        view.reg_lo = r0; view.reg_hi = r0 + per;
+        const P3Set* sets = h->d_band_sets.as<P3Set>() + (size_t)b * P3_MAX_SETS;
+        Q4SetsRow rows = {};
+        int rc;
+        if (table_pass_wants_matrix(fmt, h->kernel_set)) {
+            const size_t need = roff_bytes(h->n_alloc_regions());
+            if (need && h->roff.bytes() < need && h->roff.alloc(need) != hipSuccess) (void)hipGetLastError();
+            if (need && h->roff.bytes() >= need) {
+                uint32_t* roff = h->roff.as<uint32_t>();
+                rows.pitch = roff_pitch(n);
+                rc = tot_take(h, &rows.tot); if (rc) return rc;
+                rows.roff = roff - r0 * rows.pitch;
+                for (uint32_t i = 0; i < n; ++i) {
+                    const kq::BandSet& s = bk.sets[bk.list[b][i]];
+                    const uintptr_t piece = (uintptr_t)h->arena.p + bk.pool.slab_at(s.slab[b]);
+                    rows.d[i].recs = (const uint32_t*)kq::band_vbase(piece, s.first[b], 4);
+                    rows.d[i].aux = bk.pool.has_aux ? (const uint8_t*)kq::band_vbase(piece + kq::band_aux_off(bk.pool.slab_recs), s.first[b], 1) : nullptr;
+                }
+                const uint64_t n_rows = roff_rows(per);
+                hipLaunchKernelGGL(k_p3_region_offsets, dim3(grid_for(h, n_rows, ROFF_ROWS, 32)), dim3(ROFF_THREADS), 0, h->stream, roff, sets, n, rows.pitch, r0, n_rows);
+            }
+        }
+        rc = launch_table_pass(h, select_table_pass(fmt, h->k, rows.roff != nullptr), grid, view, sets, n, rows, empty, hot, rps);
+        if (!rc) rc = launch_table_pass(h, select_hot_pass(fmt), grid_hot, view, sets, n, rows, empty, hot, rps);
+        if (rc) return rc;
+        if (rows.roff && rows.tot) hipLaunchKernelGGL(k_fold_totals, dim3(1), dim3(256), 0, h->stream, rows.tot, h->d_state());
+    }
+    bk.applied(b);
+    band_counts_to_handle(h);
+    ++h->band_passes;
+    h->band_written |= (uint8_t)(1u << b);
+    if (h->band_written == (1u << kq::N_BANDS) - 1u) { h->slots_dirty = false; h->table_empty = false; h->band_written = 0; }
+    return KQ_OK;
+}
+static int band_passes(kq_handle* h, uint32_t mask) {
+    int rc = pass_prepare(h);
+    for (uint32_t b = 0; b < kq::N_BANDS && !rc; ++b) if (mask >> b & 1) rc = band_pass(h, b);
+    if (rc) return rc;
+    ++h->table_passes;
+    mark(h, "k_count_regions");
+    HIPC(hipGetLastError());
+    return KQ_OK;
+}
+static int band_take(kq_handle* h, const PartPlan& p, const unsigned long long* offs, uint64_t bound, Dest* d, bool* banded) {
+    *banded = false;
+    if ((h->kernel_set & KS_NO_BANDS) || h->pend_budget == 0 || h->windowed || h->stream != h->base) return KQ_OK;
+    if (p.fmt != FMT_NARROW || p.R % (1u << NARROW_CBITS) != 0 || bound >= (1ull << 32) - 16 || offs[1u << NARROW_CBITS] > bound) return KQ_OK;
+    const bool tight = tight_ok(p.fmt, p.R, (bool)h->rstart);
+    const int fmt = tight ? FMT_TIGHT : FMT_NARROW, aux_fmt = tight ? AUX_TIGHT : AUX_IDX6;
+    int rc;
+    if (h->n_pend && (!h->pend_banded || h->pend_fmt != fmt)) { rc = flush_pending(h); if (rc) return rc; }
+    kq::BandBook& bk = h->bands;
+    const uint64_t want_recs = kq::band_slab_recs(bound);
+    bool was_full = false, event = false;
+    for (;;) {
+        if (h->n_pend == 0) {
+            const size_t need = (size_t)kq::N_BANDS * kq::band_slab_bytes(want_recs, !tight) + kq::band_off_bytes(p.R);
+            const size_t had = h->arena_bytes;
+            bool fits = false;
+            rc = arena_fit(h, need, was_full, &fits); if (rc) return rc;
+            if (was_full && h->arena_bytes == had) h->arena_final = true;
+            if (!fits) return KQ_OK;
+            const bool carved = h->pool_arena == h->arena.p && h->pool_bytes == h->arena_bytes && h->pool_regions == p.R && bk.pool.has_aux == !tight;
+            if (!carved || !kq::bands_fit(offs, bk.pool.slab_recs) || 2 * want_recs < bk.pool.slab_recs) {
+                bk.reset();
+                h->pool_arena = nullptr;
+                if (!bk.pool.format(h->arena_bytes, want_recs, !tight, p.R)) return KQ_OK;
+                h->pool_arena = h->arena.p; h->pool_bytes = h->arena_bytes; h->pool_regions = p.R;
+            }
+        }
+        if (!kq::bands_fit(offs, bk.pool.slab_recs)) return KQ_OK;
+        if (bk.can_admit()) break;
+        if (h->n_pend == 0) return KQ_OK;
+        if (h->pend_budget < 0 && !h->arena_final) {
+            rc = flush_pending(h); if (rc) return rc;
+            was_full = true;
+            continue;
+        }
+        const int b = bk.fullest();
+        if (b < 0) return KQ_OK;
+        if (!event) { rc = pass_prepare(h); if (rc) return rc; event = true; }
+        rc = band_pass(h, (uint32_t)b); if (rc) return rc;
+    }
+    if (event) { ++h->table_passes; mark(h, "k_count_regions"); HIPC(hipGetLastError()); }
+    const uint32_t id = bk.admit(offs);
+    const kq::BandSet& s = bk.sets[id];
+    for (uint32_t b = 0; b < kq::N_BANDS; ++b) {
+        const uintptr_t piece = (uintptr_t)h->arena.p + bk.pool.slab_at(s.slab[b]);
+        d->vrec[b] = (uint32_t*)kq::band_vbase(piece, s.first[b], 4);
+        d->vaux[b] = tight ? nullptr : (uint8_t*)kq::band_vbase(piece + kq::band_aux_off(bk.pool.slab_recs), s.first[b], 1);
+    }
+    d->tight = tight; d->fmt = fmt; d->aux_fmt = aux_fmt;
+    d->recs = (uint64_t*)d->vrec[0]; d->aux = d->vaux[0];
+    d->base = (unsigned long long*)((uint8_t*)h->arena.p + bk.pool.off_at(s.off_slab));
+    d->n_max = bound;
+    d->band = &s; d->band_id = id;
+    h->pend_banded = true; h->pend_fmt = fmt; h->pend_aux_fmt = aux_fmt;
+    band_counts_to_handle(h);
+    *banded = true;
+    return KQ_OK;
+}
+static int band_submit(kq_handle* h, const Dest& d) {
+    if (!h->d_band_sets) HIPC(h->d_band_sets.alloc(sizeof(P3Set) * P3_MAX_SETS * kq::N_BANDS));
+    BandCols c;
+    for (uint32_t b = 0; b < kq::N_BANDS; ++b) {
+        c.v[b] = P3Set{(const uint64_t*)d.vrec[b], d.vaux[b], d.base, d.n_max};
+        c.col[b] = h->bands.n_list[b] - 1;
+    }
+    hipLaunchKernelGGL(k_p3set_bands, dim3(1), dim3(64), 0, h->stream, h->d_band_sets.as<P3Set>(), c);
     return KQ_OK;
 }
 
@@ -932,6 +1120,21 @@
     d->tight = tight_ok(p.fmt, p.R, (bool)h->rstart);
     if (d->tight) { d->fmt = FMT_TIGHT; d->aux_fmt = AUX_TIGHT; }
     return arena_take(h, n_max, p.R, d);
+}
+static int run_level_bands(kq_handle* h, PartPlan* p, const LevelCfg& lv, const LevelIn& in, const Dest& d, unsigned long long* gb) {
+    const uint32_t per = lv.n_seg / kq::N_BANDS;
+    const bool prof = h->profile;
+    int rc = KQ_OK;
+    for (uint32_t b = 0; b < kq::N_BANDS && !rc; ++b) {
+        LevelCfg lb = lv;
+        lb.n_seg = per; lb.seg0 = b * per;
+        const LevelIn ib{in.recs, in.aux, in.seg_lo + (size_t)b * per, in.seg_hi + (size_t)b * per, per, 1};
+        const unsigned long long seed = d.band->first[b];
+        h->profile = prof && b + 1 == kq::N_BANDS;
+        rc = run_level(h, p, lb, ib, (uint64_t*)d.vrec[b], d.vaux[b], gb + (uint64_t)b * per * lv.nb, &seed);
+    }
+    h->profile = prof;
+    return rc;
 }
 static int sort_to_regions(kq_handle* h, PartPlan* p, const LevelIn& in, const Dest& d, P3Set* set) {
     const bool arena = d.in_arena();
@@ -949,7 +1152,7 @@
         if (d.tight) last.rstart = h->rstart.as<uint32_t>();
         if (sb == 0) {
             last.n_seg = in.n_seg; last.spb = in.spb;
-            rc = run_level(h, p, last, in, fin, fin_aux, fin_base);
+            rc = d.band ? run_level_bands(h, p, last, in, d, fin_base) : run_level(h, p, last, in, fin, fin_aux, fin_base);
         } else {
             LevelCfg mid = level_narrow(p->cfg, sb, true, t8);
             mid.n_seg = in.n_seg; mid.spb = in.spb;
@@ -959,7 +1162,14 @@
             if (rc) return rc;
             (void)hipMemcpyAsync(p->seg_off, p->group_base, (size_t)(((1u << NARROW_CBITS) << sb) + 1) * 8, hipMemcpyDeviceToDevice, h->stream);
             if (select_last_level(p->fmt, last.narrow, last.rstart != nullptr, last.nr_shift, last.nb, last.spb, p->even_buckets, h->kernel_set).fam == K_LV_SEGMENT_S)
-                run_segment_level(h, p, last, m, m_aux, fin, fin_base);
+            {
+                SegOut where;
+                for (uint32_t b = 0; b < kq::N_BANDS; ++b) where.v[b] = d.band ? d.vrec[b] : (uint32_t*)fin;
+                where.shift = 5 + sb;
+                run_segment_level(h, p, last, m, m_aux, where, fin_base);
+            }
+            else if (d.band)
+                rc = run_level_bands(h, p, last, own_segments(*p, m, m_aux, last.n_seg), d, fin_base);
             else
                 rc = run_level(h, p, last, own_segments(*p, m, m_aux, last.n_seg), fin, fin_aux, fin_base);
         }
@@ -975,13 +1185,16 @@
 
 static int submit(kq_handle* h, const P3Set& set, const Dest& d) {
     HIPC(hipGetLastError());
+    if (d.band) return band_submit(h, d);
     int rc = pend_add(h, set, d.fmt, d.aux_fmt);
     if (rc) return rc;
     return d.in_arena() ? KQ_OK : flush_pending(h);
 }
 static int sort_and_submit(kq_handle* h, PartPlan* p, const LevelIn& in, const Dest& d) {
     P3Set set; int rc = sort_to_regions(h, p, in, d, &set);
-    return rc ? rc : submit(h, set, d);
+    if (!rc) rc = submit(h, set, d);
+    if (rc && d.band) { h->bands.retract(d.band_id); band_counts_to_handle(h); }
+    return rc;
 }
 
 static int plan_sequence(kq_handle* h, PartPlan* p, uint64_t lead, uint64_t len) {
@@ -1003,18 +1216,28 @@
     if (leveled && !filtered) { rc = dest_take(h, p, p.n_max, &dst); if (rc) return rc; }
     marks_reset(h);
     mark(h, "start");
-    rc = run_p1(h, &p, p.cfg, ab, lead, len, er, p.recs1, p.a1(), AUX_IDX6, pinv);
-    if (rc) return rc;
-    if (leveled && filtered) {
-        constexpr uint32_t NBK = 1u << NARROW_CBITS;
-        const bool with_offsets = p.fmt == FMT_NARROW && p.cfg.sub_bits != 0 && p.cfg.n_coarse == NBK;
+    constexpr uint32_t NBK = 1u << NARROW_CBITS;
+    const bool read_back = leveled && filtered, with_offsets = p.fmt == FMT_NARROW && p.cfg.n_coarse == NBK;
+    P1Readback back{};
+    if (read_back) {
+        if (!h->offs_host) HIPC(h->offs_host.alloc((NBK + 1) * sizeof(unsigned long long)));
+        back.dst = h->offs_host.get();
+        back.src = with_offsets ? p.seg_off : p.total;
+        back.bytes = (with_offsets ? NBK + 1 : 1) * sizeof(unsigned long long);
+        rc = ev_get(h, &back.ev); if (rc) return rc;
+    }
+    rc = run_p1(h, &p, p.cfg, ab, lead, len, er, p.recs1, p.a1(), AUX_IDX6, pinv, read_back ? &back : nullptr);
+    if (rc) return rc;
+    if (read_back) {
+        HIPC(hipEventSynchronize(back.ev));
         unsigned long long offs[NBK + 1];
-        unsigned long long n_recs = 0;
-        if (with_offsets) HIPC(hipMemcpyAsync(offs, p.seg_off, sizeof offs, hipMemcpyDeviceToHost, h->stream));
-        else HIPC(hipMemcpyAsync(&n_recs, p.total, sizeof n_recs, hipMemcpyDeviceToHost, h->stream));
-        HIPC(hipStreamSynchronize(h->stream));
-        if (with_offsets) { n_recs = offs[NBK]; p.even_buckets = kq::seg_gate_even(offs, NBK); }
-        rc = dest_take(h, p, std::min<uint64_t>(p.n_max, ((uint64_t)n_recs + 15) & ~7ull), &dst); if (rc) return rc;
+        memcpy(offs, h->offs_host.get(), back.bytes);
+        unsigned long long n_recs = offs[0];
+        if (with_offsets) { n_recs = offs[NBK]; p.even_buckets = p.cfg.sub_bits != 0 && kq::seg_gate_even(offs, NBK); }
+        const uint64_t bound = std::min<uint64_t>(p.n_max, ((uint64_t)n_recs + 15) & ~7ull);
+        bool banded = false;
+        if (with_offsets) { rc = band_take(h, p, offs, bound, &dst, &banded); if (rc) return rc; }
+        if (!banded) { rc = dest_take(h, p, bound, &dst); if (rc) return rc; }
     }
     return sort_and_submit(h, &p, own_segments(p, p.recs1, p.a1(), p.cfg.n_coarse), dst);
 }
```
